# itailang/geometric_adv

Hardware: AMD Instinct MI355X
Metric: attack-iterations/sec (B=32, N=2048) at 1/2/4/8 GPUs; Chamfer rel-err vs ref (higher is better)
Workload: dtype f32 (encoder products: f16x2); 1 GPU; BASELINE configs[1]: B=32 random clouds x N=2048, output-space attack (chamfer/chamfer, dist_weight 1.0, lr 0.01), one batch per GPU; batch_per_gpu=32, n_points=2048, global_batch=32, parallelism=batches sharded, dp1, no data-path collective, ranks=1, collective_backend=none, collective_world=1

## Files before the change

### geometric_adv_amd/_abi.py

```python
import ctypes as C

_TYPES = {"i": C.c_int, "f": C.c_float, "d": C.c_double, "q": C.c_longlong, "Q": C.c_ulonglong, "z": C.c_size_t, "p": C.c_void_p,
          "s": C.c_char_p, "v": None}

SIGNATURES = {
    "geoadv_version": "i:",
    "geoadv_last_error": "s:",
    "geoadv_nn_distance": "i:iipipppppp",
    "geoadv_nn_distance_sym_workspace_floats": "z:iii",
    "geoadv_nn_distance_sym_is_screened": "i:iii",
    "geoadv_set_chamfer_screen": "i:i",
    "geoadv_nn_distance_sym": "i:iipippppppzp",
    "geoadv_chamfer_per_pc": "i:iiipppp",
    "geoadv_nn_distance_paired": "i:iippppppp",
    "geoadv_nn_distance_grad": "i:iipipppppppp",
    "geoadv_chamfer_matrix_workspace_floats": "z:iiii",
    "geoadv_chamfer_matrix": "i:iiiippppzp",
    "geoadv_approx_match_temp_floats": "z:iii",
    "geoadv_approx_match": "i:iiippppp",
    "geoadv_approx_match_mode": "i:iiiippppp",
    "geoadv_emd_sparse_levels": "i:i",
    "geoadv_match_cost": "i:iiippppp",
    "geoadv_match_cost_workspace_floats": "z:iii",
    "geoadv_match_cost_ws": "i:iiipppppzp",
    "geoadv_emd_cost_grad1_temp_floats": "z:iii",
    "geoadv_emd_cost_grad1": "i:iiipppppp",
    "geoadv_emd_cost_grad1_mode": "i:iiiipppppp",
    "geoadv_match_cost_grad": "i:iiipppppp",
    "geoadv_query_ball_point": "i:iiifippppp",
    "geoadv_selection_sort": "i:iiiipppp",
    "geoadv_group_point": "i:iiiiipppp",
    "geoadv_group_point_grad": "i:iiiiipppp",
    "geoadv_group_point_grad_workspace_bytes": "z:iiiii",
    "geoadv_group_point_grad_ws": "i:iiiiippppzp",
    "geoadv_knn_point": "i:iiiippppp",
    "geoadv_knn_dists": "i:iiippp",
    "geoadv_knn_workspace_bytes": "z:iiii",
    "geoadv_knn_point_ws": "i:iiiiipppppzp",
    "geoadv_knn_dists_ws": "i:iiiipppzp",
    "geoadv_knn_grid_mode": "i:i",
    "geoadv_farthest_point_sample": "i:iipipipppp",
    "geoadv_farthest_point_sample_plan": "i:iippp",
    "geoadv_outlier_filter": "i:iippiifppppp",
    "geoadv_sor_filter": "i:iippiidpppppp",
    "geoadv_random_drop": "i:iipiQQQppp",
    "geoadv_knn_outlier_loss_workspace_bytes": "z:iii",
    "geoadv_knn_outlier_loss": "i:iiiidppppppppzp",
    "geoadv_debug_knn_outlier_loss_launch": "i:iiidppppzp",
    "geoadv_critical_split": "i:iiippppppppp",
    "geoadv_sort_axes": "i:iipppip",
    "geoadv_batch_gather": "i:iipqpppppp",
    "geoadv_normalize_clouds": "i:iiippp",
    "geoadv_augment_batch": "i:iipqipppppp",
    "geoadv_latent_dist_matrix": "i:iiipppp",
    "geoadv_ae_create": "i:pp",
    "geoadv_ae_destroy": "v:p",
    "geoadv_set_default_encoder_arith": "i:i",
    "geoadv_ae_set_encoder_arith": "i:pi",
    "geoadv_ae_encoder_arith": "i:p",
    "geoadv_ae_status": "i:pp",
    "geoadv_ae_workspace_bytes": "z:pi",
    "geoadv_ae_critical": "i:pippppp",
    "geoadv_ae_forward": "i:pippppp",
    "geoadv_ae_decode": "i:pipppp",
    "geoadv_cls_create": "i:pp",
    "geoadv_cls_destroy": "v:p",
    "geoadv_cls_workspace_bytes": "z:pii",
    "geoadv_cls_forward": "i:piippppppp",
    "geoadv_cls_input_grad_workspace_bytes": "z:pii",
    "geoadv_cls_input_grad": "i:piippifpppppp",
    "geoadv_rotate_y": "i:iipddpp",
    "geoadv_cls_evaluate_workspace_bytes": "z:pii",
    "geoadv_cls_evaluate": "i:piippippppppp",
    "geoadv_cls_trainer_create": "i:ppp",
    "geoadv_cls_trainer_destroy": "v:p",
    "geoadv_cls_trainer_set_slots": "i:pppff",
    "geoadv_cls_trainer_step": "i:pppppp",
    "geoadv_cls_trainer_buffers": "i:pppp",
    "geoadv_cls_trainer_layout": "i:ppp",
    "geoadv_cls_trainer_counters": "i:pppp",
    "geoadv_cls_trainer_state": "i:piipp",
    "geoadv_atlas_create": "i:pppp",
    "geoadv_atlas_destroy": "v:p",
    "geoadv_atlas_workspace_bytes": "z:pii",
    "geoadv_atlas_forward": "i:piippppp",
    "geoadv_fold_create": "i:pp",
    "geoadv_fold_destroy": "v:p",
    "geoadv_fold_workspace_bytes": "z:pii",
    "geoadv_fold_graph": "i:piipppppp",
    "geoadv_fold_forward": "i:piipiQqppppppp",
    "geoadv_fold_trainer_create": "i:ppp",
    "geoadv_fold_trainer_destroy": "v:p",
    "geoadv_fold_trainer_set_slots": "i:ppp",
    "geoadv_fold_trainer_step": "i:ppipppp",
    "geoadv_fold_trainer_buffers": "i:pppp",
    "geoadv_fold_trainer_layout": "i:ppp",
    "geoadv_fold_trainer_counters": "i:ppp",
    "geoadv_fold_trainer_state": "i:piipp",
    "geoadv_fold_train_pool": "i:iiippppp",
    "geoadv_fold_train_pool_grad": "i:iiippppppp",
    "geoadv_fold_train_gmax": "i:iiipppppp",
    "geoadv_atlas_trainer_create": "i:pppp",
    "geoadv_atlas_trainer_destroy": "v:p",
    "geoadv_atlas_trainer_set_slots": "i:ppp",
    "geoadv_atlas_trainer_set_learning_rate": "i:pfi",
    "geoadv_atlas_trainer_step": "i:ppippp",
    "geoadv_atlas_trainer_buffers": "i:pppp",
    "geoadv_atlas_trainer_layout": "i:ppp",
    "geoadv_atlas_trainer_counters": "i:ppp",
    "geoadv_atlas_trainer_state": "i:piipp",
    "geoadv_train_gemm_partial_floats": "z:",
    "geoadv_train_gemm": "i:ipqqqpqqqpqqpqiiiipzpp",
    "geoadv_attack_create": "i:ppp",
    "geoadv_attack_destroy": "v:p",
    "geoadv_attack_set_inputs": "i:pppppp",
    "geoadv_attack_init_pert": "i:ppip",
    "geoadv_attack_run": "i:piiipp",
    "geoadv_attack_get_best": "i:pppppp",
    "geoadv_attack_set_source_search": "i:pi",
    "geoadv_attack_status": "i:pp",
    "geoadv_attack_peek": "i:ppppppppppp",
    "geoadv_attack_test_loss_form": "i:pi",
    "geoadv_attack_test_loss_state": "i:ppppppp",
    "geoadv_attack_test_plan": "i:pppp",
    "geoadv_debug_chamfer_sym_plan": "i:pp",
    "geoadv_debug_chamfer_sym_workspace_floats": "z:iiii",
    "geoadv_debug_h2_split": "i:pipppp",
    "geoadv_debug_emd_sparse_state": "i:iiiippp",
    "geoadv_attack_search_state": "i:pppp",
    "geoadv_trainer_create": "i:ppp",
    "geoadv_trainer_destroy": "v:p",
    "geoadv_trainer_step": "i:pppppp",
    "geoadv_trainer_forward_backward": "i:pppppp",
    "geoadv_trainer_apply": "i:pfp",
    "geoadv_trainer_set_world": "i:pi",
    "geoadv_trainer_num_phases": "i:",
    "geoadv_trainer_run_phase": "i:pippp",
    "geoadv_trainer_exchange": "i:pipp",
    "geoadv_trainer_fetch": "i:pppp",
    "geoadv_trainer_buffers": "i:pppp",
    "geoadv_trainer_layout": "i:pp",
    "geoadv_trainer_state": "i:piipp",
    "geoadv_trainer_export": "i:ppp",
    "geoadv_attack_profile": "i:pi",
    "geoadv_attack_profile_read": "i:pipp",
    "geoadv_attack_markers": "i:pi",
    "geoadv_attack_profile_stride": "i:pi",
}


def ctypes_signature(name):
    ret, _, args = SIGNATURES[name].partition(":")
    return _TYPES[ret], tuple(_TYPES[a] for a in args)


GEOADV_OK, GEOADV_EINVAL = 0, 1
GEOADV_EMD_FAST, GEOADV_EMD_REFERENCE, GEOADV_EMD_DENSE_LEVELS = 0, 1, 0x100
GEOADV_KNN_AUTO, GEOADV_KNN_ALL_POINTS, GEOADV_KNN_GRID, GEOADV_KNN_GRID_SHELLS = 0, 1, 2, 3
GEOADV_KNN_LOSS_SURFACE = 0x100
GEOADV_FPS_AUTO, GEOADV_FPS_WORKGROUP, GEOADV_FPS_WAVE = 0, 1, 2
GEOADV_NORMALIZE_IDENTITY, GEOADV_NORMALIZE_UNIT_BALL, GEOADV_NORMALIZE_BOUNDING_BOX = 0, 1, 2
GEOADV_AUGMENT_RECORD = 45
GEOADV_ENC_LAYERS, GEOADV_DEC_LAYERS = 5, 3
GEOADV_ENC_ARITH_AUTO, GEOADV_ENC_ARITH_F32, GEOADV_ENC_ARITH_BF16X3, GEOADV_ENC_ARITH_F16X2 = -1, 0, 1, 2
GEOADV_CLS_LAYERS = 20
GEOADV_CLS_LOSS_XENT, GEOADV_CLS_LOSS_CW_TARGETED, GEOADV_CLS_LOSS_CW_UNTARGETED = 0, 1, 2
GEOADV_CLS_OPT_ADAM, GEOADV_CLS_OPT_MOMENTUM = 0, 1
(GEOADV_CLS_STATE_BN_MEAN, GEOADV_CLS_STATE_BN_VAR, GEOADV_CLS_STATE_MOVING_MEAN, GEOADV_CLS_STATE_MOVING_VAR,
 GEOADV_CLS_STATE_DROPOUT_MASK, GEOADV_CLS_STATE_POOL_ARGMAX, GEOADV_CLS_STATE_T1, GEOADV_CLS_STATE_T2, GEOADV_CLS_STATE_LOGITS,
 GEOADV_CLS_STATE_SLOT1, GEOADV_CLS_STATE_SLOT2, GEOADV_CLS_STATE_PRE_BN, GEOADV_CLS_STATE_BN_INV, GEOADV_CLS_STATE_BN_SHIFT) = range(14)
GEOADV_ATLAS_ENC_LAYERS, GEOADV_ATLAS_MAX_DEC_LAYERS = 5, 7
GEOADV_FOLD_ENC_LAYERS, GEOADV_FOLD_DEC_LAYERS = 7, 6
GEOADV_FOLD_PICKS_GIVEN, GEOADV_FOLD_PICKS_DEVICE = 0, 1
(GEOADV_FOLD_STATE_BN_MEAN, GEOADV_FOLD_STATE_BN_VAR, GEOADV_FOLD_STATE_RUNNING_MEAN, GEOADV_FOLD_STATE_RUNNING_VAR,
 GEOADV_FOLD_STATE_BN_INV, GEOADV_FOLD_STATE_BN_SHIFT, GEOADV_FOLD_STATE_PRE_BN, GEOADV_FOLD_STATE_POOL_WINNER,
 GEOADV_FOLD_STATE_GMAX_ROW, GEOADV_FOLD_STATE_HIDDEN, GEOADV_FOLD_STATE_PICKS, GEOADV_FOLD_STATE_COLS, GEOADV_FOLD_STATE_COV,
 GEOADV_FOLD_STATE_CODE, GEOADV_FOLD_STATE_MID, GEOADV_FOLD_STATE_RECON, GEOADV_FOLD_STATE_CHAMFER_IDX, GEOADV_FOLD_STATE_SLOT1,
 GEOADV_FOLD_STATE_SLOT2) = range(19)
(GEOADV_ATLAS_STATE_BN_MEAN, GEOADV_ATLAS_STATE_BN_VAR, GEOADV_ATLAS_STATE_RUNNING_MEAN, GEOADV_ATLAS_STATE_RUNNING_VAR,
 GEOADV_ATLAS_STATE_BN_INV, GEOADV_ATLAS_STATE_BN_SHIFT, GEOADV_ATLAS_STATE_PRE_BN, GEOADV_ATLAS_STATE_GMAX_ROW,
 GEOADV_ATLAS_STATE_TEMPLATE, GEOADV_ATLAS_STATE_LATENT, GEOADV_ATLAS_STATE_RECON, GEOADV_ATLAS_STATE_CHAMFER_IDX,
 GEOADV_ATLAS_STATE_SLOT1, GEOADV_ATLAS_STATE_SLOT2) = range(14)
GEOADV_LOSS_ADV_CHAMFER, GEOADV_LOSS_ADV_LATENT = 0, 1
GEOADV_LOSS_DIST_CHAMFER, GEOADV_LOSS_DIST_PERT = 0, 1
GEOADV_ENC_BWD_AUTO, GEOADV_ENC_BWD_MASKED, GEOADV_ENC_BWD_JACOBIAN = 0, 1, 2
GEOADV_CHAMFER_AUTO, GEOADV_CHAMFER_TWO_SCAN, GEOADV_CHAMFER_SYMMETRIC = 0, 1, 2
GEOADV_PLAN_COUNT = 9
GEOADV_TRAIN_LOSS_CHAMFER, GEOADV_TRAIN_LOSS_EMD = 0, 1
(GEOADV_TRAIN_STATE_ACT, GEOADV_TRAIN_STATE_BN_MEAN, GEOADV_TRAIN_STATE_BN_INV_STD, GEOADV_TRAIN_STATE_BN_SCALE,
 GEOADV_TRAIN_STATE_BN_SHIFT, GEOADV_TRAIN_STATE_IDX1, GEOADV_TRAIN_STATE_IDX2, GEOADV_TRAIN_STATE_POOL_MAX,
 GEOADV_TRAIN_STATE_POOL_TIES, GEOADV_TRAIN_STATE_DEC1, GEOADV_TRAIN_STATE_DEC2) = range(11)
(GEOADV_PROF_ENCODER_FWD, GEOADV_PROF_DECODER_FWD, GEOADV_PROF_CHAMFER_FWD, GEOADV_PROF_LOSS_GRAD, GEOADV_PROF_DECODER_BWD,
 GEOADV_PROF_ENCODER_BWD, GEOADV_PROF_ADAM, GEOADV_PROF_COUNT) = range(8)


def _ptrs(count, *names):
    return [(n, C.c_void_p * count) for n in names]


class BatchAugment(C.Structure):
    _fields_ = [("seed", C.c_ulonglong), ("counter", C.c_ulonglong), ("slot_offset", C.c_int), ("noise_mu", C.c_float),
                ("noise_sigma", C.c_float), ("noise_clip", C.c_float), ("rot_count", C.c_int), ("rotate_first", C.c_int)]


class CloudAugment(C.Structure):
    _fields_ = [("seed", C.c_ulonglong), ("counter", C.c_ulonglong), ("slot_offset", C.c_int), ("sample", C.c_int),
                ("rot_axes", C.c_int), ("range_rot", C.c_float), ("rot_3d", C.c_int), ("scale", C.c_int), ("scale_min", C.c_float),
                ("scale_max", C.c_float), ("flip_axes", C.c_int), ("translate", C.c_int), ("translate_scale", C.c_float)]
    DEFAULTS = dict(range_rot=360.0, scale_min=0.75, scale_max=1.25, translate_scale=0.03)


class AEWeights(C.Structure):
    _fields_ = [("n_points", C.c_int), ("enc_dims", C.c_int * (GEOADV_ENC_LAYERS + 1)), ("dec_dims", C.c_int * (GEOADV_DEC_LAYERS + 1))] + \
               _ptrs(GEOADV_ENC_LAYERS, "enc_w", "enc_b", "bn_gamma", "bn_beta", "bn_mean", "bn_var") + \
               _ptrs(GEOADV_DEC_LAYERS, "dec_w", "dec_b")


class ClsWeights(C.Structure):
    _fields_ = [("num_classes", C.c_int)] + _ptrs(GEOADV_CLS_LAYERS, "w", "b", "gamma", "beta", "mean", "var")


class ClsTrainConfig(C.Structure):
    _fields_ = [("batch", C.c_int), ("n_points", C.c_int), ("optimizer", C.c_int), ("learning_rate", C.c_float),
                ("momentum", C.c_float), ("decay_step", C.c_int), ("decay_rate", C.c_float), ("initial_step", C.c_int),
                ("dropout_seed", C.c_int)]


class AtlasConfig(C.Structure):
    _fields_ = [(f, C.c_int) for f in ("nb_primitives", "points_per_primitive", "dim_template", "bottleneck_size",
                                       "hidden_neurons", "num_layers", "activation", "decoder_bn")]


class AtlasWeights(C.Structure):
    _fields_ = _ptrs(GEOADV_ATLAS_ENC_LAYERS, "enc_w", "enc_b", "enc_gamma", "enc_beta", "enc_mean", "enc_var") + \
               _ptrs(GEOADV_ATLAS_MAX_DEC_LAYERS, "dec_w", "dec_b", "dec_gamma", "dec_beta", "dec_mean", "dec_var")


class FoldWeights(C.Structure):
    _fields_ = _ptrs(GEOADV_FOLD_ENC_LAYERS, "enc_w", "enc_b", "enc_gamma", "enc_beta", "enc_mean", "enc_var") + \
               _ptrs(GEOADV_FOLD_DEC_LAYERS, "dec_w", "dec_b")


class FoldTrainConfig(C.Structure):
    _fields_ = [("batch", C.c_int), ("n_points", C.c_int), ("learning_rate", C.c_float), ("weight_decay", C.c_float),
                ("seed", C.c_longlong), ("initial_step", C.c_longlong), ("initial_ordinal", C.c_longlong)]


class AtlasTrainConfig(C.Structure):
    _fields_ = [("batch", C.c_int), ("n_points", C.c_int), ("points_per_primitive", C.c_int), ("learning_rate", C.c_float),
                ("seed", C.c_longlong), ("initial_step", C.c_longlong), ("initial_tracked", C.c_longlong)]


class AttackConfig(C.Structure):
    _fields_ = [("batch", C.c_int), ("loss_adv_type", C.c_int), ("loss_dist_type", C.c_int),
                ("max_point_pert_weight", C.c_float), ("max_point_dist_weight", C.c_float),
                ("learning_rate", C.c_float), ("emd_weight", C.c_float), ("all_pairs_source_dist", C.c_int),
                ("emd_weight_mode", C.c_int), ("recompute_backward", C.c_int), ("encoder_backward", C.c_int),
                ("separate_adam", C.c_int), ("chamfer_kernel", C.c_int),
                ("knn_rule", C.c_int), ("knn_thresh", C.c_float),
                ("knn_weight", C.c_float), ("knn_k", C.c_int), ("knn_alpha", C.c_float), ("loss_in_scan", C.c_int)]


class TrainConfig(C.Structure):
    _fields_ = [("batch", C.c_int), ("learning_rate", C.c_float), ("bn_decay", C.c_float), ("loss", C.c_int),
                ("max_workgroups", C.c_int)]


STRUCTS = {"geoadv_batch_augment": BatchAugment, "geoadv_cloud_augment": CloudAugment, "geoadv_ae_weights": AEWeights,
           "geoadv_cls_weights": ClsWeights, "geoadv_cls_train_config": ClsTrainConfig, "geoadv_atlas_config": AtlasConfig,
           "geoadv_atlas_weights": AtlasWeights, "geoadv_fold_weights": FoldWeights, "geoadv_fold_train_config": FoldTrainConfig,
           "geoadv_atlas_train_config": AtlasTrainConfig, "geoadv_attack_config": AttackConfig, "geoadv_train_config": TrainConfig}
```

### geometric_adv_amd/adv_ae.py

```python
import ctypes as C
import math
import time

import numpy as np
import torch

from . import _abi, _lib
from ._abi import AttackConfig as _AttackConfig
from .adversary import init_pert_value
from .autoencoder import PointNetAE


class Configuration:

    def __init__(self, batch_size, n_points, weights, loss="chamfer", loss_adv_type="chamfer",
                 loss_dist_type="chamfer", dist_weight_list=(1.0,), max_point_pert_weight=0.0,
                 max_point_dist_weight=0.0, num_iterations=500, num_iterations_thresh=400,
                 learning_rate=0.01, ae_name="autoencoder", emd_weight=0.0, verbose=False, batch_slots=1,
                 chamfer_prune=True, emd_reference_weights=False, recompute_backward=False, separate_adam=False,
                 chamfer_kernel="auto", encoder_backward="auto", emd_dense_levels=False, encoder_arith=None, loss_in_scan=True,
                 knn_weight=0.0, knn_k=5, knn_alpha=1.05, knn_rule="sor", knn_thresh=0.04):
        self.batch_size = int(batch_size)
        self.n_input = [int(n_points), 3]
        self.n_output = [int(n_points), 3]
        self.weights = weights
        self.loss = loss
        self.loss_adv_type = loss_adv_type
        self.loss_dist_type = loss_dist_type
        self.dist_weight_list = list(dist_weight_list)
        self.max_point_pert_weight = float(max_point_pert_weight)
        self.max_point_dist_weight = float(max_point_dist_weight)
        self.num_iterations = int(num_iterations)
        self.num_iterations_thresh = int(num_iterations_thresh)
        self.learning_rate = float(learning_rate)
        self.ae_name = ae_name
        self.emd_weight = float(emd_weight)
        self.verbose = verbose
        self.batch_slots = int(batch_slots)
        if chamfer_prune not in (True, False, "always", "pinned"):
            raise ValueError("chamfer_prune must be True (grid search except for tiny batches; adaptive), 'pinned' (the same, never "
                             "switched off by adapt_source_search), False or 'always'")
        self.chamfer_prune = chamfer_prune
        self.emd_reference_weights = bool(emd_reference_weights)
        self.encoder_arith = encoder_arith
        self.emd_dense_levels = bool(emd_dense_levels)
        self.recompute_backward = bool(recompute_backward)
        self.separate_adam = bool(separate_adam)
        if chamfer_kernel not in CHAMFER_KERNELS:
            raise ValueError("chamfer_kernel must be one of %s" % sorted(CHAMFER_KERNELS))
        self.chamfer_kernel = chamfer_kernel
        if encoder_backward not in ENCODER_BACKWARDS:
            raise ValueError("encoder_backward must be one of %s" % sorted(ENCODER_BACKWARDS))
        self.encoder_backward = encoder_backward
        if loss_in_scan not in (True, False, "always"):
            raise ValueError("loss_in_scan must be True (where it pays), False or 'always'")
        self.loss_in_scan = loss_in_scan
        self.knn_weight, self.knn_k, self.knn_alpha = float(knn_weight), int(knn_k), float(knn_alpha)
        self.knn_rule, self.knn_thresh = knn_rule, float(knn_thresh)
        if self.knn_weight != 0.0:
            if knn_rule not in KNN_RULES:
                raise ValueError("knn_rule must be one of %s (got %r)" % (sorted(KNN_RULES), knn_rule))
            n = self.n_input[0]
            if not math.isfinite(self.knn_weight):
                raise ValueError("knn_weight must be finite (got %r)" % self.knn_weight)
            if loss_dist_type == "pert":
                raise ValueError("knn_weight needs loss_dist_type='chamfer': the 'pert' path has no Chamfer gradient to add the term to")
            surface = knn_rule == "surface"
            max_k = KNN_SURFACE_MAX_K if surface else KNN_TERM_MAX_K
            if not 1 <= self.knn_k <= max_k:
                raise ValueError("knn_k must be in [1, %d]%s (got %d)" % (max_k, " under knn_rule='surface'" if surface else "", self.knn_k))
            if surface:
                if not (self.knn_thresh >= 0.0 and math.isfinite(self.knn_thresh) and self.knn_thresh <= 3.4028234663852886e38):
                    raise ValueError("knn_thresh must be finite and >= 0 (got %r)" % self.knn_thresh)
            elif not (self.knn_alpha >= 0.0 and math.isfinite(self.knn_alpha) and self.knn_alpha <= 3.4028234663852886e38):
                raise ValueError("knn_alpha must be finite and >= 0 (got %r)" % self.knn_alpha)
            if not self.knn_k + 2 <= n <= KNN_TERM_MAX_POINTS:
                raise ValueError("the kNN term needs clouds of knn_k + 2 = %d <= n_points <= %d (got %d)"
                                 % (self.knn_k + 2, KNN_TERM_MAX_POINTS, n))
            if self.batch_size > KNN_TERM_MAX_BATCH:
                raise ValueError("the kNN term takes at most %d clouds per batch (got %d)" % (KNN_TERM_MAX_BATCH, self.batch_size))


CHAMFER_KERNELS = {"auto": _abi.GEOADV_CHAMFER_AUTO, "two_scan": _abi.GEOADV_CHAMFER_TWO_SCAN, "symmetric": _abi.GEOADV_CHAMFER_SYMMETRIC}
ENCODER_BACKWARDS = {"auto": _abi.GEOADV_ENC_BWD_AUTO, "masked": _abi.GEOADV_ENC_BWD_MASKED, "jacobian": _abi.GEOADV_ENC_BWD_JACOBIAN}
KNN_TERM_MAX_K, KNN_TERM_MAX_POINTS, KNN_TERM_MAX_BATCH = 15, 16384, 65535
KNN_RULES = {"sor": 0, "surface": 1}
KNN_SURFACE_MAX_K = 7
PROF_NAMES = ["encoder_fwd", "decoder_fwd", "chamfer_fwd", "loss_grad", "decoder_bwd", "encoder_bwd", "adam"]


class AdvAE:
    def __init__(self, adversary_name, configuration, device=None, ae=None):
        c = configuration
        self.configuration = c
        self.name = adversary_name
        if c.loss != "chamfer":
            raise ValueError("loss=%r: AdvAE as shipped only builds with loss='chamfer' (adv_ae.py:124 fails for 'emd')" % c.loss)
        if c.loss_adv_type not in ("chamfer", "latent"):
            raise ValueError("loss_adv_type must be 'latent' or 'chamfer' (run_attack.py:49)")
        if c.loss_dist_type not in ("pert", "chamfer"):
            raise ValueError("loss_dist_type must be 'pert' or 'chamfer' (run_attack.py:50)")
        self.device = torch.device(device if device is not None else "cuda:0")
        self.ae = ae if ae is not None else PointNetAE(c.weights, c.n_input[0], c.ae_name, self.device,
                                                       encoder_arith=getattr(c, "encoder_arith", None))
        self.n = c.n_input[0]
        self.B = c.batch_size
        emd_mode = (_abi.GEOADV_EMD_REFERENCE if getattr(c, "emd_reference_weights", False) else _abi.GEOADV_EMD_FAST) | \
                   (_abi.GEOADV_EMD_DENSE_LEVELS if getattr(c, "emd_dense_levels", False) else 0)
        cfg = _AttackConfig(self.B, _abi.GEOADV_LOSS_ADV_LATENT if c.loss_adv_type == "latent" else _abi.GEOADV_LOSS_ADV_CHAMFER,
                            _abi.GEOADV_LOSS_DIST_PERT if c.loss_dist_type == "pert" else _abi.GEOADV_LOSS_DIST_CHAMFER,
                            c.max_point_pert_weight, c.max_point_dist_weight, c.learning_rate, c.emd_weight,
                            {True: 0, "pinned": 0, False: 1, "always": 2}[getattr(c, "chamfer_prune", True)], emd_mode,
                            1 if getattr(c, "recompute_backward", False) else 0, ENCODER_BACKWARDS[getattr(c, "encoder_backward", "auto")],
                            1 if getattr(c, "separate_adam", False) else 0,
                            CHAMFER_KERNELS[getattr(c, "chamfer_kernel", "auto")],
                            KNN_RULES[getattr(c, "knn_rule", "sor")] if getattr(c, "knn_weight", 0.0) != 0.0 else 0,
                            float(getattr(c, "knn_thresh", 0.04)),
                            float(getattr(c, "knn_weight", 0.0)), int(getattr(c, "knn_k", 5)), float(getattr(c, "knn_alpha", 1.05)),
                            {True: 0, False: 1, "always": 2}[getattr(c, "loss_in_scan", True)])
        self._h = C.c_void_p()
        with torch.cuda.device(self.device):
            _lib.check(_lib.lib().geoadv_attack_create(C.byref(self._h), self.ae.handle, C.byref(cfg)), "attack_create")
        self.last_history = None

    def __del__(self):
        try:
            if getattr(self, "_h", None) is not None and self._h.value:
                _lib.lib().geoadv_attack_destroy(self._h)
                self._h = C.c_void_p()
        except Exception:
            pass

    def _dev(self, a, shape=None):
        t = a if isinstance(a, torch.Tensor) else torch.as_tensor(np.asarray(a, dtype=np.float32))
        t = t.to(self.device, dtype=torch.float32).contiguous()
        if shape is not None and tuple(t.shape) != tuple(shape):
            raise ValueError("expected shape %s, got %s" % (tuple(shape), tuple(t.shape)))
        return t

    def set_inputs(self, source_pc, target_pc, target_latent, dist_weight):
        B, n = self.B, self.n
        x = self._dev(source_pc, (B, n, 3)); gt = self._dev(target_pc, (B, n, 3))
        tz = None if target_latent is None else self._dev(target_latent, (B, self.ae.bneck))
        if tz is not None and self.ae.bneck != 128:
            tz = torch.cat([tz, torch.zeros((B, 128 - self.ae.bneck), dtype=torch.float32, device=self.device)], dim=1).contiguous()
        w = self._dev(np.ones(B, np.float32) * dist_weight if np.isscalar(dist_weight) else dist_weight, (B,))
        with torch.cuda.device(self.device):
            _lib.check(_lib.lib().geoadv_attack_set_inputs(self._h, _lib.ptr(x), _lib.ptr(gt), _lib.ptr(tz), _lib.ptr(w),
                                                           _lib.stream_handle()), "attack_set_inputs")
        if self.configuration.chamfer_prune is True and not getattr(self, "_search_on", True):
            self.set_source_search(True)

    def init_pert(self, init=None, reset_optimizer=False):
        if init is None:
            init = init_pert_value(self.B, self.n)
        p = self._dev(init, (self.B, self.n, 3))
        with torch.cuda.device(self.device):
            _lib.check(_lib.lib().geoadv_attack_init_pert(self._h, _lib.ptr(p), int(bool(reset_optimizer)),
                                                          _lib.stream_handle()), "attack_init_pert")

    def search_state(self):
        a, b = C.c_int(0), C.c_int(0)
        with torch.cuda.device(self.device):
            _lib.check(_lib.lib().geoadv_attack_search_state(self._h, C.byref(a), C.byref(b), _lib.stream_handle()), "attack_search_state")
        return bool(a.value), b.value

    def run(self, first_iteration, iterations, thresh, history=None):
        if history is not None and tuple(history.shape) != (iterations, 6, self.B):
            raise ValueError("history must be of shape (iterations, 6, batch)")
        with torch.cuda.device(self.device):
            _lib.check(_lib.lib().geoadv_attack_run(self._h, int(first_iteration), int(iterations), int(thresh),
                                                    _lib.ptr(history), _lib.stream_handle()), "attack_run")

    def get_best(self, target_ae_loss_ref, clouds=True):
        B, n = self.B, self.n
        ref = self._dev(target_ae_loss_ref, (B,))
        metrics = torch.empty((B, 5), dtype=torch.float32, device=self.device)
        adv = torch.empty((B, n, 3), dtype=torch.float32, device=self.device) if clouds else None
        recon = torch.empty((B, n, 3), dtype=torch.float32, device=self.device) if clouds else None
        with torch.cuda.device(self.device):
            _lib.check(_lib.lib().geoadv_attack_get_best(self._h, _lib.ptr(ref), _lib.ptr(metrics), _lib.ptr(adv),
                                                         _lib.ptr(recon), _lib.stream_handle()), "attack_get_best")
        return metrics, adv, recon

    def set_source_search(self, on):
        _lib.check(_lib.lib().geoadv_attack_set_source_search(self._h, int(bool(on))), "attack_set_source_search")
        self._search_on = bool(on)

    def adapt_source_search(self):
        if self.configuration.chamfer_prune is not True or not getattr(self, "_search_on", True):
            return None
        searched, handed_back = self.search_state()
        if not searched:
            return None
        if 2 * handed_back > self.B:
            self.set_source_search(False)
        return handed_back

    def status(self):
        with torch.cuda.device(self.device):
            _lib.check(_lib.lib().geoadv_attack_status(self._h, _lib.stream_handle()), "attack_status")

    def peek(self):
        B, n, dev = self.B, self.n, self.device
        f = lambda *s: torch.empty(s, dtype=torch.float32, device=dev)
        i = lambda *s: torch.empty(s, dtype=torch.int32, device=dev)
        out = dict(pert=f(B, n, 3), adv=f(B, n, 3), recon=f(B, n, 3), latent=f(B, 128), grad=f(B, n, 3),
                   idx_r1=i(B, n), idx_r2=i(B, n), idx_a1=i(B, n), idx_a2=i(B, n))
        with torch.cuda.device(dev):
            p = {k: _lib.ptr(t) for k, t in out.items()}
            _lib.check(_lib.lib().geoadv_attack_peek(self._h, p["pert"], p["adv"], p["recon"], p["latent"], p["grad"], p["idx_r1"],
                                                     p["idx_r2"], p["idx_a1"], p["idx_a2"], _lib.stream_handle()), "attack_peek")
        if self.ae.bneck != 128:
            out["latent"] = out["latent"][:, :self.ae.bneck].contiguous()
        return out

    def _test_loss_form(self, form):
        _lib.check(_lib.lib().geoadv_attack_test_loss_form(self._h, int(form)), "attack_test_loss_form")

    def _test_loss_state(self):
        B, n, dev = self.B, self.n, self.device
        f = lambda *s: torch.empty(s, dtype=torch.float32, device=dev)
        out = dict(g_recon=f(B, n, 3), g_dist=f(B, n, 3), losses=f(8, B), dist_r1=f(B, n), dist_a1=f(B, n))
        with torch.cuda.device(dev):
            p = {k: _lib.ptr(t) for k, t in out.items()}
            _lib.check(_lib.lib().geoadv_attack_test_loss_state(self._h, p["g_recon"], p["g_dist"], p["losses"], p["dist_r1"],
                                                                p["dist_a1"], _lib.stream_handle()), "attack_test_loss_state")
        return out

    def _test_plan(self):
        plan = (C.c_int * _abi.GEOADV_PLAN_COUNT)()
        jstar = torch.empty((2, self.B), dtype=torch.int32, device=self.device)
        with torch.cuda.device(self.device):
            _lib.check(_lib.lib().geoadv_attack_test_plan(self._h, plan, _lib.ptr(jstar), _lib.stream_handle()), "attack_test_plan")
        return dict(symmetric=bool(plan[0]), screened=bool(plan[1]), rtiles=plan[2], rslices=plan[3],
                    rows=("final", "partials", "packed", "merge_launch")[plan[4]], loss=("metrics", "fused", "riders")[plan[5]],
                    grad=("none", "fused_1pass", "fused_general", "step_fx_1pass", "step_fx_general", "step_sorted")[plan[6]],
                    H=plan[7], range=plan[8], jstar=jstar)

    def profile(self, classes, stride=1):
        _lib.check(_lib.lib().geoadv_attack_profile_stride(self._h, int(stride)), "attack_profile_stride")
        if classes is True:
            mask = -1
        elif not classes:
            mask = 0
        else:
            mask = sum(1 << PROF_NAMES.index(c) for c in classes)
        _lib.check(_lib.lib().geoadv_attack_profile(self._h, int(mask)), "attack_profile")

    def markers(self, enable=True):
        _lib.check(_lib.lib().geoadv_attack_markers(self._h, int(bool(enable))), "attack_markers")

    def profile_read(self):
        out = {}
        for k, name in enumerate(PROF_NAMES):
            n_, ms = C.c_int(0), C.c_float(0)
            _lib.check(_lib.lib().geoadv_attack_profile_read(self._h, k, C.byref(n_), C.byref(ms)), "attack_profile_read")
            out[name] = (n_.value, ms.value)
        return out

    def reconstruct(self, X, GT=None, compute_loss=True):
        return self.ae.reconstruct(X, GT, compute_loss)

    def attack(self, source_pc, target_latent, target_pc, target_ae_loss_ref, configuration=None, log_file=None):
        c = configuration if configuration is not None else self.configuration
        n_examples = len(source_pc)
        batch_size = c.batch_size
        assert n_examples % batch_size == 0, \
            'The number of examples (%d) should be divided by the batch size (%d)' % (n_examples, batch_size)
        n_batches = n_examples // batch_size
        if min(int(getattr(c, "batch_slots", 1)), n_batches) > 1:
            return self._attack_slots(source_pc, target_latent, target_pc, target_ae_loss_ref, n_batches, log_file)
        metrics, pcs_in, pcs_rec = [], [], []
        for i in range(n_batches):
            start_time = time.time()
            s, e = i * batch_size, (i + 1) * batch_size
            m_, a_, r_ = self._attack_one_batch(source_pc[s:e], None if target_latent is None else target_latent[s:e],
                                                target_pc[s:e], target_ae_loss_ref[s:e], log_file)
            metrics.append(m_); pcs_in.append(a_); pcs_rec.append(r_)
            duration = time.time() - start_time
            print("Batch: %04d out of %04d, attack time (minutes): %.4f" % (i + 1, n_batches, duration / 60.0))
            if log_file is not None:
                log_file.write('Batch %04d\tDuration %.4f\n' % (i + 1, duration / 60.0))
        return np.concatenate(metrics, axis=1), np.concatenate(pcs_in, axis=1), np.concatenate(pcs_rec, axis=1)

    def _attack_slots(self, source_pc, target_latent, target_pc, target_ae_loss_ref, n_batches, log_file):
        import io
        import threading
        from .dist import shard_batches
        c = self.configuration
        bs = c.batch_size
        slots = min(int(c.batch_slots), n_batches)
        if not hasattr(self, "_slot_workers"):
            self._slot_workers = []
        while len(self._slot_workers) < slots - 1:
            self._slot_workers.append(AdvAE(self.name, c, self.device, ae=self.ae))
        workers = [self] + self._slot_workers[:slots - 1]
        results, logs, errors = [None] * n_batches, [None] * n_batches, []
        lock = threading.Lock()

        def work(slot):
            try:
                with torch.cuda.device(self.device), torch.cuda.stream(torch.cuda.Stream(self.device)):
                    for i in shard_batches(n_batches, slot, slots):
                        start_time = time.time()
                        s, e = i * bs, (i + 1) * bs
                        buf = io.StringIO() if log_file is not None else None
                        results[i] = workers[slot]._attack_one_batch(source_pc[s:e], None if target_latent is None else target_latent[s:e],
                                                                     target_pc[s:e], target_ae_loss_ref[s:e], buf)
                        duration = time.time() - start_time
                        with lock:
                            print("Batch: %04d out of %04d, attack time (minutes): %.4f" % (i + 1, n_batches, duration / 60.0))
                        if buf is not None:
                            logs[i] = buf.getvalue() + 'Batch %04d\tDuration %.4f\n' % (i + 1, duration / 60.0)
            except BaseException as exc:
                errors.append(exc)

        threads = [threading.Thread(target=work, args=(k,)) for k in range(slots)]
        for t in threads:
            t.start()
        for t in threads:
            t.join()
        if errors:
            raise errors[0]
        if log_file is not None:
            for text in logs:
                log_file.write(text)
        return (np.concatenate([r[0] for r in results], axis=1), np.concatenate([r[1] for r in results], axis=1),
                np.concatenate([r[2] for r in results], axis=1))

    def _attack_one_batch(self, source_pc, target_latent, target_pc, target_ae_loss_ref, log_file=None, init_pert=None):
        c = self.configuration
        W = len(c.dist_weight_list)
        B, n = self.B, self.n
        metrics_all = np.zeros((W, B, 5), np.float32)
        adv_all = np.zeros((W, B, n, 3), np.float32)
        rec_all = np.zeros((W, B, n, 3), np.float32)
        hist = torch.empty((c.num_iterations, 6, B), dtype=torch.float32, device=self.device)
        self.last_history = []
        for i, dist_weight in enumerate(c.dist_weight_list):
            self.set_inputs(source_pc, target_pc, target_latent, float(dist_weight))
            self.init_pert(init_pert)
            self.run(0, c.num_iterations, c.num_iterations_thresh, hist)
            m_, a_, r_ = self.get_best(target_ae_loss_ref)
            self.status()
            self.adapt_source_search()
            h = hist.cpu().numpy()
            self.last_history.append(h)
            step = (c.num_iterations // 10) or 1
            for it in range(c.num_iterations):
                if (it + 1) % step == 0:
                    la, ld, lp, lm = (h[it, k].mean() for k in range(4))
                    loss = (h[it, 0] + dist_weight * h[it, 1]).mean()
                    if c.verbose:
                        print("Weight {} of {}, Iteration {} of {}, loss={} loss_adv={} loss_dist={} loss_pert={} loss_max={}"
                              .format(i + 1, W, it + 1, c.num_iterations, loss, la, ld, lp, lm))
                    if log_file is not None:
                        log_file.write('Dist weight %.4f\tIteration %.04d\tloss: %.4f\tloss_adv: %.4f\tloss_dist: %.4f\t'
                                       'loss_pert: %.4f\tloss_max: %.4f\n' % (dist_weight, it + 1, loss, la, ld, lp, lm))
            metrics_all[i] = m_.cpu().numpy(); adv_all[i] = a_.cpu().numpy(); rec_all[i] = r_.cpu().numpy()
        return metrics_all, adv_all, rec_all
```

### geometric_adv_amd/csrc/attack.hip

```cpp
#include "ae.h"
#include "chamfer_sym.h"
#include "chamfer_grad.h"
#include "chamfer_grid.h"
#include "encoder_jac.h"
#include "decoder_tail.h"
#include "knn_loss.h"
#define LC_STAMP(K, I) GA_STAMP(K, I)
#include "loss_cgrad.h"
#include "host_util.h"
#include <assert.h>
#include <dlfcn.h>
#include <limits.h>
#include <math.h>
#include <stdlib.h>
#include <vector>

#pragma clang fp contract(off)

namespace geoadv {

__global__ __launch_bounds__(256) void loss_metrics_kernel(LossArgs a) { loss_metrics_body(a, blockIdx.x, gridDim.x); }

__global__ __launch_bounds__(256) void chamfer_per_pc_kernel(int n, int m, const float *d1, const float *d2, float *out) {
    __shared__ float shf[4][8];
    __shared__ int shi[4][2];
    const int b = blockIdx.x, t = threadIdx.x;
    CloudRed r;
    r.s1 = r.s2 = r.s3 = r.s4 = r.sp = 0.f;
    r.ma = r.mp = -1.f;
    r.ja = r.jp = INT_MAX;
    for (int j = t; j < n; j += 256) r.s3 += d1[(size_t)b * n + j];
    for (int j = t; j < m; j += 256) r.s4 += d2[(size_t)b * m + j];
    r = block_reduce(r, shf, shi);
    if (t == 0) out[b] = r.s3 * (1.0f / (float)n) + r.s4 * (1.0f / (float)m);
}

__global__ __launch_bounds__(CGA_THREADS) void chamfer_grad_attack_kernel(CGradArgs a) {
    extern __shared__ __attribute__((aligned(16))) unsigned lds[];
    const CGradProblem pr = a.pr[blockIdx.y];
    const int b = blockIdx.x, n = a.n;
    const float wb = pr.w ? pr.w[b] : 1.0f;
    const float gd = wb * (1.0f / (float)n);
    GradSide s;
    s.n_own = n; s.n_oth = n;
    s.own = pr.p + (size_t)b * n * 3; s.oth = pr.q + (size_t)b * n * 3;
    s.match_own = pr.idx1 + (size_t)b * n; s.match_oth = pr.idx2 + (size_t)b * n;
    s.gd_own = nullptr; s.gd_oth = nullptr; s.gd_own_s = gd; s.gd_oth_s = gd;
    s.jstar = (pr.jstar && pr.extra_w > 0.f) ? pr.jstar[b] : -1;
    s.extra = wb * pr.extra_w;
    s.gout = pr.g + (size_t)b * n * 3;
    chamfer_grad_side<true, CGA_THREADS>(s, lds, a.P);
}

__global__ __launch_bounds__(CGA_THREADS) void chamfer_grad_attack_fx_kernel(CGradArgs a, int H) {
    extern __shared__ __attribute__((aligned(16))) unsigned fx_lds[];
    cgrad_fx(a, blockIdx.y / H, blockIdx.x, blockIdx.y % H, H, fx_lds);
}

__global__ __launch_bounds__(CGA_THREADS) void loss_cgrad_kernel(LossArgs la, CGradArgs ca, int H) {
    extern __shared__ __attribute__((aligned(16))) unsigned lc_lds[];
    GA_STAMP(0, 0);
    loss_cgrad_block(la, ca, H, blockIdx.x, gridDim.x, blockIdx.y, lc_lds);
    GA_STAMP(0, 7);
}

struct AdamArgs {
    int n, B;
    float *pert, *m, *v;
    float *g_enc;
    const float *g_dist;
    const float *w, *losses;
    const int *jstar;
    int loss_dist_type;
    float mp_pert_w;
    float alpha, one_minus_b1, one_minus_b2, eps;
    float *grad_out;
    const float *x;
    float *adv_out;
};

__global__ __launch_bounds__(256) void adam_kernel(AdamArgs a) {
    const size_t per = (size_t)a.n * 3;
    const size_t e = (size_t)blockIdx.x * 256 + threadIdx.x;
    if (e >= per * a.B) return;
    const int b = (int)(e / per);
    float g = a.g_enc[e];
    a.g_enc[e] = 0.f;
    if (a.loss_dist_type == GEOADV_LOSS_DIST_PERT) {
        const float p = a.pert[e];
        const float wb = a.w[b];
        float gp = wb * (p / a.losses[2 * a.B + b]);
        if (a.mp_pert_w > 0.f) {
            const int pt = (int)((e % per) / 3);
            if (pt == a.jstar[a.B + b]) gp += wb * a.mp_pert_w * (p / a.losses[6 * a.B + b]);
        }
        g += gp;
    } else {
        g += a.g_dist[e];
    }
    if (a.grad_out) a.grad_out[e] = g;
    float m = a.m[e], v = a.v[e];
    m += (g - m) * a.one_minus_b1;
    v += (g * g - v) * a.one_minus_b2;
    a.m[e] = m; a.v[e] = v;
    const float pnew = a.pert[e] - (m * a.alpha) / (sqrtf(v) + a.eps);
    a.pert[e] = pnew;
    a.adv_out[e] = a.x[e] + pnew;
}

__global__ void axpy_kernel(float *y, const float *x, float a, size_t count) {
    const size_t i = (size_t)blockIdx.x * blockDim.x + threadIdx.x;
    if (i < count) y[i] = fmaf(a, x[i], y[i]);
}

__global__ void fill_kernel(float *p, float v, size_t count) {
    const size_t i = (size_t)blockIdx.x * blockDim.x + threadIdx.x;
    if (i < count) p[i] = v;
}

__global__ void best_metrics_kernel(int B, const float *best_metrics, const float *best_err, const float *ref, float *out, const int *failed) {
    const int b = blockIdx.x * blockDim.x + threadIdx.x;
    if (b >= B) return;
    if (failed && *failed) {
        for (int k = 0; k < 5; ++k) out[b * 5 + k] = NAN;
        return;
    }
    out[b * 5 + 0] = best_metrics[b * 4 + 0];
    out[b * 5 + 1] = best_metrics[b * 4 + 1];
    out[b * 5 + 2] = best_metrics[b * 4 + 2];
    out[b * 5 + 3] = best_metrics[b * 4 + 3] / ref[b];
    out[b * 5 + 4] = best_err[b];
}

__global__ void xcd_probe_kernel(unsigned *out) {
    if (threadIdx.x == 0) {
        unsigned v;
        asm volatile("s_getreg_b32 %0, hwreg(HW_REG_XCC_ID)" : "=s"(v));
        out[blockIdx.x] = v & 0xf;
    }
}

}

using namespace geoadv;

struct geoadv_attack {
    const geoadv_ae *ae;
    geoadv_attack_config cfg;
    int B, n;
    void *arena; size_t arena_bytes;
    float *x, *gt, *tz, *w;
    float *pert, *m, *v;
    float *adv, *recon, *g_recon, *g_dist, *g_enc, *grad_last;
    float *r1, *r2, *a1, *a2; int *ir1, *ir2, *ia1, *ia2;
    ForwardScratch fs;
    float *dz, *dec_partial;
    float *losses; int *jstar;
    float *best_err, *best_metrics, *best_adv, *best_recon;
    float *emd_temp, *emd_cost, *emd_g1;
    char *knn_ws; size_t knn_ws_bytes;
    double *knn_loss;
    float *sym_ws;
    unsigned long long *row64;
    int test_loss_form = 0;
    int plan[GEOADV_PLAN_COUNT] = {};
    bool cgrad_done;
    bool counted = false;
    bool chamfer_prune;
    int *need_adv[2];
    int *need_last;
    float *x_box;
    int grid_calls;
    unsigned *masks;
    float *jac;
    bool jac_valid;
    unsigned *tail_ready;
    unsigned tail_epoch;
    unsigned *loss_done;
    unsigned loss_target;
    bool host_loss_force;
    bool host_loss;
    int cus;
    bool chamfer_sym;
    float beta1_pow, beta2_pow;
    bool fwd_valid;
    bool adv_valid;
    bool fuse_adam;
    bool adam_pending;
    FusedAdam pending;
    unsigned prof_mask;
    int prof_stride;
    unsigned prof_seen[GEOADV_PROF_COUNT];
    std::vector<hipEvent_t> ev;
    int ev_used;
    struct Mark { int which, e0, e1; };
    std::vector<Mark> marks;
    double prof_ms[GEOADV_PROF_COUNT];
    int prof_n[GEOADV_PROF_COUNT];
    hipStream_t prof_stream;
    bool markers;
};

namespace {

int prof_flush(geoadv_attack *at) {
    if (at->marks.empty()) return GEOADV_OK;
    GA_HIP(hipStreamSynchronize(at->prof_stream));
    for (const auto &mk : at->marks) {
        float ms = 0;
        GA_HIP(hipEventElapsedTime(&ms, at->ev[mk.e0], at->ev[mk.e1]));
        at->prof_ms[mk.which] += ms;
        at->prof_n[mk.which] += 1;
    }
    at->marks.clear();
    at->ev_used = 0;
    return GEOADV_OK;
}

struct Roctx {
    int (*push)(const char *) = nullptr;
    int (*pop)() = nullptr;
    Roctx() {
        void *h = dlopen("libroctx64.so.4", RTLD_LAZY | RTLD_GLOBAL);
        if (!h) h = dlopen("libroctx64.so", RTLD_LAZY | RTLD_GLOBAL);
        if (!h) return;
        push = reinterpret_cast<int (*)(const char *)>(dlsym(h, "roctxRangePushA"));
        pop = reinterpret_cast<int (*)()>(dlsym(h, "roctxRangePop"));
        if (!push || !pop) { push = nullptr; pop = nullptr; }
    }
};
const Roctx &roctx() { static const Roctx r; return r; }
const char *const kClassNames[GEOADV_PROF_COUNT] = {"geoadv:encoder_fwd", "geoadv:decoder_fwd", "geoadv:chamfer_fwd", "geoadv:loss_grad",
                                                    "geoadv:decoder_bwd", "geoadv:encoder_bwd", "geoadv:adam"};

struct ProfScope {
    geoadv_attack *at; int which; int e0, e1; hipStream_t st; bool on, kernel, marked;
    ProfScope(geoadv_attack *a, int w, hipStream_t s, bool kernel_timed = false)
        : at(a), which(w), e0(-1), e1(-1), st(s), on((a->prof_mask >> w) & 1u), kernel(kernel_timed),
          marked(a->markers && roctx().push != nullptr) {
        if (marked) roctx().push(kClassNames[w]);
        if (on && at->prof_stride > 1) on = (at->prof_seen[w]++ % (unsigned)at->prof_stride) == 0;
        if (!on) return;
        if (at->ev_used + 2 > (int)at->ev.size()) prof_flush(at);
        e0 = at->ev_used++;
        if (kernel) e1 = at->ev_used++;
        else (void)hipEventRecord(at->ev[e0], st);
    }
    hipEvent_t start() const { return on && kernel ? at->ev[e0] : nullptr; }
    hipEvent_t stop() const { return on && kernel ? at->ev[e1] : nullptr; }
    ~ProfScope() {
        if (marked) roctx().pop();
        if (!on) return;
        if (!kernel) {
            e1 = at->ev_used++;
            (void)hipEventRecord(at->ev[e1], st);
        }
        at->marks.push_back({which, e0, e1});
    }
};


bool cgrad_step_sorted(int n) { return n > CG_FX_MAX_N_PLANE; }

struct ForwardForm { bool pruned, rides_scan, rides_latent, loss_fused, merge_in_loss, jac_rides; };

int do_forward(geoadv_attack *at, float *hist_slot, int keep, hipStream_t st) {
    const DeviceAE &A = at->ae->d;
    const int B = at->B, n = at->n, H = cgrad_fx_parts(n);
    const bool adv_chamfer = at->cfg.loss_adv_type == GEOADV_LOSS_ADV_CHAMFER;
    const bool dist_chamfer = at->cfg.loss_dist_type == GEOADV_LOSS_DIST_CHAMFER;
    const bool max_term = dist_chamfer && at->cfg.max_point_dist_weight > 0.f;
    ForwardForm f;
    f.pruned = at->chamfer_prune && chamfer_grid_supports(n, n);
    f.rides_scan = f.pruned && chamfer_grid_rides(n) && at->chamfer_sym;
    f.rides_latent = f.pruned && chamfer_grid_rides(n) && !at->chamfer_sym;
    f.loss_fused = (adv_chamfer || dist_chamfer) && !max_term && n <= CG_FX_MAX_N_PLANE;
    f.merge_in_loss = f.loss_fused && adv_chamfer && dist_chamfer;
    f.jac_rides = at->jac && at->chamfer_sym;
    SymPlan plan{};
    if (at->chamfer_sym) {
        SymRequest rq{2, B, n, n, true, f.pruned, f.rides_scan, f.jac_rides};
        rq.loss = at->host_loss && f.merge_in_loss && !at->emd_temp; rq.loss_rows = 1 + 2 * H; rq.loss_force = at->host_loss_force;
        rq.defer = f.merge_in_loss; rq.packed = f.merge_in_loss && at->row64 != nullptr;
        rq.pack_from = (at->test_loss_form & 1) ? SYM_PACK_FROM + 1 : SYM_PACK_FROM;
        rq.screen = chamfer_sym_screen_on();
        plan = chamfer_sym_plan(rq);
    }
    const SymRows rows = chamfer_sym_rows(plan, at->sym_ws, at->row64);
    const bool packed = plan.rows == GEOADV_PLAN_ROWS_PACKED, hosted = plan.loss.count > 0;
    const int call = at->grid_calls;
    int *need_new = at->need_adv[f.rides_scan ? (call + 1) & 1 : 0];
    const int *need_scan = at->need_adv[f.rides_scan ? call & 1 : 0];
    if (f.pruned) { at->grid_calls++; at->need_last = need_new; }
    {
        ProfScope ps(at, GEOADV_PROF_ENCODER_FWD, st, true);
        if (int rc = launch_encoder_fwd(A, B, at->x, at->pert, (at->adv_valid && !at->adam_pending) ? nullptr : at->adv, at->fs.pmax,
                                        at->fs.parg, at->fs.pcnt, at->masks, st, ps.start(), ps.stop(),
                                        at->adam_pending ? &at->pending : nullptr)) return rc;
        at->adam_pending = false;
        at->adv_valid = true;
    }
    {
        ProfScope ps(at, GEOADV_PROF_DECODER_FWD, st);
        if (f.pruned && !f.rides_scan && !f.rides_latent) {
            if (int rc = launch_chamfer_grid(at->adv, at->x, at->a1, at->ia1, at->a2, at->ia2, B, n, need_new, call, at->x_box, st)) return rc;
        }
        if (f.rides_latent) {
            if (int rc = launch_latent_decode_and_grid(A, B, at->fs.pmax, at->fs.parg, at->fs.pcnt, at->fs.z, at->fs.crit, at->fs.zcnt,
                                                       at->fs.dense, at->fs.d1, at->fs.d2, at->adv, at->x, at->a1, at->ia1, at->a2,
                                                       at->ia2, n, need_new, call, at->x_box, st)) return rc;
        } else if (int rc = launch_latent_decode(A, B, at->fs.pmax, at->fs.parg, at->fs.pcnt, at->fs.z, at->fs.crit, at->fs.zcnt,
                                                 at->fs.dense, at->fs.d1, at->fs.d2, st)) return rc;
        if (int rc = launch_decoder_fc2(A, B, at->fs.d2, at->recon, st, packed ? at->row64 : nullptr, packed ? 2 * (size_t)B * n : 0)) return rc;
    }
    const JacArgs jargs{n, at->masks, at->fs.crit, at->fs.z, at->fs.dense, at->jac};
    at->jac_valid = f.jac_rides;
    if (at->jac && !f.jac_rides && at->cfg.encoder_backward == GEOADV_ENC_BWD_JACOBIAN) {
        ProfScope ps(at, GEOADV_PROF_ENCODER_BWD, st);
        if (int rc = launch_encoder_jac(A, B, jargs, st)) return rc;
        at->jac_valid = true;
    }
    LossArgs la;
    CGradArgs ca;
    int np = 0;
    la.n = n; la.loss_adv_type = at->cfg.loss_adv_type; la.loss_dist_type = at->cfg.loss_dist_type;
    la.mp_pert_w = at->cfg.max_point_pert_weight; la.mp_dist_w = at->cfg.max_point_dist_weight;
    la.r1 = at->r1; la.r2 = at->r2; la.a1 = at->a1; la.a2 = at->a2; la.pert = at->pert;
    la.z = at->fs.z; la.tz = at->tz; la.w = at->w; la.losses = at->losses; la.jstar = at->jstar;
    la.emd_cost = at->emd_temp ? at->emd_cost : nullptr; la.emd_weight = at->cfg.emd_weight;
    la.dz_latent = at->dz; la.hist = hist_slot; la.keep = keep; la.best_err = at->best_err;
    la.best_metrics = at->best_metrics; la.adv = at->adv; la.recon = at->recon;
    la.best_adv = at->best_adv; la.best_recon = at->best_recon;
    la.fold_in_lds = (at->test_loss_form & 2) ? 1 : 0; ca.general = la.fold_in_lds;
    la.part = rows; la.a1_need = f.pruned ? need_scan : nullptr; la.a1_all = f.pruned ? 0 : 1; la.r1_out = at->r1; la.a1_out = at->a1;
    if (adv_chamfer) {
        ca.pr[np] = CGradProblem{at->recon, at->gt, at->ir1, at->ir2, at->g_recon, nullptr, nullptr, 0.f};
        if (rows.deferred) {
            ca.pr[np].part_d = rows.rowpart_d; ca.pr[np].part_i = rows.rowpart_i; ca.pr[np].part_slices = rows.slices;
            ca.pr[np].part_need = nullptr; ca.pr[np].idx1_out = at->ir1; ca.pr[np].part_w = rows.row64;
        }
        ++np;
    }
    if (dist_chamfer) {
        ca.pr[np] = CGradProblem{at->adv, at->x, at->ia1, at->ia2, at->g_dist, at->w, at->jstar, 0.f};
        if (rows.deferred) {
            const size_t off = (size_t)B * rows.slices * n;
            ca.pr[np].part_d = rows.rowpart_d + off; ca.pr[np].part_i = rows.rowpart_i + off; ca.pr[np].part_slices = rows.slices;
            ca.pr[np].part_need = f.pruned ? need_scan : nullptr; ca.pr[np].idx1_out = at->ia1;
            ca.pr[np].part_w = rows.row64 ? rows.row64 + (size_t)B * n : nullptr;
        }
        ++np;
    }
    ca.n = n; ca.P = 0;
    {
        ProfScope ps(at, GEOADV_PROF_CHAMFER_FWD, st);
        if (at->chamfer_sym) {
            const ChamferPair pairs[2] = {{at->recon, at->gt, at->r1, at->ir1, at->r2, at->ir2},
                                          {at->adv, at->x, at->a1, at->ia1, at->a2, at->ia2}};
            const GridArgs rider{at->adv, at->x, at->a1, at->ia1, at->a2, at->ia2, n, need_new, need_scan, call, at->x_box};
            JacRider jr;
            jr.j = jargs; jr.A = A; jr.first_block = 0; jr.blocks = 0; jr.raise_prio = 0;
            LossRider lr;
            if (hosted) {
                at->loss_target += plan.loss_arrivals;
                lr = LossRider{la, ca, H, 1 + 2 * H, 0, 0, B, at->loss_done, at->loss_target, reinterpret_cast<int *>(at->tail_ready + B)};
            }
            if (int rc = launch_chamfer_sym(plan, pairs, at->sym_ws, f.pruned ? need_scan : nullptr, f.rides_scan ? &rider : nullptr,
                                            f.jac_rides ? &jr : nullptr, hosted ? &lr : nullptr, at->row64, st)) return rc;
        } else {
            ChamferScan all[4] = {{at->recon, at->gt, at->r1, at->ir1, n, n}, {at->gt, at->recon, at->r2, at->ir2, n, n},
                                  {at->adv, at->x, at->a1, at->ia1, n, n}, {at->x, at->adv, at->a2, at->ia2, n, n}};
            if (f.pruned) all[2].need = all[3].need = need_scan;
            if (int rc = launch_chamfer_scans(all, 4, B, st)) return rc;
        }
    }
    if (at->emd_temp) {
        ProfScope ps(at, GEOADV_PROF_CHAMFER_FWD, st);
        if (int rc = geoadv_emd_cost_grad1_mode(at->cfg.emd_weight_mode, B, n, n, at->recon, at->gt, at->emd_cost, at->emd_g1, at->emd_temp, st)) return rc;
    }
    at->cgrad_done = hosted || f.loss_fused;
    if (!hosted) {
        ProfScope ps(at, GEOADV_PROF_LOSS_GRAD, st);
        if (f.loss_fused) loss_cgrad_kernel<<<dim3(B, 1 + np * H), CGA_THREADS, loss_cgrad_lds_bytes(n), st>>>(la, ca, H);
        else loss_metrics_kernel<<<B, 256, 0, st>>>(la);
        GA_LAUNCH_CHECK();
    }
    {
        const int general = (at->test_loss_form & 2) ? 1 : 0;
        int *pl = at->plan;
        pl[GEOADV_PLAN_SYMMETRIC] = at->chamfer_sym ? 1 : 0; pl[GEOADV_PLAN_SCREENED] = plan.shape.mx ? 1 : 0;
        pl[GEOADV_PLAN_RTILES] = plan.shape.rtiles; pl[GEOADV_PLAN_RSLICES] = plan.rslices; pl[GEOADV_PLAN_ROWS] = plan.rows;
        pl[GEOADV_PLAN_LOSS] = hosted ? GEOADV_PLAN_LOSS_RIDERS : f.loss_fused ? GEOADV_PLAN_LOSS_FUSED : GEOADV_PLAN_LOSS_METRICS;
        if (at->cgrad_done) pl[GEOADV_PLAN_GRAD] = cgrad_fx_one_pass(n, H, general) ? GEOADV_PLAN_GRAD_FUSED_1PASS : GEOADV_PLAN_GRAD_FUSED_GENERAL;
        else if (np == 0) pl[GEOADV_PLAN_GRAD] = GEOADV_PLAN_GRAD_NONE;
        else if (cgrad_step_sorted(n)) pl[GEOADV_PLAN_GRAD] = GEOADV_PLAN_GRAD_STEP_SORTED;
        else pl[GEOADV_PLAN_GRAD] = cgrad_fx_one_pass(n, H, 0) ? GEOADV_PLAN_GRAD_STEP_FX_1PASS : GEOADV_PLAN_GRAD_STEP_FX_GENERAL;
        const int g = pl[GEOADV_PLAN_GRAD];
        const bool fx = !(g == GEOADV_PLAN_GRAD_NONE || g == GEOADV_PLAN_GRAD_STEP_SORTED);
        pl[GEOADV_PLAN_H] = fx ? H : 0; pl[GEOADV_PLAN_RANGE] = fx ? cgrad_fx_range(n) : 0;
    }
    at->fwd_valid = true;
    return GEOADV_OK;
}

int pow2_ge(int v) { int p = 2; while (p < v) p <<= 1; return p; }

int launch_cgrad(const CGradProblem *pr, int np, int B, int n, hipStream_t st) {
    CGradArgs ca;
    for (int i = 0; i < np; ++i) ca.pr[i] = pr[i];
    ca.n = n; ca.P = pow2_ge(n);
    if (!cgrad_step_sorted(n)) {
        const int H = cgrad_fx_parts(n);
        chamfer_grad_attack_fx_kernel<<<dim3(B, np * H), CGA_THREADS, cgrad_fx_lds_bytes(n), st>>>(ca, H);
        GA_LAUNCH_CHECK();
        return GEOADV_OK;
    }
    chamfer_grad_attack_kernel<<<dim3(B, np), CGA_THREADS, sizeof(unsigned) * (size_t)ca.P * (ca.P <= CG_TERMS_MAX_P ? 4 : 1), st>>>(ca);
    GA_LAUNCH_CHECK();
    return GEOADV_OK;
}

int do_step(geoadv_attack *at, hipStream_t st) {
    const DeviceAE &A = at->ae->d;
    const int B = at->B, n = at->n;
    const bool adv_chamfer = at->cfg.loss_adv_type == GEOADV_LOSS_ADV_CHAMFER;
    const bool dist_chamfer = at->cfg.loss_dist_type == GEOADV_LOSS_DIST_CHAMFER;
    const CGradProblem p_recon{at->recon, at->gt, at->ir1, at->ir2, at->g_recon, nullptr, nullptr, 0.f};
    const CGradProblem p_dist{at->adv, at->x, at->ia1, at->ia2, at->g_dist, at->w, at->jstar, at->cfg.max_point_dist_weight};
    if (!at->cgrad_done) {
        ProfScope ps(at, GEOADV_PROF_LOSS_GRAD, st);
        CGradProblem pr[2];
        int np = 0;
        if (adv_chamfer) pr[np++] = p_recon;
        if (dist_chamfer) pr[np++] = p_dist;
        if (np)
            if (int rc = launch_cgrad(pr, np, B, n, st)) return rc;
    }
    at->cgrad_done = false;
    if (at->knn_ws) {
        ProfScope ps(at, GEOADV_PROF_LOSS_GRAD, st);
        const bool surface = at->cfg.knn_rule == 1;
        if (int rc = launch_knn_term(at->cfg.knn_rule, B, n, at->cfg.knn_k, (double)(surface ? at->cfg.knn_thresh : at->cfg.knn_alpha),
                                     at->cfg.knn_weight, at->w, at->adv, at->g_dist, at->knn_loss, at->knn_ws, at->knn_ws_bytes, st)) return rc;
    }
    if (adv_chamfer && at->emd_temp) {
        ProfScope ps(at, GEOADV_PROF_LOSS_GRAD, st);
        const size_t total = (size_t)B * n * 3;
        axpy_kernel<<<(unsigned)((total + 255) / 256), 256, 0, st>>>(at->g_recon, at->emd_g1, at->cfg.emd_weight / (float)n, total);
        GA_LAUNCH_CHECK();
    }
    if (adv_chamfer) {
        ProfScope ps(at, GEOADV_PROF_DECODER_BWD, st);
        if (at->jac_valid) {
            if (B + 2 * cdiv(n, 32) > at->cus) {
                if (int rc = launch_decoder_bwd(A, B, at->g_recon, at->fs.d1, at->fs.d2, at->dec_partial, at->dz, st, at->fs.crit, at->jac,
                                                at->fs.dense, at->g_enc)) return rc;
                if (int rc = launch_encoder_bwd_dense(A, B, at->adv, at->fs.z, at->fs.zcnt, at->dz, at->fs.dense, at->g_enc, st)) return rc;
            } else {
            if (int rc = launch_decoder_fc2_bwd(A, B, at->g_recon, at->dec_partial, st)) return rc;
            TailDenseArgs ta;
            ta.batch = B; ta.chunks = decoder_bwd_chunks(A); ta.n = n;
            ta.partial = at->dec_partial; ta.d1 = at->fs.d1; ta.d2 = at->fs.d2; ta.dz = at->dz;
            ta.ja = JacApply{at->fs.crit, at->jac, at->fs.dense, at->g_enc, n};
            ta.adv = at->adv; ta.z = at->fs.z; ta.zcnt = at->fs.zcnt; ta.dense_flag = at->fs.dense; ta.g_enc = at->g_enc;
            ta.ready = at->tail_ready; ta.epoch = ++at->tail_epoch; ta.spin_timeout = reinterpret_cast<int *>(at->tail_ready + B);
            if (int rc = launch_decoder_tail_dense(A, ta, st)) return rc;
            }
        } else if (int rc = launch_decoder_bwd(A, B, at->g_recon, at->fs.d1, at->fs.d2, at->dec_partial, at->dz, st)) return rc;
    }
    if (!(adv_chamfer && at->jac_valid)) {
        ProfScope ps(at, GEOADV_PROF_ENCODER_BWD, st);
        if (int rc = launch_encoder_bwd(A, B, at->adv, at->fs.crit, at->fs.z, at->fs.zcnt, at->dz, at->fs.dense, at->g_enc, at->masks, st))
            return rc;
    }
    {
        const float beta1 = 0.9f, beta2 = 0.999f;
        const float alpha = at->cfg.learning_rate * sqrtf(1.0f - at->beta2_pow) / (1.0f - at->beta1_pow);
        if (at->fuse_adam && dist_chamfer) {
            at->pending = FusedAdam{at->pert, at->m, at->v, at->g_enc, at->g_dist, at->grad_last, alpha, 1.0f - beta1, 1.0f - beta2, 1e-8f};
            at->adam_pending = true;
        } else {
            ProfScope ps(at, GEOADV_PROF_ADAM, st);
            AdamArgs aa;
            aa.n = n; aa.B = B; aa.pert = at->pert; aa.m = at->m; aa.v = at->v; aa.g_enc = at->g_enc;
            aa.g_dist = dist_chamfer ? at->g_dist : nullptr; aa.w = at->w; aa.losses = at->losses; aa.jstar = at->jstar;
            aa.loss_dist_type = at->cfg.loss_dist_type; aa.mp_pert_w = at->cfg.max_point_pert_weight;
            aa.alpha = alpha;
            aa.one_minus_b1 = 1.0f - beta1; aa.one_minus_b2 = 1.0f - beta2; aa.eps = 1e-8f;
            aa.grad_out = at->grad_last; aa.x = at->x; aa.adv_out = at->adv;
            const size_t total = (size_t)B * n * 3;
            adam_kernel<<<(unsigned)((total + 255) / 256), 256, 0, st>>>(aa);
            GA_LAUNCH_CHECK();
        }
        at->beta1_pow *= beta1;
        at->beta2_pow *= beta2;
    }
    at->fwd_valid = false;
    at->adv_valid = !at->adam_pending;
    return GEOADV_OK;
}

size_t carve_arena(geoadv_attack *at, void *base) {
    const geoadv_attack_config &cfg = at->cfg;
    const size_t B = at->B, n = at->n, bn3 = B * n * 3, bn = B * n;
    Carver c(base);
    auto F = [&](size_t count) { return c.take<float>(count); };
    auto I = [&](size_t count) { return c.take<int>(count); };
    at->x = F(bn3); at->gt = F(bn3); at->tz = F(B * 128); at->w = F(B);
    at->pert = F(bn3); at->m = F(bn3); at->v = F(bn3);
    at->adv = F(bn3); at->recon = F(bn3); at->g_recon = F(bn3); at->g_dist = F(bn3); at->g_enc = F(bn3); at->grad_last = F(bn3);
    at->r1 = F(bn); at->r2 = F(bn); at->a1 = F(bn); at->a2 = F(bn);
    at->ir1 = I(bn); at->ir2 = I(bn); at->ia1 = I(bn); at->ia2 = I(bn);
    at->fs = carve_forward_scratch(c.take<char>(carve_forward_scratch(nullptr, at->B, at->n).bytes), at->B, at->n);
    at->dz = F(B * 128); at->dec_partial = F((size_t)decoder_bwd_chunks(at->ae->d) * B * 256);
    at->losses = F(8 * B); at->jstar = I(2 * B);
    at->best_err = F(B); at->best_metrics = F(B * 4); at->best_adv = F(bn3); at->best_recon = F(bn3);
    at->sym_ws = F(chamfer_sym_workspace_floats(2, at->B, at->n, at->n));
    at->row64 = c.take<unsigned long long>(2 * bn);
    const size_t mask_words = cfg.recompute_backward ? 0 : (size_t)encoder_mask_words() * bn;
    at->masks = mask_words ? c.take<unsigned>(mask_words) : nullptr;
    const bool use_jac = mask_words != 0 && cfg.loss_adv_type == GEOADV_LOSS_ADV_CHAMFER && cfg.encoder_backward != GEOADV_ENC_BWD_MASKED;
    at->jac = use_jac ? F(B * 128 * 3) : nullptr;
    at->tail_ready = c.take<unsigned>(B + 1);
    at->loss_done = c.take<unsigned>(B);
    at->need_adv[0] = I(8 * B); at->need_adv[1] = I(8 * B);
    at->x_box = F(6 * B);
    at->emd_temp = at->emd_cost = at->emd_g1 = nullptr;
    if (cfg.emd_weight > 0.f) {
        at->emd_temp = F(geoadv_emd_cost_grad1_temp_floats(at->B, at->n, at->n) + 2);
        at->emd_cost = F(B); at->emd_g1 = F(bn3);
    }
    at->knn_ws = nullptr; at->knn_ws_bytes = 0; at->knn_loss = nullptr;
    if (cfg.knn_weight != 0.f) {
        at->knn_ws_bytes = geoadv_knn_outlier_loss_workspace_bytes(at->B, at->n, cfg.knn_k);
        at->knn_ws = c.take<char>(at->knn_ws_bytes);
        at->knn_loss = c.take<double>(B);
    }
    return c.bytes();
}

}

namespace geoadv {
int launch_chamfer_grad(const CGradProblem *pr, int np, int B, int n, hipStream_t st) { return launch_cgrad(pr, np, B, n, st); }
}

extern "C" int geoadv_chamfer_per_pc(int b, int n, int m, const float *dist1, const float *dist2, float *out, void *stream) {
    GA_REQUIRE(b >= 0 && n >= 1 && m >= 1, "chamfer_per_pc: bad dimensions (b=%d n=%d m=%d)", b, n, m);
    if (b == 0) return GEOADV_OK;
    GA_REQUIRE(dist1 && dist2 && out, "chamfer_per_pc: null pointer");
    chamfer_per_pc_kernel<<<b, 256, 0, as_stream(stream)>>>(n, m, dist1, dist2, out);
    GA_LAUNCH_CHECK();
    return GEOADV_OK;
}

extern "C" int geoadv_attack_create(geoadv_attack **out, const geoadv_ae *ae, const geoadv_attack_config *cfg) {
    GA_REQUIRE(out && ae && cfg, "attack_create: null argument");
    GA_REQUIRE(cfg->batch >= 1 && cfg->batch <= 65535, "attack_create: batch %d out of range", cfg->batch);
    GA_REQUIRE(cfg->loss_adv_type == GEOADV_LOSS_ADV_CHAMFER || cfg->loss_adv_type == GEOADV_LOSS_ADV_LATENT,
               "attack_create: unknown loss_adv_type %d", cfg->loss_adv_type);
    GA_REQUIRE(cfg->loss_dist_type == GEOADV_LOSS_DIST_CHAMFER || cfg->loss_dist_type == GEOADV_LOSS_DIST_PERT,
               "attack_create: unknown loss_dist_type %d", cfg->loss_dist_type);
    GA_REQUIRE(cfg->emd_weight >= 0.f, "attack_create: emd_weight must be >= 0");
    GA_REQUIRE((cfg->emd_weight_mode & ~GEOADV_EMD_DENSE_LEVELS) == GEOADV_EMD_FAST || (cfg->emd_weight_mode & ~GEOADV_EMD_DENSE_LEVELS) == GEOADV_EMD_REFERENCE,
               "attack_create: unknown emd_weight_mode %d", cfg->emd_weight_mode);
    GA_REQUIRE(cfg->all_pairs_source_dist >= 0 && cfg->all_pairs_source_dist <= 2, "attack_create: all_pairs_source_dist must be 0, 1 or 2");
    GA_REQUIRE(cfg->encoder_backward >= GEOADV_ENC_BWD_AUTO && cfg->encoder_backward <= GEOADV_ENC_BWD_JACOBIAN,
               "attack_create: unknown encoder_backward %d", cfg->encoder_backward);
    GA_REQUIRE(cfg->chamfer_kernel >= GEOADV_CHAMFER_AUTO && cfg->chamfer_kernel <= GEOADV_CHAMFER_SYMMETRIC,
               "attack_create: unknown chamfer_kernel %d", cfg->chamfer_kernel);
    GA_REQUIRE(cfg->emd_weight == 0.f || cfg->loss_adv_type == GEOADV_LOSS_ADV_CHAMFER,
               "attack_create: emd_weight needs the output-space attack (loss_adv_type chamfer)");
    if (cfg->knn_weight != 0.f) {
        const int n = ae->d.n_points;
        GA_REQUIRE(isfinite(cfg->knn_weight), "attack_create: knn_weight must be finite (got %g)", (double)cfg->knn_weight);
        GA_REQUIRE(cfg->loss_dist_type == GEOADV_LOSS_DIST_CHAMFER,
                   "attack_create: knn_weight needs loss_dist_type chamfer (the 'pert' path has no Chamfer gradient g_dist to add the term to)");
        GA_REQUIRE(cfg->knn_rule == 0 || cfg->knn_rule == 1, "attack_create: unknown knn_rule %d (0 = SOR, 1 = surface)", cfg->knn_rule);
        GA_REQUIRE(cfg->knn_k >= 1 && cfg->knn_k <= 15, "attack_create: knn_k=%d must be in [1, 15]", cfg->knn_k);
        if (cfg->knn_rule == 1) {
            GA_REQUIRE(cfg->knn_k <= 7, "attack_create: knn_k=%d must be in [1, 7] under knn_rule 1, as geoadv_outlier_filter's top_k", cfg->knn_k);
            GA_REQUIRE(cfg->knn_thresh >= 0.f && isfinite(cfg->knn_thresh), "attack_create: knn_thresh must be finite and >= 0 (got %g)",
                       (double)cfg->knn_thresh);
        } else
            GA_REQUIRE(cfg->knn_alpha >= 0.f && isfinite(cfg->knn_alpha), "attack_create: knn_alpha must be finite and >= 0 (got %g)", (double)cfg->knn_alpha);
        GA_REQUIRE(n >= cfg->knn_k + 2 && n <= 16384, "attack_create: the kNN term needs clouds of knn_k + 2 = %d <= n <= 16384 points (n=%d)",
                   cfg->knn_k + 2, n);
    }
    geoadv_attack *at = new geoadv_attack();
    at->ae = ae; at->cfg = *cfg; at->B = cfg->batch; at->n = ae->d.n_points;
    const size_t total = at->arena_bytes = carve_arena(at, nullptr);
    if (hipMalloc(&at->arena, total) != hipSuccess) {
        delete at;
        set_error("attack_create: hipMalloc of %zu bytes failed", total);
        return GEOADV_ENOMEM;
    }
    if (hipMemsetAsync(at->arena, 0, total, nullptr) != hipSuccess || hipStreamSynchronize(nullptr) != hipSuccess) {
        (void)hipFree(at->arena);
        delete at;
        set_error("attack_create: clearing %zu bytes failed", total);
        return GEOADV_EHIP;
    }
    const size_t carved = carve_arena(at, at->arena);
    assert(carved == at->arena_bytes); (void)carved;
    at->need_last = at->need_adv[0];
    at->jac_valid = false;
    at->tail_epoch = 0; at->loss_target = 0; at->grid_calls = 0;
    {
        int dev = 0, cus = 0;
        if (hipGetDevice(&dev) == hipSuccess && hipDeviceGetAttribute(&cus, hipDeviceAttributeMultiprocessorCount, dev) == hipSuccess) at->cus = cus;
        else at->cus = 0;
    }
    at->chamfer_prune = cfg->all_pairs_source_dist == 2 || (cfg->all_pairs_source_dist == 0 && (long)at->B * at->n >= GEOADV_SMALL_BATCH_POINTS);
    {
        at->chamfer_sym = cfg->chamfer_kernel == GEOADV_CHAMFER_AUTO ? (long)at->B * at->n >= GEOADV_SYM_MIN_POINTS
                                                                     : cfg->chamfer_kernel == GEOADV_CHAMFER_SYMMETRIC;
    }
    at->cgrad_done = false;
    at->fuse_adam = cfg->separate_adam == 0;
    at->adam_pending = false;
    at->beta1_pow = 0.9f; at->beta2_pow = 0.999f;
    at->fwd_valid = false; at->adv_valid = false;
    at->prof_mask = 0; at->ev_used = 0; at->prof_stream = nullptr; at->prof_stride = 1; at->markers = false;
    for (int i = 0; i < GEOADV_PROF_COUNT; ++i) at->prof_seen[i] = 0;
    for (int i = 0; i < GEOADV_PROF_COUNT; ++i) { at->prof_ms[i] = 0; at->prof_n[i] = 0; }
    static DeviceOnce attr;
    if (int rc = attr.run([]() -> int {
            GA_HIP(hipFuncSetAttribute(reinterpret_cast<const void *>(chamfer_grad_attack_kernel),
                                       hipFuncAttributeMaxDynamicSharedMemorySize, 160 * 1024 - 256));
            GA_HIP(hipFuncSetAttribute(reinterpret_cast<const void *>(chamfer_grad_attack_fx_kernel),
                                       hipFuncAttributeMaxDynamicSharedMemorySize, 24 * CG_FX_MAX_N));
            GA_HIP(hipFuncSetAttribute(reinterpret_cast<const void *>(loss_cgrad_kernel),
                                       hipFuncAttributeMaxDynamicSharedMemorySize, 24 * CG_FX_MAX_N));
            return GEOADV_OK;
        })) { geoadv_attack_destroy(at); return rc; }
    at->host_loss = false;
    at->host_loss_force = cfg->loss_in_scan == 2;
    if (cfg->loss_in_scan != 1 && at->chamfer_sym) {
        unsigned *d = reinterpret_cast<unsigned *>(at->sym_ws), h[64];
        xcd_probe_kernel<<<64, 64>>>(d);
        if (hipMemcpy(h, d, sizeof(h), hipMemcpyDeviceToHost) == hipSuccess) {
            bool ok = true;
            for (int i = 8; i < 64; ++i) ok = ok && h[i] == h[i & 7];
            for (int i = 0; i < 8; ++i)
                for (int j = 0; j < i; ++j) ok = ok && h[i] != h[j];
            at->host_loss = ok;
        }
        (void)hipGetLastError();
    }
    ae->attack_refs.fetch_add(1);
    at->counted = true;
    *out = at;
    return GEOADV_OK;
}

extern "C" void geoadv_attack_destroy(geoadv_attack *at) {
    if (!at) return;
    if (at->counted) at->ae->attack_refs.fetch_sub(1);
    for (auto e : at->ev) (void)hipEventDestroy(e);
    (void)hipFree(at->arena);
    delete at;
}

extern "C" int geoadv_attack_set_inputs(geoadv_attack *at, const float *source_pc, const float *target_pc,
                                        const float *target_latent, const float *dist_weight, void *stream) {
    GA_REQUIRE(at && source_pc && target_pc && dist_weight, "attack_set_inputs: null argument");
    GA_REQUIRE(target_latent || at->cfg.loss_adv_type != GEOADV_LOSS_ADV_LATENT,
               "attack_set_inputs: target_latent is required for loss_adv_type 'latent'");
    hipStream_t st = as_stream(stream);
    const size_t bn3 = (size_t)at->B * at->n * 3;
    if (at->adam_pending)
        if (int rc = do_forward(at, nullptr, 0, st)) return rc;
    GA_HIP(hipMemcpyAsync(at->x, source_pc, 4 * bn3, hipMemcpyDeviceToDevice, st));
    GA_HIP(hipMemcpyAsync(at->gt, target_pc, 4 * bn3, hipMemcpyDeviceToDevice, st));
    if (target_latent) GA_HIP(hipMemcpyAsync(at->tz, target_latent, 4 * (size_t)at->B * 128, hipMemcpyDeviceToDevice, st));
    GA_HIP(hipMemcpyAsync(at->w, dist_weight, 4 * (size_t)at->B, hipMemcpyDeviceToDevice, st));
    if (int rc = launch_chamfer_grid_box(at->x, at->B, at->n, at->x_box, st)) return rc;
    for (int i = 0; i < 2; ++i)
        GA_HIP(hipMemsetAsync(at->need_adv[i], 0, sizeof(int) * 8 * (size_t)at->B, st));
    GA_HIP(hipMemsetAsync(at->tail_ready + at->B, 0, sizeof(unsigned), st));
    at->fwd_valid = false; at->adv_valid = false;
    return GEOADV_OK;
}

extern "C" int geoadv_attack_init_pert(geoadv_attack *at, const float *init_pert, int reset_optimizer, void *stream) {
    GA_REQUIRE(at && init_pert, "attack_init_pert: null argument");
    hipStream_t st = as_stream(stream);
    const size_t bn3 = (size_t)at->B * at->n * 3;
    at->adam_pending = false;
    GA_HIP(hipMemsetAsync(at->tail_ready + at->B, 0, sizeof(unsigned), st));
    GA_HIP(hipMemcpyAsync(at->pert, init_pert, 4 * bn3, hipMemcpyDeviceToDevice, st));
    if (reset_optimizer) {
        GA_HIP(hipMemsetAsync(at->m, 0, 4 * bn3, st));
        GA_HIP(hipMemsetAsync(at->v, 0, 4 * bn3, st));
        at->beta1_pow = 0.9f; at->beta2_pow = 0.999f;
    }
    fill_kernel<<<(at->B + 255) / 256, 256, 0, st>>>(at->best_err, 1e10f, (size_t)at->B);
    GA_LAUNCH_CHECK();
    GA_HIP(hipMemsetAsync(at->best_metrics, 0, 4 * (size_t)at->B * 4, st));
    GA_HIP(hipMemsetAsync(at->best_adv, 0, 4 * bn3, st));
    GA_HIP(hipMemsetAsync(at->best_recon, 0, 4 * bn3, st));
    at->fwd_valid = false; at->adv_valid = false;
    return GEOADV_OK;
}

extern "C" int geoadv_attack_run(geoadv_attack *at, int first_iteration, int iterations, int thresh,
                                 float *metrics_hist, void *stream) {
    GA_REQUIRE(at && first_iteration >= 0 && iterations >= 0, "attack_run: bad arguments");
    hipStream_t st = as_stream(stream);
    at->prof_stream = st;
    if (iterations == 0) return GEOADV_OK;
    if (!at->fwd_valid)
        if (int rc = do_forward(at, nullptr, 0, st)) return rc;
    for (int i = 0; i < iterations; ++i) {
        if (int rc = do_step(at, st)) return rc;
        const int it = first_iteration + i;
        const int keep = (it + 1) >= thresh ? 1 : 0;
        float *slot = metrics_hist ? metrics_hist + (size_t)i * 6 * at->B : nullptr;
        if (int rc = do_forward(at, slot, keep, st)) return rc;
    }
    return GEOADV_OK;
}

extern "C" int geoadv_attack_get_best(geoadv_attack *at, const float *target_ae_loss_ref, float *metrics, float *adv,
                                      float *recon, void *stream) {
    GA_REQUIRE(at, "attack_get_best: null handle");
    hipStream_t st = as_stream(stream);
    const size_t bn3 = (size_t)at->B * at->n * 3;
    if (metrics) {
        GA_REQUIRE(target_ae_loss_ref, "attack_get_best: target_ae_loss_ref is required for the metrics");
        best_metrics_kernel<<<(at->B + 63) / 64, 64, 0, st>>>(at->B, at->best_metrics, at->best_err, target_ae_loss_ref, metrics,
                                                              reinterpret_cast<const int *>(at->tail_ready + at->B));
        GA_LAUNCH_CHECK();
    }
    if (adv) GA_HIP(hipMemcpyAsync(adv, at->best_adv, 4 * bn3, hipMemcpyDeviceToDevice, st));
    if (recon) GA_HIP(hipMemcpyAsync(recon, at->best_recon, 4 * bn3, hipMemcpyDeviceToDevice, st));
    return GEOADV_OK;
}

extern "C" int geoadv_attack_set_source_search(geoadv_attack *at, int on) {
    GA_REQUIRE(at, "attack_set_source_search: null handle");
    at->chamfer_prune = on != 0;
    return GEOADV_OK;
}

extern "C" int geoadv_attack_test_loss_form(geoadv_attack *at, int form) {
    GA_REQUIRE(at && form >= 0 && form <= 3, "attack_test_loss_form: bad arguments");
    at->test_loss_form = form;
    return GEOADV_OK;
}

extern "C" int geoadv_attack_test_loss_state(geoadv_attack *at, float *g_recon, float *g_dist, float *losses, float *dist_r1,
                                             float *dist_a1, void *stream) {
    GA_REQUIRE(at, "attack_test_loss_state: null handle");
    hipStream_t st = as_stream(stream);
    const size_t bn3 = 4 * (size_t)at->B * at->n * 3, bn = 4 * (size_t)at->B * at->n;
    if (at->adam_pending || !at->fwd_valid)
        if (int rc = do_forward(at, nullptr, 0, st)) return rc;
    GA_REQUIRE(at->cgrad_done || !(g_recon || g_dist), "attack_test_loss_state: this configuration forms the Chamfer gradients in the step");
    if (g_recon) GA_HIP(hipMemcpyAsync(g_recon, at->g_recon, bn3, hipMemcpyDeviceToDevice, st));
    if (g_dist) GA_HIP(hipMemcpyAsync(g_dist, at->g_dist, bn3, hipMemcpyDeviceToDevice, st));
    if (losses) GA_HIP(hipMemcpyAsync(losses, at->losses, 4 * 8 * (size_t)at->B, hipMemcpyDeviceToDevice, st));
    if (dist_r1) GA_HIP(hipMemcpyAsync(dist_r1, at->r1, bn, hipMemcpyDeviceToDevice, st));
    if (dist_a1) GA_HIP(hipMemcpyAsync(dist_a1, at->a1, bn, hipMemcpyDeviceToDevice, st));
    return GEOADV_OK;
}

extern "C" int geoadv_attack_test_plan(geoadv_attack *at, int plan[GEOADV_PLAN_COUNT], int *jstar, void *stream) {
    GA_REQUIRE(at && plan, "attack_test_plan: null argument");
    hipStream_t st = as_stream(stream);
    if (at->adam_pending || !at->fwd_valid)
        if (int rc = do_forward(at, nullptr, 0, st)) return rc;
    for (int i = 0; i < GEOADV_PLAN_COUNT; ++i) plan[i] = at->plan[i];
    if (jstar) GA_HIP(hipMemcpyAsync(jstar, at->jstar, sizeof(int) * 2 * (size_t)at->B, hipMemcpyDeviceToDevice, st));
    return GEOADV_OK;
}

extern "C" int geoadv_attack_status(geoadv_attack *at, void *stream) {
    GA_REQUIRE(at, "attack_status: null handle");
    hipStream_t st = as_stream(stream);
    int failed = 0;
    GA_HIP(hipMemcpyAsync(&failed, at->tail_ready + at->B, sizeof(int), hipMemcpyDeviceToHost, st));
    GA_HIP(hipStreamSynchronize(st));
    if (failed) {
        set_error("attack: an in-launch hand-off (decoder backward tail -> dense encoder backward of a cloud with a tied pool "
                  "maximum) timed out since the last set_inputs / init_pert; iterations after it used a stale latent gradient -- "
                  "the results of this run are invalid");
        return GEOADV_EHIP;
    }
    return ae_range_check(at->ae, st, "attack_status");
}

extern "C" int geoadv_attack_peek(geoadv_attack *at, float *pert, float *adv, float *recon, float *latent, float *grad,
                                  int *idx_r1, int *idx_r2, int *idx_a1, int *idx_a2, void *stream) {
    GA_REQUIRE(at, "attack_peek: null handle");
    hipStream_t st = as_stream(stream);
    const size_t bn3 = 4 * (size_t)at->B * at->n * 3, bn = 4 * (size_t)at->B * at->n;
    if (at->adam_pending || (!at->fwd_valid && (adv || recon || latent || idx_r1 || idx_r2 || idx_a1 || idx_a2)))
        if (int rc = do_forward(at, nullptr, 0, st)) return rc;
    if (pert) GA_HIP(hipMemcpyAsync(pert, at->pert, bn3, hipMemcpyDeviceToDevice, st));
    if (adv) GA_HIP(hipMemcpyAsync(adv, at->adv, bn3, hipMemcpyDeviceToDevice, st));
    if (recon) GA_HIP(hipMemcpyAsync(recon, at->recon, bn3, hipMemcpyDeviceToDevice, st));
    if (latent) GA_HIP(hipMemcpyAsync(latent, at->fs.z, 4 * (size_t)at->B * 128, hipMemcpyDeviceToDevice, st));
    if (grad) GA_HIP(hipMemcpyAsync(grad, at->grad_last, bn3, hipMemcpyDeviceToDevice, st));
    if (idx_r1) GA_HIP(hipMemcpyAsync(idx_r1, at->ir1, bn, hipMemcpyDeviceToDevice, st));
    if (idx_r2) GA_HIP(hipMemcpyAsync(idx_r2, at->ir2, bn, hipMemcpyDeviceToDevice, st));
    if (idx_a1) GA_HIP(hipMemcpyAsync(idx_a1, at->ia1, bn, hipMemcpyDeviceToDevice, st));
    if (idx_a2) GA_HIP(hipMemcpyAsync(idx_a2, at->ia2, bn, hipMemcpyDeviceToDevice, st));
    return GEOADV_OK;
}

extern "C" int geoadv_attack_search_state(geoadv_attack *at, int *searched, int *handed_back, void *stream) {
    GA_REQUIRE(at && searched && handed_back, "attack_search_state: null argument");
    const bool pruned = at->chamfer_prune && chamfer_grid_supports(at->n, at->n);
    *searched = pruned ? 1 : 0;
    *handed_back = 0;
    if (!pruned) return GEOADV_OK;
    hipStream_t st = as_stream(stream);
    std::vector<int> h(8 * (size_t)at->B);
    GA_HIP(hipMemcpyAsync(h.data(), at->need_last, sizeof(int) * h.size(), hipMemcpyDeviceToHost, st));
    GA_HIP(hipStreamSynchronize(st));
    for (int c = 0; c < at->B; ++c) {
        int any = 0;
        for (int k = 0; k < 8; ++k) any |= h[8 * (size_t)c + k];
        *handed_back += any ? 1 : 0;
    }
    return GEOADV_OK;
}

extern "C" int geoadv_attack_profile(geoadv_attack *at, int enable) {
    GA_REQUIRE(at, "attack_profile: null handle");
    if (enable && at->ev.empty()) {
        at->ev.resize(4096);
        for (auto &e : at->ev) GA_HIP(hipEventCreate(&e));
    }
    if (at->prof_mask) { if (int rc = prof_flush(at)) return rc; }
    at->prof_mask = (unsigned)enable;
    if (enable) for (int i = 0; i < GEOADV_PROF_COUNT; ++i) { at->prof_ms[i] = 0; at->prof_n[i] = 0; }
    return GEOADV_OK;
}

extern "C" int geoadv_attack_markers(geoadv_attack *at, int enable) {
    GA_REQUIRE(at, "attack_markers: null handle");
    GA_REQUIRE(!enable || roctx().push, "attack_markers: libroctx64.so not found");
    at->markers = enable != 0;
    return GEOADV_OK;
}

extern "C" int geoadv_attack_profile_stride(geoadv_attack *at, int stride) {
    GA_REQUIRE(at && stride >= 1, "attack_profile_stride: bad arguments");
    at->prof_stride = stride;
    return GEOADV_OK;
}

extern "C" int geoadv_attack_profile_read(geoadv_attack *at, int which, int *launches, float *total_ms) {
    GA_REQUIRE(at && which >= 0 && which < GEOADV_PROF_COUNT && launches && total_ms, "attack_profile_read: bad arguments");
    if (int rc = prof_flush(at)) return rc;
    *launches = at->prof_n[which];
    *total_ms = (float)at->prof_ms[which];
    return GEOADV_OK;
}
GA_STAMPS_GETTER(geoadv_debug_stamps_attack)
```

### geometric_adv_amd/csrc/chamfer_sym.h

```cpp
#pragma once
#include "common.h"

namespace geoadv {

struct ChamferPair {
    const float *p, *q;
    float *dist1; int *idx1;
    float *dist2; int *idx2;
};

constexpr int SYM_PACK_FROM = 8;
struct SymRows { const float *rowpart_d; const int *rowpart_i; int slices, clouds; bool deferred; const unsigned long long *row64; int unused_ = 0; };

struct SymRequest {
    int np, b, n, m;
    bool loop = false;
    bool need1 = false;
    bool search = false, jac = false, loss = false;
    int loss_rows = 0;
    bool loss_force = false;
    bool defer = false;
    bool packed = false;
    int pack_from = SYM_PACK_FROM;
    int q_clouds = 0, pair_base = 0;
    bool screen = true;
};
struct SymShape { int rw, cw, rtiles, C, S, cslices; bool mx; };
struct SymBlocks { int first, count; };
struct SymPlan {
    SymRequest req;
    SymShape shape;
    int kernel;
    int rslices;
    int rows;
    SymBlocks search, scan, jac, loss;
    unsigned grid;
    size_t lds_bytes;
    unsigned loss_arrivals;
    int raise_prio;
    size_t group_floats;
    size_t part_off[4];
};
SymPlan chamfer_sym_plan(const SymRequest &r);
bool chamfer_sym_screen_on();
SymRows chamfer_sym_rows(const SymPlan &p, const float *workspace, const unsigned long long *row64);

#ifdef __HIPCC__
__device__ __forceinline__ bool sym_needed(const int *need, int c) {
    if (!need) return true;
    const int4 lo = reinterpret_cast<const int4 *>(need)[2 * c], hi = reinterpret_cast<const int4 *>(need)[2 * c + 1];
    return (lo.x | lo.y | lo.z | lo.w | hi.x | hi.y | hi.z | hi.w) != 0;
}

__device__ __forceinline__ float sym_merge_pick(const float *d, int slices, size_t stride, int &slice) {
    float bd = d[0];
    int bs = 0;
    for (int s0 = 1; s0 < slices; s0 += 8) {
        float vd[8];
#pragma unroll
        for (int u = 0; u < 8; ++u) vd[u] = d[(size_t)(s0 + u < slices ? s0 + u : 0) * stride];
#pragma unroll
        for (int u = 0; u < 8; ++u)
            if (s0 + u < slices && vd[u] < bd) { bd = vd[u]; bs = s0 + u; }
    }
    slice = bs;
    return bd;
}
__device__ __forceinline__ void sym_merge_slices(const float *d, const int *i, int slices, size_t stride, float &od, int &oi) {
    int s;
    od = sym_merge_pick(d, slices, stride, s);
    oi = i[(size_t)s * stride];
}
__device__ __forceinline__ unsigned long long sym_pack(float d, int i) {
    return ((unsigned long long)__float_as_uint(d) << 32) | (unsigned)i;
}
__device__ __forceinline__ float sym_merge_min(const float *d, int slices, size_t stride) {
    float bd = d[0];
    for (int s0 = 1; s0 < slices; s0 += 8) {
        float vd[8];
#pragma unroll
        for (int u = 0; u < 8; ++u) vd[u] = d[(size_t)(s0 + u < slices ? s0 + u : 0) * stride];
#pragma unroll
        for (int u = 0; u < 8; ++u) bd = fminf(bd, vd[u]);
    }
    return bd;
}
#endif

struct CGradProblem {
    const float *p, *q;
    const int *idx1, *idx2;
    float *g;
    const float *w;
    const int *jstar;
    float extra_w;
    const float *part_d; const int *part_i; int part_slices; const int *part_need; int *idx1_out;
    const unsigned long long *part_w;
};
int launch_chamfer_grad(const CGradProblem *pr, int np, int B, int n, hipStream_t st);

struct ChamferScan {
    const float *query;
    const float *target;
    float *dist;
    int *idx;
    int nq, nt;
    const int *need;
};
int launch_chamfer_scans(const ChamferScan *scans, int nscan, int b, hipStream_t stream);

int launch_nn_nonfinite_fix(int b, int n, const float *xyz1, int m, const float *xyz2, float *dist1, int *idx1, float *dist2,
                            int *idx2, hipStream_t stream);

size_t chamfer_sym_workspace_floats(int pairs, int b, int n, int m);
struct GridArgs;
struct JacRider;
struct LossRider;
int launch_chamfer_sym(const SymPlan &p, const ChamferPair *pairs, float *workspace, const int *need1, const GridArgs *rider,
                       const JacRider *jac, const LossRider *loss, unsigned long long *row64, hipStream_t stream);
int launch_chamfer_sym(const ChamferPair *pairs, int np, int b, int n, int m, float *workspace, hipStream_t stream);

}
```

### geometric_adv_amd/csrc/chamfer_sym.hip

```cpp
#include "common.h"
#include "chamfer_grid.h"
#include "encoder_jac.h"
#include "chamfer_sym.h"
#include "chamfer_mx.h"
#include "loss_cgrad.h"
#include <atomic>
#include <limits.h>
#include <math.h>
#include <stdlib.h>

#pragma clang fp contract(off)

namespace geoadv {

struct ChamferSymArgs {
    ChamferPair pr[2];
    int n, m, clouds, pairs;
    int rw, cw;
    int rtiles;
    int C, S, cslices;
    int pair_base, q_clouds;
    float *rowpart_d;
    int *rowpart_i;
    float *colpart_d;
    int *colpart_i;
    unsigned long long *row64;
    const int *need[2];
    GridRider rider;
    JacRider jac;
    LossRider loss;
};

constexpr int CS_THREADS = 512;
constexpr int CS_WAVES = 8;
constexpr int CS_R = 4;
constexpr int CS_WROWS = kWave * CS_R;
constexpr int CS_CHUNK = 8;
constexpr int CS_ROUND = 16;
constexpr int CS_CMAX = 256;
constexpr int CS_CMIN = 64;
constexpr int CS_MAX_STAGES = 4;
constexpr int CS_TSTRIDE = 68;
constexpr int CS_SEG = CS_WROWS + 4;

__device__ __forceinline__ float sqdist_s(float tx, float ty, float tz, float qx, float qy, float qz) {
    const float dx = tx - qx, dy = ty - qy, dz = tz - qz;
    const float xx = dx * dx, yy = dy * dy, zz = dz * dz;
    return (xx + yy) + zz;
}

constexpr size_t CS_LDS_FLOATS = 3 * CS_CMAX + 4 * CS_WAVES * CS_CMAX + CS_WAVES * CS_ROUND * CS_TSTRIDE;
constexpr size_t CS_LDS_BYTES = sizeof(float) * CS_LDS_FLOATS;
static_assert(3 * CS_WAVES * CS_SEG <= CS_WAVES * CS_ROUND * CS_TSTRIDE, "the staged rows reuse the transpose buffers");

__device__ __forceinline__ int sym_find_half(const float *sx, const float *sy, const float *sz, int q, int h, float qx, float qy, float qz, float v) {
    int found = INT_MAX;
#pragma unroll
    for (int rr = 1; rr >= 0; --rr)
#pragma unroll
        for (int j4 = 3; j4 >= 0; --j4) {
            const int o = 64 * (2 * h + rr) + 16 * q + 4 * j4;
            const float4 xa = *reinterpret_cast<const float4 *>(sx + o);
            const float4 ya = *reinterpret_cast<const float4 *>(sy + o);
            const float4 za = *reinterpret_cast<const float4 *>(sz + o);
            const float d3 = sqdist_s(qx, qy, qz, xa.w, ya.w, za.w), d2 = sqdist_s(qx, qy, qz, xa.z, ya.z, za.z);
            const float d1 = sqdist_s(qx, qy, qz, xa.y, ya.y, za.y), d0 = sqdist_s(qx, qy, qz, xa.x, ya.x, za.x);
            found = d3 == v ? o + 3 : found;
            found = d2 == v ? o + 2 : found;
            found = d1 == v ? o + 1 : found;
            found = d0 == v ? o : found;
        }
    return found;
}

__global__ __launch_bounds__(CS_THREADS, 4) void chamfer_sym_kernel(ChamferSymArgs a) {
    constexpr int R = CS_R;
    extern __shared__ __attribute__((aligned(16))) float stage[];
    if (grid_rider_block<GR_MAX_N>(a.rider)) return;
    if (jac_rider_block(a.jac, stage)) return;
    if (loss_rider_block(a.loss, reinterpret_cast<unsigned *>(stage))) return;
    GA_STAMP(0, 0);
    const int lin = blockIdx.x - a.rider.blocks;
    const int xcd = lin & 7, slot = lin >> 3;
    const int per = a.rtiles * a.cslices;
    const int group = (slot / per) * 8 + xcd, sub = slot % per;
    if (group >= a.clouds * a.pairs) return;
    const int rt = sub % a.rtiles, cs = sub / a.rtiles;
    const int pi = group / a.clouds, c = group % a.clouds;
    if (!sym_needed(a.need[pi], c)) {
        if (a.loss.blocks) loss_rider_arrive(a.loss.done, c);
        return;
    }
    const ChamferPair pr = a.pr[pi];
    const int n = a.n, m = a.m;
    const int cp = a.q_clouds > 0 ? (a.pair_base + c) / a.q_clouds : c;
    const int cq = a.q_clouds > 0 ? (a.pair_base + c) % a.q_clouds : c;
    const float *P = pr.p + (size_t)cp * n * 3;
    const float *Q = pr.q + (size_t)cq * m * 3;

    float *sx = stage, *sy = stage + CS_CMAX, *sz = stage + 2 * CS_CMAX;
    unsigned *colq = reinterpret_cast<unsigned *>(stage + 3 * CS_CMAX);
    float *tbase = stage + 3 * CS_CMAX + 4 * CS_WAVES * CS_CMAX;

    const int lane = threadIdx.x & 63, wave = threadIdx.x >> 6;
    const int rwi = wave % a.rw, cwi = wave / a.rw;
    const int q0 = (rt * a.rw + rwi) * CS_WROWS;
    float px[R], py[R], pz[R], best[R];
    int bestk[R];
#pragma unroll
    for (int r = 0; r < R; ++r) {
        int j = q0 + r * kWave + lane;
        j = j < n ? j : n - 1;
        px[r] = P[3 * j]; py[r] = P[3 * j + 1]; pz[r] = P[3 * j + 2];
        best[r] = INFINITY; bestk[r] = -1;
    }
    float *tb = tbase + wave * (CS_ROUND * CS_TSTRIDE);
    unsigned *cq4 = colq + (size_t)rwi * CS_CMAX * 4;
    float *rx = tbase, *ry = tbase + CS_WAVES * CS_SEG, *rz = tbase + 2 * CS_WAVES * CS_SEG;
    int found[R];
#pragma unroll
    for (int r = 0; r < R; ++r) found[r] = INT_MAX;
    float nx = INFINITY, ny = INFINITY, nz = INFINITY;
    auto request = [&](int st) {
        nx = ny = nz = INFINITY;
        const int k = (cs * a.S + st) * a.C + (int)threadIdx.x;
        if (st < a.S && (int)threadIdx.x < a.C && k < m) { nx = Q[3 * (size_t)k]; ny = Q[3 * (size_t)k + 1]; nz = Q[3 * (size_t)k + 2]; }
    };
    request(0);
    for (int st = 0; st < a.S; ++st) {
        const int cbeg = (cs * a.S + st) * a.C;
        if (cbeg >= m) break;
        const int cnt = min(a.C, m - cbeg);
        const int cntp = (cnt + CS_ROUND - 1) / CS_ROUND * CS_ROUND;
        if ((int)threadIdx.x < cntp) { sx[threadIdx.x] = nx; sy[threadIdx.x] = ny; sz[threadIdx.x] = nz; }
        __syncthreads();
        const int nrounds = cntp / CS_ROUND;
        const int rbeg = nrounds * cwi / a.cw, rend = nrounds * (cwi + 1) / a.cw;
        float prev[R];
#pragma unroll
        for (int r = 0; r < R; ++r) prev[r] = best[r];
        if (st == 0 && rbeg < rend) {
#pragma unroll
            for (int r = 0; r < R; ++r) bestk[r] = rbeg * CS_ROUND;
        }
        for (int rd = rbeg; rd < rend; ++rd) {
            const int k0 = rd * CS_ROUND;
            float colp[CS_ROUND];
#pragma unroll
            for (int hf = 0; hf < CS_ROUND / CS_CHUNK; ++hf) {
                float tx[CS_CHUNK], ty[CS_CHUNK], tz[CS_CHUNK];
#pragma unroll
                for (int v = 0; v < CS_CHUNK / 4; ++v) {
                    const float4 xa = *reinterpret_cast<const float4 *>(&sx[k0 + hf * CS_CHUNK + 4 * v]);
                    const float4 ya = *reinterpret_cast<const float4 *>(&sy[k0 + hf * CS_CHUNK + 4 * v]);
                    const float4 za = *reinterpret_cast<const float4 *>(&sz[k0 + hf * CS_CHUNK + 4 * v]);
                    tx[4 * v] = xa.x; tx[4 * v + 1] = xa.y; tx[4 * v + 2] = xa.z; tx[4 * v + 3] = xa.w;
                    ty[4 * v] = ya.x; ty[4 * v + 1] = ya.y; ty[4 * v + 2] = ya.z; ty[4 * v + 3] = ya.w;
                    tz[4 * v] = za.x; tz[4 * v + 1] = za.y; tz[4 * v + 2] = za.z; tz[4 * v + 3] = za.w;
                }
#pragma unroll
                for (int r = 0; r < R; ++r) {
                    float cm = INFINITY;
#pragma unroll
                    for (int u = 0; u < CS_CHUNK; ++u) {
                        const float d = sqdist_s(tx[u], ty[u], tz[u], px[r], py[r], pz[r]);
                        cm = fminf(cm, d);
                        colp[hf * CS_CHUNK + u] = r == 0 ? d : fminf(colp[hf * CS_CHUNK + u], d);
                    }
                    if (cm < best[r]) { best[r] = cm; bestk[r] = k0 + hf * CS_CHUNK; }
                    __builtin_amdgcn_sched_barrier(0);
                }
            }
#pragma unroll
            for (int u = 0; u < CS_ROUND; ++u) tb[u * CS_TSTRIDE + lane] = colp[u];
            __builtin_amdgcn_wave_barrier();
            {
                const int col = lane >> 2, quarter = lane & 3;
                const uint4 *src = reinterpret_cast<const uint4 *>(tb + col * CS_TSTRIDE + quarter * 16);
                const uint4 v0 = src[0], v1 = src[1], v2 = src[2], v3 = src[3];
                unsigned mb = min(min(min(v0.x, v0.y), min(v0.z, v0.w)), min(min(v1.x, v1.y), min(v1.z, v1.w)));
                mb = min(mb, min(min(min(v2.x, v2.y), min(v2.z, v2.w)), min(min(v3.x, v3.y), min(v3.z, v3.w))));
                cq4[(k0 + col) * 4 + quarter] = mb;
            }
            __builtin_amdgcn_wave_barrier();
        }
        GA_STAMP(0, 1);
#pragma unroll
        for (int r = 0; r < R; ++r) {
            if ((st == 0 && rbeg < rend) || best[r] < prev[r]) {
                const int kb = bestk[r];
                const float4 xa = *reinterpret_cast<const float4 *>(&sx[kb]), xb = *reinterpret_cast<const float4 *>(&sx[kb + 4]);
                const float4 ya = *reinterpret_cast<const float4 *>(&sy[kb]), yb = *reinterpret_cast<const float4 *>(&sy[kb + 4]);
                const float4 za = *reinterpret_cast<const float4 *>(&sz[kb]), zb = *reinterpret_cast<const float4 *>(&sz[kb + 4]);
                const float tx[CS_CHUNK] = {xa.x, xa.y, xa.z, xa.w, xb.x, xb.y, xb.z, xb.w};
                const float ty[CS_CHUNK] = {ya.x, ya.y, ya.z, ya.w, yb.x, yb.y, yb.z, yb.w};
                const float tz[CS_CHUNK] = {za.x, za.y, za.z, za.w, zb.x, zb.y, zb.z, zb.w};
                int f = kb;
#pragma unroll
                for (int u = CS_CHUNK - 1; u >= 0; --u)
                    f = sqdist_s(tx[u], ty[u], tz[u], px[r], py[r], pz[r]) == best[r] ? kb + u : f;
                found[r] = f + cbeg;
            }
        }
        request(st + 1);
        __syncthreads();
        if (cwi == 0) {
#pragma unroll
            for (int r = 0; r < R; ++r) {
                rx[rwi * CS_SEG + r * kWave + lane] = px[r];
                ry[rwi * CS_SEG + r * kWave + lane] = py[r];
                rz[rwi * CS_SEG + r * kWave + lane] = pz[r];
            }
        }
        __syncthreads();
        GA_STAMP(0, 2);
        {
            const int col = threadIdx.x >> 1, h = threadIdx.x & 1;
            const int cc = col < cnt ? col : 0;
            const float4 *cq = reinterpret_cast<const float4 *>(colq);
            float4 cpv[CS_WAVES];
#pragma unroll
            for (int w = 0; w < CS_WAVES; ++w) cpv[w] = cq[(w < a.rw ? w : 0) * CS_CMAX + cc];
            float4 win = cpv[0];
            float v = fminf(fminf(win.x, win.y), fminf(win.z, win.w));
            int bt = 0;
#pragma unroll
            for (int w = 1; w < CS_WAVES; ++w) {
                const float tv = fminf(fminf(cpv[w].x, cpv[w].y), fminf(cpv[w].z, cpv[w].w));
                if (w < a.rw && tv < v) { v = tv; bt = w; win = cpv[w]; }
            }
            const float qx = sx[cc], qy = sy[cc], qz = sz[cc];
            const float *wx = rx + bt * CS_SEG, *wy = ry + bt * CS_SEG, *wz = rz + bt * CS_SEG;
            const float qv[4] = {win.x, win.y, win.z, win.w};
// ... 75 lines not shown
        if (row_atomic) atomicMin(&a.row64[((size_t)pi * a.clouds + c) * n + j], sym_pack(d, i));
        else {
            __builtin_amdgcn_raw_buffer_store_b32(__float_as_uint(d), rd, (unsigned)j * 4u, 0, 0);
            __builtin_amdgcn_raw_buffer_store_b32((unsigned)i, ri, (unsigned)j * 4u, 0, 0);
        }
    };
    auto out_col = [&](int k, float d, int i) {
        asm volatile("" : "+v"(k));
        __builtin_amdgcn_raw_buffer_store_b32(__float_as_uint(d), cd, (unsigned)k * 4u, 0, 0);
        __builtin_amdgcn_raw_buffer_store_b32((unsigned)i, ci, (unsigned)k * 4u, 0, 0);
    };
#ifdef GA_STAMPS
    unsigned long long clk0_, clk1_;
    asm volatile("s_memtime %0\n\ts_waitcnt lgkmcnt(0)" : "=s"(clk0_)::"memory");
#endif
    mx_scan_block<NCT>(v, reinterpret_cast<unsigned *>(stage), out_row, out_col);
#ifdef GA_STAMPS
    asm volatile("s_memtime %0\n\ts_waitcnt lgkmcnt(0)" : "=s"(clk1_)::"memory");
    if (threadIdx.x == 0 && blockIdx.x < GA_STAMP_BLOCKS) ga_stamps[(2 * GA_STAMP_BLOCKS + blockIdx.x) * 8 + 1] = clk1_ - clk0_;
    GA_STAMP(0, 6);
    __syncthreads();
#endif
    GA_STAMP(0, 7);
}

__global__ __launch_bounds__(256) void chamfer_sym_merge_kernel(ChamferSymArgs a) {
    const int group = blockIdx.y;
    const int pi = group / a.clouds, c = group % a.clouds;
    if (!sym_needed(a.need[pi], c)) return;
    const ChamferPair pr = a.pr[pi];
    const int n = a.n, m = a.m, e = blockIdx.x * 256 + threadIdx.x;
    const int rslices = a.cslices * a.cw;
    if (rslices > 1 && e < n) {
        const size_t o = ((size_t)pi * a.clouds + c) * rslices * n + e;
        float d; int i;
        sym_merge_slices(a.rowpart_d + o, a.rowpart_i + o, rslices, n, d, i);
        pr.dist1[(size_t)c * n + e] = d;
        pr.idx1[(size_t)c * n + e] = i;
    }
    if (a.rtiles > 1 && e < m) {
        const size_t o = ((size_t)pi * a.clouds + c) * a.rtiles * m + e;
        float d; int i;
        sym_merge_slices(a.colpart_d + o, a.colpart_i + o, a.rtiles, m, d, i);
        pr.dist2[(size_t)c * m + e] = d;
        pr.idx2[(size_t)c * m + e] = i;
    }
}

static std::atomic<int> g_mx_on{1};
bool chamfer_sym_screen_on() { return g_mx_on.load() != 0; }
static SymShape sym_shape(long groups, int n, int m, bool loop, bool screen) {
    SymShape s;
    s.mx = false;
    if (screen && n > 1024 && (long)cdiv(n, MX_ROWS) * cdiv(m, MX_CMAX) * groups >= (loop ? 4 : 1) * (long)kCUs) {
        s.mx = true; s.rw = MX_WAVES; s.cw = 1;
        s.rtiles = cdiv(n, MX_ROWS);
        s.C = MX_CMAX;
        s.S = 1;
        {
            const int ctiles = cdiv(m, s.C);
            long best = -1;
            for (int S = 1; S <= MX_MAX_STAGES && S <= std::max(1, ctiles); S *= 2) {
                const long wgs = (long)s.rtiles * cdiv(ctiles, S) * groups;
                const long cost = ((wgs + kCUs - 1) / kCUs) * (6 + 18L * S);
                if (best < 0 || cost < best) { best = cost; s.S = S; }
            }
        }
        s.cslices = cdiv(m, s.C * s.S);
        return s;
    }
    s.rw = n > 1024 ? 8 : n > 512 ? 4 : n > 256 ? 2 : 1;
    s.cw = CS_WAVES / s.rw;
    s.rtiles = cdiv(n, CS_WROWS * s.rw);
    const int cmin = std::max(CS_CMIN, 2 * CS_ROUND * s.cw);
    s.C = CS_CMAX;
    while (s.C > cmin && (long)s.rtiles * cdiv(m, s.C) * groups < kCUs &&
           (s.C > 128 || (long)s.rtiles * cdiv(m, s.C / 2) * groups <= kCUs)) s.C /= 2;
    s.S = 1;
    while (s.cw == 1 && s.S < CS_MAX_STAGES && (long)s.rtiles * cdiv(m, s.C * s.S * 2) * groups >= 4 * kCUs) s.S *= 2;
    s.cslices = cdiv(m, s.C * s.S);
    return s;
}
SymPlan chamfer_sym_plan(const SymRequest &r) {
    SymPlan p{};
    p.req = r;
    p.rows = GEOADV_PLAN_ROWS_FINAL;
    if (r.b <= 0 || r.np <= 0) return p;
    const int np_live = r.need1 ? 1 : r.np;
    const SymShape s = p.shape = sym_shape((long)r.b * np_live, r.n, r.m, r.loop, r.screen);
    p.kernel = s.mx ? 8 : 0;
    p.rslices = s.cslices * s.cw;
    p.group_floats = 2 * (size_t)p.rslices * r.n + (s.rtiles > 1 ? 2 * (size_t)s.rtiles * r.m : 0);
    const size_t groups = (size_t)r.np * r.b;
    p.part_off[0] = 0; p.part_off[1] = groups * p.rslices * r.n;
    p.part_off[2] = 2 * groups * p.rslices * r.n; p.part_off[3] = p.part_off[2] + groups * s.rtiles * r.m;
    if (p.rslices == 1 && s.rtiles == 1) p.rows = GEOADV_PLAN_ROWS_FINAL;
    else if (r.defer && r.packed && s.rtiles == 1 && p.rslices >= r.pack_from) p.rows = GEOADV_PLAN_ROWS_PACKED;
    else if (r.defer && s.rtiles == 1 && p.rslices <= 8) p.rows = GEOADV_PLAN_ROWS_PARTIALS;
    else p.rows = GEOADV_PLAN_ROWS_MERGE_LAUNCH;
    p.lds_bytes = s.mx ? MX_LDS_BYTES : CS_LDS_BYTES;
    if (r.search) {
        p.search.count = grid_rider_blocks(r.b);
        p.lds_bytes = std::max(p.lds_bytes, chamfer_grid_lds_bytes(r.n));
    }
    p.scan.first = p.search.count;
    p.scan.count = s.rtiles * s.cslices * 8 * cdiv(r.b * r.np, 8);
    p.grid = (unsigned)(p.search.count + p.scan.count);
    if (r.jac) {
        p.jac.first = (int)p.grid;
        p.jac.count = r.b * (128 / JAC_ROWS);
        p.raise_prio = p.jac.count * 2 <= kCUs ? 1 : 0;
        p.grid += (unsigned)p.jac.count;
        p.lds_bytes = std::max(p.lds_bytes, JAC_LDS_BYTES);
    }
    if (r.loss && !s.mx && s.rtiles == 1 && r.b % 8 == 0 && r.q_clouds == 0 && p.rows != GEOADV_PLAN_ROWS_MERGE_LAUNCH &&
        (r.loss_force || (r.search && (long)s.rtiles * s.cslices * r.b * np_live >= 2 * (long)kCUs))) {
        p.loss.first = (int)p.grid;
        p.loss.count = loss_rider_blocks(r.b, r.loss_rows);
        p.loss_arrivals = (unsigned)(r.np * s.rtiles * s.cslices + (r.search ? 2 * GR_QSPLIT : 0));
        p.grid += (unsigned)p.loss.count;
        p.lds_bytes = std::max(p.lds_bytes, loss_cgrad_lds_bytes(r.n));
    }
    return p;
}

static size_t sym_group_floats(long groups, int n, int m, bool loop) {
    SymRequest plain{1, (int)groups, n, m, loop}, screened = plain;
    plain.screen = false;
    return std::max(chamfer_sym_plan(plain).group_floats, chamfer_sym_plan(screened).group_floats);
}
size_t chamfer_sym_workspace_floats(int pairs, int b, int n, int m) {
    size_t per = 0;
    for (int loop = 0; loop < 2; ++loop) {
        for (long g = 1; g <= (long)pairs * b; g *= 2) per = std::max(per, sym_group_floats(g, n, m, loop != 0));
        per = std::max(per, sym_group_floats((long)pairs * b, n, m, loop != 0));
    }
    return (size_t)pairs * b * per + 64;
}

SymRows chamfer_sym_rows(const SymPlan &p, const float *workspace, const unsigned long long *row64) {
    if (p.rows == GEOADV_PLAN_ROWS_PACKED) return SymRows{nullptr, nullptr, 0, p.req.b, true, row64};
    if (p.rows == GEOADV_PLAN_ROWS_PARTIALS)
        return SymRows{workspace + p.part_off[0], reinterpret_cast<const int *>(workspace + p.part_off[1]), p.rslices, p.req.b, true, nullptr};
    return SymRows{nullptr, nullptr, 1, p.req.b, false, nullptr};
}

int launch_chamfer_sym(const ChamferPair *pairs, int np, int b, int n, int m, float *workspace, hipStream_t stream) {
    SymRequest r{np, b, n, m};
    r.screen = chamfer_sym_screen_on();
    return launch_chamfer_sym(chamfer_sym_plan(r), pairs, workspace, nullptr, nullptr, nullptr, nullptr, nullptr, stream);
}

int launch_chamfer_sym(const SymPlan &p, const ChamferPair *pairs, float *workspace, const int *need1, const GridArgs *rider,
                       const JacRider *jac, const LossRider *loss, unsigned long long *row64, hipStream_t stream) {
    const SymRequest &r = p.req;
    if (p.grid == 0) return GEOADV_OK;
    GA_REQUIRE((need1 != nullptr) == r.need1 && (rider != nullptr) == (p.search.count > 0) && (jac != nullptr) == (p.jac.count > 0) &&
                   (p.loss.count == 0 || loss) && (p.rows != GEOADV_PLAN_ROWS_PACKED || row64),
               "chamfer_sym: the launch's arguments are not the ones its plan was made for");
    const SymShape &s = p.shape;
    ChamferSymArgs a;
    a.need[0] = nullptr; a.need[1] = need1;
    a.pair_base = r.pair_base; a.q_clouds = r.q_clouds;
    for (int i = 0; i < r.np; ++i) a.pr[i] = pairs[i];
    a.n = r.n; a.m = r.m; a.clouds = r.b; a.pairs = r.np;
    a.rw = s.rw; a.cw = s.cw; a.rtiles = s.rtiles; a.C = s.C; a.S = s.S; a.cslices = s.cslices;
    a.rowpart_d = workspace + p.part_off[0];
    a.rowpart_i = reinterpret_cast<int *>(workspace + p.part_off[1]);
    a.colpart_d = workspace + p.part_off[2];
    a.colpart_i = reinterpret_cast<int *>(workspace + p.part_off[3]);
    a.row64 = p.rows == GEOADV_PLAN_ROWS_PACKED ? row64 : nullptr;
    static DeviceOnce attr;
    if (int rc = attr.run([]() -> int {
            const int need = (int)std::max(std::max(std::max(CS_LDS_BYTES, MX_LDS_BYTES), chamfer_grid_lds_bytes(GR_MAX_N)), JAC_LDS_BYTES);
            GA_HIP(hipFuncSetAttribute(reinterpret_cast<const void *>(chamfer_sym_kernel), hipFuncAttributeMaxDynamicSharedMemorySize, need));
            GA_HIP(hipFuncSetAttribute(reinterpret_cast<const void *>(chamfer_mx_kernel<8>), hipFuncAttributeMaxDynamicSharedMemorySize, need));
            return GEOADV_OK;
        })) return rc;
    a.rider.first_block = p.search.first; a.rider.blocks = p.search.count; a.rider.clouds = rider ? r.b : 0;
    a.rider.done = rider && p.loss.count ? loss->done : nullptr;
    if (rider) a.rider.g = *rider;
    if (jac) a.jac = *jac;
    a.jac.first_block = p.jac.first; a.jac.blocks = p.jac.count; a.jac.raise_prio = p.raise_prio;
    if (p.loss.count) a.loss = *loss;
    else a.loss.done = nullptr;
    a.loss.first_block = p.loss.first; a.loss.blocks = p.loss.count; a.loss.clouds = r.b;
    if (p.kernel == 0) chamfer_sym_kernel<<<p.grid, CS_THREADS, p.lds_bytes, stream>>>(a);
    else chamfer_mx_kernel<8><<<p.grid, MX_THREADS, p.lds_bytes, stream>>>(a);
    GA_LAUNCH_CHECK();
    if (p.rows != GEOADV_PLAN_ROWS_MERGE_LAUNCH) return GEOADV_OK;
    chamfer_sym_merge_kernel<<<dim3(cdiv(std::max(r.n, r.m), 256), r.b * r.np), 256, 0, stream>>>(a);
    GA_LAUNCH_CHECK();
    return GEOADV_OK;
}

__global__ __launch_bounds__(256) void chamfer_pair_mean_kernel(int n, int m, const float *d1, const float *d2, float *out) {
    __shared__ float sh[8];
    const int c = blockIdx.x, t = threadIdx.x;
    float s1 = 0.f, s2 = 0.f;
    for (int j = t; j < n; j += 256) s1 += d1[(size_t)c * n + j];
    for (int k = t; k < m; k += 256) s2 += d2[(size_t)c * m + k];
#pragma unroll
    for (int off = 32; off > 0; off >>= 1) { s1 += __shfl_xor(s1, off); s2 += __shfl_xor(s2, off); }
    if ((t & 63) == 0) { sh[t >> 6] = s1; sh[4 + (t >> 6)] = s2; }
    __syncthreads();
    if (t == 0) {
        const float a = ((sh[0] + sh[1]) + sh[2]) + sh[3], b = ((sh[4] + sh[5]) + sh[6]) + sh[7];
        out[c] = a * (1.0f / (float)n) + b * (1.0f / (float)m);
    }
}

}

using namespace geoadv;

static size_t matrix_floats(size_t cnt, int n, int m) {
    return cnt * 2 * ((size_t)n + m) + cnt * sym_group_floats((long)cnt, n, m, false) + 64;
}

extern "C" size_t geoadv_chamfer_matrix_workspace_floats(int na, int nb, int n, int m) {
    if (na <= 0 || nb <= 0 || n <= 0 || m <= 0) return 256;
    const size_t pairs = (size_t)na * nb;
    const size_t chunk = pairs < 8192 ? pairs : 8192;
    return std::max(matrix_floats(chunk, n, m), matrix_floats(1, n, m)) + 256;
}

extern "C" int geoadv_chamfer_matrix(int na, int nb, int n, int m, const float *A, const float *B, float *out,
                                     float *workspace, size_t workspace_floats, void *stream) {
    GA_REQUIRE(na >= 0 && nb >= 0 && n >= 1 && m >= 1, "chamfer_matrix: bad dimensions (na=%d nb=%d n=%d m=%d)", na, nb, n, m);
    if (na == 0 || nb == 0) return GEOADV_OK;
    GA_REQUIRE(A && B && out && workspace, "chamfer_matrix: null pointer");
    GA_REQUIRE(workspace_floats >= matrix_floats(1, n, m) + 256, "chamfer_matrix: workspace too small (%zu floats, need >= %zu)",
               workspace_floats, matrix_floats(1, n, m) + 256);
    const size_t avail = workspace_floats - 256;
    hipStream_t st = as_stream(stream);
    const size_t pairs = (size_t)na * nb;
    for (size_t base = 0; base < pairs;) {
        size_t cnt_ = std::min<size_t>(pairs - base, 32768);
        while (cnt_ > 1 && matrix_floats(cnt_, n, m) > avail) cnt_ = cnt_ * 7 / 8;
        const int cnt = (int)cnt_;
        float *d1 = workspace, *d2 = d1 + (size_t)cnt * n;
        int *i1 = reinterpret_cast<int *>(d2 + (size_t)cnt * m), *i2 = i1 + (size_t)cnt * n;
        float *ws = reinterpret_cast<float *>(i2 + (size_t)cnt * m);
        const ChamferPair pr{A, B, d1, i1, d2, i2};
        GA_REQUIRE(base <= 0x7fffffff, "chamfer_matrix: too many pairs");
        SymRequest rq{1, cnt, n, m};
        rq.q_clouds = nb; rq.pair_base = (int)base; rq.screen = chamfer_sym_screen_on();
        if (int rc = launch_chamfer_sym(chamfer_sym_plan(rq), &pr, ws, nullptr, nullptr, nullptr, nullptr, nullptr, st)) return rc;
        chamfer_pair_mean_kernel<<<cnt, 256, 0, st>>>(n, m, d1, d2, out + base);
        GA_LAUNCH_CHECK();
        base += cnt_;
    }
    return GEOADV_OK;
}

static size_t nn_sym_floats(int b, int n, int m) {
    return (size_t)b * sym_group_floats((long)b, n, m, false) + 64;
}
extern "C" int geoadv_set_chamfer_screen(int on) { return g_mx_on.exchange(on ? 1 : 0); }
extern "C" int geoadv_nn_distance_sym_is_screened(int b, int n, int m) {
    return (b > 0 && n > 0 && m > 0 && sym_shape((long)b, n, m, false, chamfer_sym_screen_on()).mx) ? 1 : 0;
}
extern "C" size_t geoadv_nn_distance_sym_workspace_floats(int b, int n, int m) {
    if (b <= 0 || n <= 0 || m <= 0) return 64;
    return nn_sym_floats(b, n, m);
}
extern "C" int geoadv_nn_distance_sym(int b, int n, const float *xyz1, int m, const float *xyz2, float *dist1, int *idx1,
                                      float *dist2, int *idx2, float *workspace, size_t workspace_floats, void *stream) {
    GA_REQUIRE(b >= 0 && n >= 1 && m >= 1, "nn_distance_sym: bad dimensions (b=%d n=%d m=%d)", b, n, m);
    if (b == 0) return GEOADV_OK;
    GA_REQUIRE(xyz1 && xyz2 && dist1 && idx1 && dist2 && idx2 && workspace, "nn_distance_sym: null pointer");
    GA_REQUIRE(workspace_floats >= nn_sym_floats(b, n, m), "nn_distance_sym: workspace too small (%zu floats, need %zu)",
               workspace_floats, nn_sym_floats(b, n, m));
    const ChamferPair pr{xyz1, xyz2, dist1, idx1, dist2, idx2};
    if (int rc = launch_chamfer_sym(&pr, 1, b, n, m, workspace, as_stream(stream))) return rc;
    return launch_nn_nonfinite_fix(b, n, xyz1, m, xyz2, dist1, idx1, dist2, idx2, as_stream(stream));
}
extern "C" int geoadv_debug_chamfer_sym_plan(const int *q, int *out) {
    GA_REQUIRE(q && out, "debug_chamfer_sym_plan: null argument");
    GA_REQUIRE(q[GEOADV_SYM_REQ_NP] >= 1 && q[GEOADV_SYM_REQ_NP] <= 2 && q[GEOADV_SYM_REQ_B] >= 1 && q[GEOADV_SYM_REQ_N] >= 1 && q[GEOADV_SYM_REQ_M] >= 1,
               "debug_chamfer_sym_plan: bad dimensions");
    SymRequest r{q[GEOADV_SYM_REQ_NP], q[GEOADV_SYM_REQ_B], q[GEOADV_SYM_REQ_N], q[GEOADV_SYM_REQ_M], q[GEOADV_SYM_REQ_LOOP] != 0,
                 q[GEOADV_SYM_REQ_NEED1] != 0, q[GEOADV_SYM_REQ_SEARCH] != 0, q[GEOADV_SYM_REQ_JAC] != 0, q[GEOADV_SYM_REQ_LOSS] != 0,
                 q[GEOADV_SYM_REQ_LOSS_ROWS], q[GEOADV_SYM_REQ_LOSS_FORCE] != 0, q[GEOADV_SYM_REQ_DEFER] != 0, q[GEOADV_SYM_REQ_PACKED] != 0,
                 q[GEOADV_SYM_REQ_PACK_FROM], q[GEOADV_SYM_REQ_Q_CLOUDS], 0, q[GEOADV_SYM_REQ_SCREEN] != 0};
    const SymPlan p = chamfer_sym_plan(r);
    auto clip = [](size_t v) { return (int)std::min<size_t>(v, INT_MAX); };
    const int o[GEOADV_SYM_OUT_COUNT] = {p.shape.mx ? 1 : 0, p.kernel, p.shape.rw, p.shape.cw, p.shape.rtiles, p.shape.C, p.shape.S, p.shape.cslices,
                                         p.rslices, p.rows, p.search.first, p.search.count, p.scan.first, p.scan.count, p.jac.first, p.jac.count,
                                         p.loss.first, p.loss.count, clip(p.grid), clip(p.lds_bytes), (int)p.loss_arrivals, p.raise_prio,
                                         clip(p.group_floats), clip(p.part_off[0]), clip(p.part_off[1]), clip(p.part_off[2]), clip(p.part_off[3])};
    for (int i = 0; i < GEOADV_SYM_OUT_COUNT; ++i) out[i] = o[i];
    return GEOADV_OK;
}
extern "C" size_t geoadv_debug_chamfer_sym_workspace_floats(int pairs, int b, int n, int m) {
    return (pairs <= 0 || b <= 0 || n <= 0 || m <= 0) ? 64 : chamfer_sym_workspace_floats(pairs, b, n, m);
}
GA_STAMPS_GETTER(geoadv_debug_stamps_chamfer_sym)
```

### geometric_adv_amd/ops.py

```python
import ctypes as C

import torch

from . import _abi, _lib
from ._abi import BatchAugment, CloudAugment


def _f32(t, name, rank):
    if not isinstance(t, torch.Tensor):
        raise TypeError("%s must be a torch.Tensor" % name)
    if not t.is_cuda:
        raise ValueError("%s must live on the GPU (got %s); there is no CPU path" % (name, t.device))
    if t.dtype != torch.float32:
        raise ValueError("%s must be float32 (got %s)" % (name, t.dtype))
    if t.dim() != rank:
        raise ValueError("%s must have rank %d (got shape %s)" % (name, rank, tuple(t.shape)))
    return t.contiguous()


def _i32(t, name, shape):
    if not t.is_cuda or t.dtype != torch.int32:
        raise ValueError("%s must be an int32 GPU tensor" % name)
    if tuple(t.shape) != tuple(shape):
        raise ValueError("%s must be of shape %s (got %s)" % (name, tuple(shape), tuple(t.shape)))
    return t.contiguous()


def _xyz_pair(xyz1, xyz2, op):
    xyz1 = _f32(xyz1, "xyz1", 3)
    xyz2 = _f32(xyz2, "xyz2", 3)
    if xyz1.shape[2] != 3:
        raise ValueError("%s only accepts 3d point set xyz1" % op)
    if xyz2.shape[2] != 3:
        raise ValueError("%s only accepts 3d point set xyz2" % op)
    if xyz1.shape[0] != xyz2.shape[0]:
        raise ValueError("%s expects xyz1 and xyz2 have same batch size" % op)
    return xyz1, xyz2


NN_SYM_MIN_PAIRS = 1 << 26


def nn_distance(xyz1, xyz2, kernel="auto"):
    if kernel not in ("auto", "scan", "symmetric"):
        raise ValueError("kernel must be 'auto', 'scan' or 'symmetric'")
    xyz1, xyz2 = _xyz_pair(xyz1, xyz2, "NnDistance")
    b, n, _ = xyz1.shape
    m = xyz2.shape[1]
    if n >= 1 and m >= 1 and b >= 1 and (kernel == "symmetric" or (kernel == "auto" and b * n * m >= NN_SYM_MIN_PAIRS)):
        return nn_distance_sym(xyz1, xyz2)
    dist1 = torch.empty((b, n), dtype=torch.float32, device=xyz1.device)
    idx1 = torch.empty((b, n), dtype=torch.int32, device=xyz1.device)
    dist2 = torch.empty((b, m), dtype=torch.float32, device=xyz1.device)
    idx2 = torch.empty((b, m), dtype=torch.int32, device=xyz1.device)
    with torch.cuda.device(xyz1.device):
        st = _lib.lib().geoadv_nn_distance(b, n, _lib.ptr(xyz1), m, _lib.ptr(xyz2), _lib.ptr(dist1), _lib.ptr(idx1),
                                           _lib.ptr(dist2), _lib.ptr(idx2), _lib.stream_handle())
    _lib.check(st, "nn_distance")
    return dist1, idx1, dist2, idx2


def chamfer_screen(on):
    return bool(_lib.lib().geoadv_set_chamfer_screen(1 if on else 0))


def nn_distance_sym(xyz1, xyz2):
    xyz1, xyz2 = _xyz_pair(xyz1, xyz2, "NnDistance")
    b, n, _ = xyz1.shape
    m = xyz2.shape[1]
    if n < 1 or m < 1:
        raise ValueError("nn_distance_sym needs non-empty clouds")
    dist1 = torch.empty((b, n), dtype=torch.float32, device=xyz1.device)
    idx1 = torch.empty((b, n), dtype=torch.int32, device=xyz1.device)
    dist2 = torch.empty((b, m), dtype=torch.float32, device=xyz1.device)
    idx2 = torch.empty((b, m), dtype=torch.int32, device=xyz1.device)
    wf = int(_lib.lib().geoadv_nn_distance_sym_workspace_floats(b, n, m))
    ws = torch.empty((wf,), dtype=torch.float32, device=xyz1.device)
    with torch.cuda.device(xyz1.device):
        st = _lib.lib().geoadv_nn_distance_sym(b, n, _lib.ptr(xyz1), m, _lib.ptr(xyz2), _lib.ptr(dist1), _lib.ptr(idx1),
                                               _lib.ptr(dist2), _lib.ptr(idx2), _lib.ptr(ws), wf, _lib.stream_handle())
    _lib.check(st, "nn_distance_sym")
    return dist1, idx1, dist2, idx2


def chamfer_per_pc(dist1, dist2):
    dist1, dist2 = _f32(dist1, "dist1", 2), _f32(dist2, "dist2", 2)
    if dist1.shape[0] != dist2.shape[0]:
        raise ValueError("chamfer_per_pc expects dist1 and dist2 have same batch size")
    b, n = dist1.shape
    m = dist2.shape[1]
    out = torch.empty((b,), dtype=torch.float32, device=dist1.device)
    with torch.cuda.device(dist1.device):
        st = _lib.lib().geoadv_chamfer_per_pc(b, n, m, _lib.ptr(dist1), _lib.ptr(dist2), _lib.ptr(out), _lib.stream_handle())
    _lib.check(st, "chamfer_per_pc")
    return out


def nn_distance_paired(xyz1, xyz2):
    xyz1, xyz2 = _xyz_pair(xyz1, xyz2, "NnDistance")
    b, n, _ = xyz1.shape
    if xyz2.shape[1] != n:
        raise ValueError("nn_distance_paired needs clouds of equal size")
    dist1 = torch.empty((b, n), dtype=torch.float32, device=xyz1.device)
    idx1 = torch.empty((b, n), dtype=torch.int32, device=xyz1.device)
    dist2, idx2 = torch.empty_like(dist1), torch.empty_like(idx1)
    with torch.cuda.device(xyz1.device):
        st = _lib.lib().geoadv_nn_distance_paired(b, n, _lib.ptr(xyz1), _lib.ptr(xyz2), _lib.ptr(dist1), _lib.ptr(idx1),
                                                  _lib.ptr(dist2), _lib.ptr(idx2), _lib.stream_handle())
    _lib.check(st, "nn_distance_paired")
    return dist1, idx1, dist2, idx2


def nn_distance_grad(xyz1, xyz2, grad_dist1, idx1, grad_dist2, idx2):
    xyz1, xyz2 = _xyz_pair(xyz1, xyz2, "NnDistanceGrad")
    b, n, _ = xyz1.shape
    m = xyz2.shape[1]
    grad_dist1 = _f32(grad_dist1, "grad_dist1", 2)
    grad_dist2 = _f32(grad_dist2, "grad_dist2", 2)
    if tuple(grad_dist1.shape) != (b, n):
        raise ValueError("NnDistanceGrad requires grad_dist1 be of shape(batch,#points)")
    if tuple(grad_dist2.shape) != (b, m):
        raise ValueError("NnDistanceGrad requires grad_dist2 be of shape(batch,#points)")
    idx1 = _i32(idx1, "idx1", (b, n))
    idx2 = _i32(idx2, "idx2", (b, m))
    g1 = torch.empty_like(xyz1)
    g2 = torch.empty_like(xyz2)
    with torch.cuda.device(xyz1.device):
        st = _lib.lib().geoadv_nn_distance_grad(b, n, _lib.ptr(xyz1), m, _lib.ptr(xyz2), _lib.ptr(grad_dist1),
                                                _lib.ptr(idx1), _lib.ptr(grad_dist2), _lib.ptr(idx2), _lib.ptr(g1),
                                                _lib.ptr(g2), _lib.stream_handle())
    _lib.check(st, "nn_distance_grad")
    return g1, g2


class _NnDistanceFn(torch.autograd.Function):

    @staticmethod
    def forward(ctx, xyz1, xyz2):
        d1, i1, d2, i2 = nn_distance(xyz1, xyz2)
        ctx.save_for_backward(xyz1, xyz2, i1, i2)
        ctx.mark_non_differentiable(i1, i2)
        return d1, i1, d2, i2

    @staticmethod
    def backward(ctx, gd1, _gi1, gd2, _gi2):
        xyz1, xyz2, i1, i2 = ctx.saved_tensors
        g1, g2 = nn_distance_grad(xyz1, xyz2, gd1.contiguous(), i1, gd2.contiguous(), i2)
        return g1, g2


def nn_distance_autograd(xyz1, xyz2):
    return _NnDistanceFn.apply(xyz1, xyz2)


def _call(name, *args):
    st = getattr(_lib.lib(), name)(*args, _lib.stream_handle())
    _lib.check(st, name.replace("geoadv_", ""))


def query_ball_point(radius, nsample, xyz1, xyz2):
    xyz1, xyz2 = _xyz_pair(xyz1, xyz2, "QueryBallPoint")
    b, n, _ = xyz1.shape
    m = xyz2.shape[1]
    idx = torch.zeros((b, m, int(nsample)), dtype=torch.int32, device=xyz1.device)
    cnt = torch.zeros((b, m), dtype=torch.int32, device=xyz1.device)
    with torch.cuda.device(xyz1.device):
        _call("geoadv_query_ball_point", b, n, m, float(radius), int(nsample), _lib.ptr(xyz1), _lib.ptr(xyz2),
              _lib.ptr(idx), _lib.ptr(cnt))
    return idx, cnt


def select_top_k(k, dist):
    dist = _f32(dist, "dist", 3)
    b, m, n = dist.shape
    outi = torch.empty((b, m, n), dtype=torch.int32, device=dist.device)
    out = torch.empty_like(dist)
    with torch.cuda.device(dist.device):
        _call("geoadv_selection_sort", b, n, m, int(k), _lib.ptr(dist), _lib.ptr(outi), _lib.ptr(out))
    return outi, out


def group_point(points, idx):
    points = _f32(points, "points", 3)
    b, n, c = points.shape
    if idx.dim() != 3 or idx.shape[0] != b:
        raise ValueError("GroupPoint expects idx of shape (batch, npoint, nsample)")
    idx = _i32(idx, "idx", idx.shape)
    m, ns = idx.shape[1], idx.shape[2]
    out = torch.empty((b, m, ns, c), dtype=torch.float32, device=points.device)
    with torch.cuda.device(points.device):
        _call("geoadv_group_point", b, n, c, m, ns, _lib.ptr(points), _lib.ptr(idx), _lib.ptr(out))
    return out


def group_point_grad(points, idx, grad_out):
    points = _f32(points, "points", 3)
    b, n, c = points.shape
    idx = _i32(idx, "idx", idx.shape)
    m, ns = idx.shape[1], idx.shape[2]
    grad_out = _f32(grad_out, "grad_out", 4)
    if tuple(grad_out.shape) != (b, m, ns, c):
        raise ValueError("GroupPointGrad expects grad_out of shape (batch, npoint, nsample, channel)")
    gp = torch.empty_like(points)
    with torch.cuda.device(points.device):
        wb = int(_lib.lib().geoadv_group_point_grad_workspace_bytes(b, n, c, m, ns))
        ws = torch.empty(wb, dtype=torch.uint8, device=points.device)
        _call("geoadv_group_point_grad_ws", b, n, c, m, ns, _lib.ptr(grad_out), _lib.ptr(idx), _lib.ptr(gp), _lib.ptr(ws), wb)
    return gp


KNN_KERNELS = {"auto": _abi.GEOADV_KNN_AUTO, "all_points": _abi.GEOADV_KNN_ALL_POINTS, "grid": _abi.GEOADV_KNN_GRID,
               "grid_shells": _abi.GEOADV_KNN_GRID_SHELLS}
_knn_default = "auto"


def _knn_kernel(kernel):
    k = _knn_default if kernel is None else kernel
    if k not in KNN_KERNELS:
        raise ValueError("kernel must be one of %s" % sorted(KNN_KERNELS))
    return KNN_KERNELS[k]


def knn_point(k, xyz1, xyz2, kernel=None):
    xyz1, xyz2 = _xyz_pair(xyz1, xyz2, "knn_point")
    b, n, _ = xyz1.shape
    m = xyz2.shape[1]
    val = torch.empty((b, m, int(k)), dtype=torch.float32, device=xyz1.device)
    idx = torch.empty((b, m, int(k)), dtype=torch.int32, device=xyz1.device)
    with torch.cuda.device(xyz1.device):
        wb = int(_lib.lib().geoadv_knn_workspace_bytes(b, n, m, int(k)))
        ws = torch.empty(wb, dtype=torch.uint8, device=xyz1.device)
        _call("geoadv_knn_point_ws", _knn_kernel(kernel), b, n, m, int(k), _lib.ptr(xyz1), _lib.ptr(xyz2), _lib.ptr(val), _lib.ptr(idx),
              _lib.ptr(ws), wb)
    return val, idx

# ... 551 lines not shown
```

### include/geoadv.h

```cpp
#ifndef GEOADV_H
#define GEOADV_H

#include <stddef.h>

#ifdef __cplusplus
extern "C" {
#endif

#define GEOADV_OK      0
#define GEOADV_EINVAL  1
#define GEOADV_EHIP    2
#define GEOADV_ENOMEM  3
#define GEOADV_ERANGE  4

int         geoadv_version(void);
const char *geoadv_last_error(void);


int geoadv_nn_distance(int b, int n, const float *xyz1, int m, const float *xyz2,
                       float *dist1, int *idx1, float *dist2, int *idx2, void *stream);

size_t geoadv_nn_distance_sym_workspace_floats(int b, int n, int m);
int geoadv_nn_distance_sym_is_screened(int b, int n, int m);
int geoadv_set_chamfer_screen(int on);
int geoadv_nn_distance_sym(int b, int n, const float *xyz1, int m, const float *xyz2,
                           float *dist1, int *idx1, float *dist2, int *idx2,
                           float *workspace, size_t workspace_floats, void *stream);

int geoadv_chamfer_per_pc(int b, int n, int m, const float *dist1, const float *dist2, float *out, void *stream);

int geoadv_nn_distance_paired(int b, int n, const float *xyz1, const float *xyz2,
                              float *dist1, int *idx1, float *dist2, int *idx2, void *stream);

int geoadv_nn_distance_grad(int b, int n, const float *xyz1, int m, const float *xyz2,
                            const float *grad_dist1, const int *idx1,
                            const float *grad_dist2, const int *idx2,
                            float *grad_xyz1, float *grad_xyz2, void *stream);

size_t geoadv_chamfer_matrix_workspace_floats(int na, int nb, int n, int m);
int geoadv_chamfer_matrix(int na, int nb, int n, int m, const float *A, const float *B, float *out,
                          float *workspace, size_t workspace_floats, void *stream);

size_t geoadv_approx_match_temp_floats(int b, int n, int m);
int geoadv_approx_match(int b, int n, int m, const float *xyz1, const float *xyz2,
                        float *match, float *temp, void *stream);
#define GEOADV_EMD_FAST 0
#define GEOADV_EMD_REFERENCE 1
#define GEOADV_EMD_DENSE_LEVELS 0x100
int geoadv_approx_match_mode(int mode, int b, int n, int m, const float *xyz1, const float *xyz2,
                             float *match, float *temp, void *stream);
int geoadv_emd_sparse_levels(int on);
int geoadv_match_cost(int b, int n, int m, const float *xyz1, const float *xyz2,
                      const float *match, float *out, void *stream);
size_t geoadv_match_cost_workspace_floats(int b, int n, int m);
int geoadv_match_cost_ws(int b, int n, int m, const float *xyz1, const float *xyz2, const float *match, float *out,
                         float *workspace, size_t workspace_floats, void *stream);
size_t geoadv_emd_cost_grad1_temp_floats(int b, int n, int m);
int geoadv_emd_cost_grad1(int b, int n, int m, const float *xyz1, const float *xyz2, float *cost, float *grad1,
                          float *temp, void *stream);
int geoadv_emd_cost_grad1_mode(int mode, int b, int n, int m, const float *xyz1, const float *xyz2, float *cost,
                               float *grad1, float *temp, void *stream);
int geoadv_match_cost_grad(int b, int n, int m, const float *xyz1, const float *xyz2,
                           const float *match, float *grad1, float *grad2, void *stream);


int geoadv_query_ball_point(int b, int n, int m, float radius, int nsample,
                            const float *xyz1, const float *xyz2, int *idx, int *pts_cnt, void *stream);
int geoadv_selection_sort(int b, int n, int m, int k, const float *dist, int *outi, float *out, void *stream);
int geoadv_group_point(int b, int n, int c, int m, int nsample, const float *points, const int *idx,
                       float *out, void *stream);
int geoadv_group_point_grad(int b, int n, int c, int m, int nsample, const float *grad_out, const int *idx,
                            float *grad_points, void *stream);
size_t geoadv_group_point_grad_workspace_bytes(int b, int n, int c, int m, int nsample);
int geoadv_group_point_grad_ws(int b, int n, int c, int m, int nsample, const float *grad_out, const int *idx,
                               float *grad_points, void *workspace, size_t workspace_bytes, void *stream);
int geoadv_knn_point(int b, int n, int m, int k, const float *xyz1, const float *xyz2,
                     float *val, int *idx, void *stream);
int geoadv_knn_dists(int b, int n, int k, const float *pc, float *out, void *stream);
#define GEOADV_KNN_AUTO        0
#define GEOADV_KNN_ALL_POINTS  1
#define GEOADV_KNN_GRID        2
#define GEOADV_KNN_GRID_SHELLS 3
size_t geoadv_knn_workspace_bytes(int b, int n, int m, int k);
int geoadv_knn_point_ws(int kernel, int b, int n, int m, int k, const float *xyz1, const float *xyz2,
                        float *val, int *idx, void *workspace, size_t workspace_bytes, void *stream);
int geoadv_knn_dists_ws(int kernel, int b, int n, int k, const float *pc, float *out,
                        void *workspace, size_t workspace_bytes, void *stream);
int geoadv_knn_grid_mode(int mode);

#define GEOADV_FPS_AUTO      0
#define GEOADV_FPS_WORKGROUP 1
#define GEOADV_FPS_WAVE      2
int geoadv_farthest_point_sample(int b, int n, const float *xyz , int m,
                                 const int *start , int form, int *idx ,
                                 float *sampled , float *mindist , void *stream);
int geoadv_farthest_point_sample_plan(int n, int form, int *form_out, int *waves, int *points_per_thread);

int geoadv_outlier_filter(int b, int n, const float *pc, const float *knn_dists, int knn_stride, int top_k, float thresh,
                          float *outlier_pc, short *outlier_idx, short *outlier_num, float *inlier_pc, void *stream);

int geoadv_sor_filter(int b, int n, const float *pc , const float *knn_dists , int knn_stride,
                      int k, double alpha, float *outlier_pc, short *outlier_idx, short *outlier_num, float *inlier_pc,
                      double *stats , void *stream);

int geoadv_random_drop(int b, int n, const float *pc , int drop, unsigned long long seed, unsigned long long counter,
                       unsigned long long slot_offset, float *kept_pc , int *dropped_idx ,
                       void *stream);

#define GEOADV_KNN_LOSS_SURFACE 0x100
size_t geoadv_knn_outlier_loss_workspace_bytes(int b, int n, int k);
int geoadv_knn_outlier_loss(int kernel , int b, int n, int k, double alpha,
                            const float *xyz , double *loss , float *grad ,
                            double *score , unsigned char *mask ,
                            int *idx , double *stats ,
                            void *workspace, size_t workspace_bytes, void *stream);
int geoadv_debug_knn_outlier_loss_launch(int b, int n, int k, double alpha, const float *xyz, double *loss, float *grad ,
                                         void *workspace, size_t workspace_bytes, void *stream);

int geoadv_critical_split(int b, int n, int c, const float *pc, const float *max_val, const int *max_idx,
                          float *critical_points, short *critical_idx, short *critical_num, float *critical_pc,
                          float *non_critical_pc, void *stream);

int geoadv_sort_axes(int b, int n, const float *pc, float *out, int *axes_idx , int neg_rot,
                     void *stream);

typedef struct geoadv_batch_augment {
    unsigned long long seed, counter;
    int   slot_offset;
    float noise_mu, noise_sigma;
    float noise_clip;
    int   rot_count;
    int   rotate_first;
} geoadv_batch_augment;
int geoadv_batch_gather(int b, int n, const float *data, long long num_clouds, const int *index ,
                        const geoadv_batch_augment *aug , const double *rot ,
                        float *clean , float *feed , void *stream);

#define GEOADV_NORMALIZE_IDENTITY 0
#define GEOADV_NORMALIZE_UNIT_BALL 1
#define GEOADV_NORMALIZE_BOUNDING_BOX 2
int geoadv_normalize_clouds(int b, int n, int kind, const float *pc, float *out, void *stream);

#define GEOADV_AUGMENT_RECORD 45
typedef struct geoadv_cloud_augment {
    unsigned long long seed, counter;
    int   slot_offset;
    int   sample;
    int   rot_axes;
    float range_rot;
    int   rot_3d;
    int   scale;
    float scale_min, scale_max;
    int   flip_axes;
    int   translate;
    float translate_scale;
} geoadv_cloud_augment;
int geoadv_augment_batch(int b, int n_out, const float *data, long long num_clouds, int n_src,
                         const int *index , const geoadv_cloud_augment *cfg ,
                         const float *params , float *params_out ,
                         float *out , void *stream);

int geoadv_latent_dist_matrix(int na, int nb, int d, const float *a, const float *b, float *out, void *stream);

typedef struct geoadv_ae geoadv_ae;

#define GEOADV_ENC_LAYERS 5
#define GEOADV_DEC_LAYERS 3

typedef struct geoadv_ae_weights {
    int n_points;
    int enc_dims[GEOADV_ENC_LAYERS + 1];
    int dec_dims[GEOADV_DEC_LAYERS + 1];
    const float *enc_w[GEOADV_ENC_LAYERS], *enc_b[GEOADV_ENC_LAYERS];
    const float *bn_gamma[GEOADV_ENC_LAYERS], *bn_beta[GEOADV_ENC_LAYERS];
    const float *bn_mean[GEOADV_ENC_LAYERS], *bn_var[GEOADV_ENC_LAYERS];
    const float *dec_w[GEOADV_DEC_LAYERS], *dec_b[GEOADV_DEC_LAYERS];
} geoadv_ae_weights;

int  geoadv_ae_create(geoadv_ae **out, const geoadv_ae_weights *host_weights);
void geoadv_ae_destroy(geoadv_ae *ae);
// ... 109 lines not shown
    int points_per_primitive;
    int dim_template;
    int bottleneck_size;
    int hidden_neurons;
    int num_layers;
    int activation;
    int decoder_bn;
} geoadv_atlas_config;
typedef struct geoadv_atlas_weights {
    const float *enc_w[GEOADV_ATLAS_ENC_LAYERS], *enc_b[GEOADV_ATLAS_ENC_LAYERS];
    const float *enc_gamma[GEOADV_ATLAS_ENC_LAYERS], *enc_beta[GEOADV_ATLAS_ENC_LAYERS];
    const float *enc_mean[GEOADV_ATLAS_ENC_LAYERS], *enc_var[GEOADV_ATLAS_ENC_LAYERS];
    const float *dec_w[GEOADV_ATLAS_MAX_DEC_LAYERS], *dec_b[GEOADV_ATLAS_MAX_DEC_LAYERS];
    const float *dec_gamma[GEOADV_ATLAS_MAX_DEC_LAYERS], *dec_beta[GEOADV_ATLAS_MAX_DEC_LAYERS];
    const float *dec_mean[GEOADV_ATLAS_MAX_DEC_LAYERS], *dec_var[GEOADV_ATLAS_MAX_DEC_LAYERS];
} geoadv_atlas_weights;

int  geoadv_atlas_create(geoadv_atlas **out, const geoadv_atlas_config *config, const geoadv_atlas_weights *host_weights,
                         const float *host_template);
void geoadv_atlas_destroy(geoadv_atlas *atlas);
size_t geoadv_atlas_workspace_bytes(const geoadv_atlas *atlas, int b, int n);
int geoadv_atlas_forward(const geoadv_atlas *atlas, int b, int n, const float *pc, float *latent, float *recon,
                         void *workspace, void *stream);

typedef struct geoadv_fold geoadv_fold;

#define GEOADV_FOLD_ENC_LAYERS  7
#define GEOADV_FOLD_DEC_LAYERS  6
#define GEOADV_FOLD_PICKS_GIVEN  0
#define GEOADV_FOLD_PICKS_DEVICE 1
typedef struct geoadv_fold_weights {
    const float *enc_w[GEOADV_FOLD_ENC_LAYERS], *enc_b[GEOADV_FOLD_ENC_LAYERS];
    const float *enc_gamma[GEOADV_FOLD_ENC_LAYERS], *enc_beta[GEOADV_FOLD_ENC_LAYERS];
    const float *enc_mean[GEOADV_FOLD_ENC_LAYERS], *enc_var[GEOADV_FOLD_ENC_LAYERS];
    const float *dec_w[GEOADV_FOLD_DEC_LAYERS], *dec_b[GEOADV_FOLD_DEC_LAYERS];
} geoadv_fold_weights;

int  geoadv_fold_create(geoadv_fold **out, const geoadv_fold_weights *host_weights);
void geoadv_fold_destroy(geoadv_fold *fold);
size_t geoadv_fold_workspace_bytes(const geoadv_fold *fold, int b, int n);
int geoadv_fold_graph(const geoadv_fold *fold, int b, int n, const float *pc, int *degree, int *knn, float *cov,
                      void *workspace, void *stream);
int geoadv_fold_forward(const geoadv_fold *fold, int b, int n, const float *pc, int sampling, unsigned long long seed,
                        long long cloud_offset, int *picks, int *cols, float *code, float *p1, float *recon,
                        void *workspace, void *stream);

typedef struct geoadv_fold_trainer geoadv_fold_trainer;
typedef struct geoadv_fold_train_config {
    int   batch;
    int   n_points;
    float learning_rate;
    float weight_decay;
    long long seed;
    long long initial_step;
    long long initial_ordinal;
} geoadv_fold_train_config;
int  geoadv_fold_trainer_create(geoadv_fold_trainer **out, const geoadv_fold_weights *init, const geoadv_fold_train_config *cfg);
void geoadv_fold_trainer_destroy(geoadv_fold_trainer *t);
int  geoadv_fold_trainer_set_slots(geoadv_fold_trainer *t, const float *slot1, const float *slot2);
int geoadv_fold_trainer_step(geoadv_fold_trainer *t, const float *x, int sampling, int *picks, float *loss, float *mid_loss,
                             void *stream);
int geoadv_fold_trainer_buffers(geoadv_fold_trainer *t, float **params, float **grads, size_t *count);
int geoadv_fold_trainer_layout(const geoadv_fold_trainer *t, size_t *offsets52, size_t *moving_offsets13);
int geoadv_fold_trainer_counters(const geoadv_fold_trainer *t, long long *step, long long *ordinal);
#define GEOADV_FOLD_STATE_BN_MEAN       0
#define GEOADV_FOLD_STATE_BN_VAR        1
#define GEOADV_FOLD_STATE_RUNNING_MEAN  2
#define GEOADV_FOLD_STATE_RUNNING_VAR   3
#define GEOADV_FOLD_STATE_BN_INV        4
#define GEOADV_FOLD_STATE_BN_SHIFT      5
#define GEOADV_FOLD_STATE_PRE_BN        6
#define GEOADV_FOLD_STATE_POOL_WINNER   7
#define GEOADV_FOLD_STATE_GMAX_ROW      8
#define GEOADV_FOLD_STATE_HIDDEN        9
#define GEOADV_FOLD_STATE_PICKS        10
#define GEOADV_FOLD_STATE_COLS         11
#define GEOADV_FOLD_STATE_COV          12
#define GEOADV_FOLD_STATE_CODE         13
#define GEOADV_FOLD_STATE_MID          14
#define GEOADV_FOLD_STATE_RECON        15
#define GEOADV_FOLD_STATE_CHAMFER_IDX  16
#define GEOADV_FOLD_STATE_SLOT1        17
#define GEOADV_FOLD_STATE_SLOT2        18
int geoadv_fold_trainer_state(const geoadv_fold_trainer *t, int what, int layer, const void **ptr, size_t *count);

int geoadv_fold_train_pool(int b, int n, int c, const float *h, const int *cols, float *g, int *win, void *stream);
int geoadv_fold_train_pool_grad(int b, int n, int c, const float *dg, const int *win, const int *off, const int *deg, const int *col,
                                float *dh, void *stream);
int geoadv_fold_train_gmax(int b, int n, int c, const float *a, const float *inv, const float *shift, float *pooled, int *arg,
                           void *stream);

typedef struct geoadv_atlas_trainer geoadv_atlas_trainer;
typedef struct geoadv_atlas_train_config {
    int   batch;
    int   n_points;
    int   points_per_primitive;
    float learning_rate;
    long long seed;
    long long initial_step;
    long long initial_tracked;
} geoadv_atlas_train_config;
int  geoadv_atlas_trainer_create(geoadv_atlas_trainer **out, const geoadv_atlas_config *config, const geoadv_atlas_weights *init,
                                 const geoadv_atlas_train_config *cfg);
void geoadv_atlas_trainer_destroy(geoadv_atlas_trainer *t);
int  geoadv_atlas_trainer_set_slots(geoadv_atlas_trainer *t, const float *slot1, const float *slot2);
int  geoadv_atlas_trainer_set_learning_rate(geoadv_atlas_trainer *t, float learning_rate, int reset_optimizer);
int geoadv_atlas_trainer_step(geoadv_atlas_trainer *t, const float *x, int given_template, float *template_points, float *loss,
                              void *stream);
int geoadv_atlas_trainer_buffers(geoadv_atlas_trainer *t, float **params, float **grads, size_t *count);
int geoadv_atlas_trainer_layout(const geoadv_atlas_trainer *t, size_t *offsets48, size_t *moving_offsets12);
int geoadv_atlas_trainer_counters(const geoadv_atlas_trainer *t, long long *step, long long *tracked);
#define GEOADV_ATLAS_STATE_BN_MEAN       0
#define GEOADV_ATLAS_STATE_BN_VAR        1
#define GEOADV_ATLAS_STATE_RUNNING_MEAN  2
#define GEOADV_ATLAS_STATE_RUNNING_VAR   3
#define GEOADV_ATLAS_STATE_BN_INV        4
#define GEOADV_ATLAS_STATE_BN_SHIFT      5
#define GEOADV_ATLAS_STATE_PRE_BN        6
#define GEOADV_ATLAS_STATE_GMAX_ROW      7
#define GEOADV_ATLAS_STATE_TEMPLATE      8
#define GEOADV_ATLAS_STATE_LATENT        9
#define GEOADV_ATLAS_STATE_RECON        10
#define GEOADV_ATLAS_STATE_CHAMFER_IDX  11
#define GEOADV_ATLAS_STATE_SLOT1        12
#define GEOADV_ATLAS_STATE_SLOT2        13
int geoadv_atlas_trainer_state(const geoadv_atlas_trainer *t, int what, int layer, const void **ptr, size_t *count);

size_t geoadv_train_gemm_partial_floats(void);
int geoadv_train_gemm(int kernel, const float *A, long long sAi, long long sAk, long long sAz, const float *B, long long sBk,
                      long long sBj, long long sBz, float *C, long long ldc, long long sCz, const float *bias, long long sBiasZ,
                      int M, int N, int K, int batch, float *partials, size_t partial_floats, int *ksplit_out, void *stream);

typedef struct geoadv_attack geoadv_attack;

#define GEOADV_LOSS_ADV_CHAMFER 0
#define GEOADV_LOSS_ADV_LATENT  1
#define GEOADV_LOSS_DIST_CHAMFER 0
#define GEOADV_LOSS_DIST_PERT    1

typedef struct geoadv_attack_config {
    int   batch;
    int   loss_adv_type;
    int   loss_dist_type;
    float max_point_pert_weight;
    float max_point_dist_weight;
    float learning_rate;
    float emd_weight;
    int   all_pairs_source_dist;
    int   emd_weight_mode;
    int   recompute_backward;
    int   encoder_backward;
    int   separate_adam;
    int   chamfer_kernel;
    int    knn_rule;
    float  knn_thresh;
    float  knn_weight;
    int    knn_k;
    float  knn_alpha;
    int   loss_in_scan;
} geoadv_attack_config;
#define GEOADV_SMALL_BATCH_POINTS 10240
#define GEOADV_SYM_MIN_POINTS      4096
#define GEOADV_ENC_BWD_AUTO      0
#define GEOADV_ENC_BWD_MASKED    1
#define GEOADV_ENC_BWD_JACOBIAN  2
#define GEOADV_CHAMFER_AUTO      0
#define GEOADV_CHAMFER_TWO_SCAN  1
#define GEOADV_CHAMFER_SYMMETRIC 2

int  geoadv_attack_create(geoadv_attack **out, const geoadv_ae *ae, const geoadv_attack_config *cfg);
void geoadv_attack_destroy(geoadv_attack *at);

int geoadv_attack_set_inputs(geoadv_attack *at, const float *source_pc, const float *target_pc,
                             const float *target_latent, const float *dist_weight, void *stream);
int geoadv_attack_init_pert(geoadv_attack *at, const float *init_pert, int reset_optimizer, void *stream);

int geoadv_attack_run(geoadv_attack *at, int first_iteration, int iterations, int thresh,
                      float *metrics_hist, void *stream);

int geoadv_attack_get_best(geoadv_attack *at, const float *target_ae_loss_ref,
                           float *metrics, float *adv, float *recon, void *stream);

int geoadv_attack_set_source_search(geoadv_attack *at, int on);

int geoadv_attack_status(geoadv_attack *at, void *stream);

int geoadv_attack_peek(geoadv_attack *at, float *pert, float *adv, float *recon, float *latent,
                       float *grad, int *idx_r1, int *idx_r2, int *idx_a1, int *idx_a2, void *stream);

int geoadv_attack_test_loss_form(geoadv_attack *at, int form);
int geoadv_attack_test_loss_state(geoadv_attack *at, float *g_recon, float *g_dist, float *losses, float *dist_r1, float *dist_a1,
                                  void *stream);
enum {
    GEOADV_PLAN_SYMMETRIC = 0,
    GEOADV_PLAN_SCREENED = 1,
    GEOADV_PLAN_RTILES = 2,
    GEOADV_PLAN_RSLICES = 3,
    GEOADV_PLAN_ROWS = 4,
    GEOADV_PLAN_LOSS = 5,
    GEOADV_PLAN_GRAD = 6,
    GEOADV_PLAN_H = 7,
    GEOADV_PLAN_RANGE = 8,
    GEOADV_PLAN_COUNT = 9
};
enum { GEOADV_PLAN_ROWS_FINAL = 0, GEOADV_PLAN_ROWS_PARTIALS = 1, GEOADV_PLAN_ROWS_PACKED = 2, GEOADV_PLAN_ROWS_MERGE_LAUNCH = 3 };
enum { GEOADV_PLAN_LOSS_METRICS = 0, GEOADV_PLAN_LOSS_FUSED = 1, GEOADV_PLAN_LOSS_RIDERS = 2 };
enum { GEOADV_PLAN_GRAD_NONE = 0, GEOADV_PLAN_GRAD_FUSED_1PASS = 1, GEOADV_PLAN_GRAD_FUSED_GENERAL = 2, GEOADV_PLAN_GRAD_STEP_FX_1PASS = 3,
       GEOADV_PLAN_GRAD_STEP_FX_GENERAL = 4, GEOADV_PLAN_GRAD_STEP_SORTED = 5 };
int geoadv_attack_test_plan(geoadv_attack *at, int plan[GEOADV_PLAN_COUNT], int *jstar, void *stream);
enum { GEOADV_SYM_REQ_NP = 0, GEOADV_SYM_REQ_B, GEOADV_SYM_REQ_N, GEOADV_SYM_REQ_M, GEOADV_SYM_REQ_LOOP, GEOADV_SYM_REQ_NEED1,
       GEOADV_SYM_REQ_SEARCH, GEOADV_SYM_REQ_JAC, GEOADV_SYM_REQ_LOSS, GEOADV_SYM_REQ_LOSS_ROWS, GEOADV_SYM_REQ_LOSS_FORCE,
       GEOADV_SYM_REQ_DEFER, GEOADV_SYM_REQ_PACKED, GEOADV_SYM_REQ_PACK_FROM, GEOADV_SYM_REQ_Q_CLOUDS, GEOADV_SYM_REQ_SCREEN,
       GEOADV_SYM_REQ_COUNT };
enum { GEOADV_SYM_OUT_SCREENED = 0, GEOADV_SYM_OUT_KERNEL, GEOADV_SYM_OUT_RW, GEOADV_SYM_OUT_CW, GEOADV_SYM_OUT_RTILES, GEOADV_SYM_OUT_C,
       GEOADV_SYM_OUT_S, GEOADV_SYM_OUT_CSLICES, GEOADV_SYM_OUT_RSLICES, GEOADV_SYM_OUT_ROWS, GEOADV_SYM_OUT_SEARCH_FIRST,
       GEOADV_SYM_OUT_SEARCH_BLOCKS, GEOADV_SYM_OUT_SCAN_FIRST, GEOADV_SYM_OUT_SCAN_BLOCKS, GEOADV_SYM_OUT_JAC_FIRST, GEOADV_SYM_OUT_JAC_BLOCKS,
       GEOADV_SYM_OUT_LOSS_FIRST, GEOADV_SYM_OUT_LOSS_BLOCKS, GEOADV_SYM_OUT_GRID, GEOADV_SYM_OUT_LDS_BYTES, GEOADV_SYM_OUT_LOSS_ARRIVALS,
       GEOADV_SYM_OUT_RAISE_PRIO, GEOADV_SYM_OUT_GROUP_FLOATS, GEOADV_SYM_OUT_ROWPART_D, GEOADV_SYM_OUT_ROWPART_I, GEOADV_SYM_OUT_COLPART_D,
       GEOADV_SYM_OUT_COLPART_I, GEOADV_SYM_OUT_COUNT };
int geoadv_debug_chamfer_sym_plan(const int *request, int *out);
size_t geoadv_debug_chamfer_sym_workspace_floats(int pairs, int b, int n, int m);
int geoadv_debug_h2_split(const float *in, int n, unsigned *w0, unsigned *w1, unsigned *w1_ref, void *stream);
#define GEOADV_EMD_SPARSE_LEVELS 3
int geoadv_debug_emd_sparse_state(int fused, int b, int n, int m, const float *temp, int *out, void *stream);

int geoadv_attack_search_state(geoadv_attack *at, int *searched, int *handed_back, void *stream);

typedef struct geoadv_trainer geoadv_trainer;
typedef struct geoadv_train_config {
    int   batch;
    float learning_rate;
    float bn_decay;
    int   loss;
    int   max_workgroups;
} geoadv_train_config;
#define GEOADV_TRAIN_LOSS_CHAMFER 0
#define GEOADV_TRAIN_LOSS_EMD     1

int  geoadv_trainer_create(geoadv_trainer **out, const geoadv_ae_weights *init, const geoadv_train_config *cfg);
void geoadv_trainer_destroy(geoadv_trainer *t);
int geoadv_trainer_step(geoadv_trainer *t, const float *x, const float *gt, float *loss, float *recon, void *stream);
int geoadv_trainer_forward_backward(geoadv_trainer *t, const float *x, const float *gt, float *loss, float *recon, void *stream);
int geoadv_trainer_apply(geoadv_trainer *t, float grad_scale, void *stream);
int geoadv_trainer_set_world(geoadv_trainer *t, int world);
int geoadv_trainer_num_phases(void);
int geoadv_trainer_run_phase(geoadv_trainer *t, int phase, const float *x, const float *gt, void *stream);
int geoadv_trainer_exchange(geoadv_trainer *t, int phase, double **buf, size_t *count);
int geoadv_trainer_fetch(geoadv_trainer *t, float *loss, float *recon, void *stream);
int geoadv_trainer_buffers(geoadv_trainer *t, float **params, float **grads, size_t *count);
int geoadv_trainer_layout(const geoadv_trainer *t, size_t *offsets26);
#define GEOADV_TRAIN_STATE_ACT         0
#define GEOADV_TRAIN_STATE_BN_MEAN     1
#define GEOADV_TRAIN_STATE_BN_INV_STD  2
#define GEOADV_TRAIN_STATE_BN_SCALE    3
#define GEOADV_TRAIN_STATE_BN_SHIFT    4
#define GEOADV_TRAIN_STATE_IDX1        5
#define GEOADV_TRAIN_STATE_IDX2        6
#define GEOADV_TRAIN_STATE_POOL_MAX    7
#define GEOADV_TRAIN_STATE_POOL_TIES   8
#define GEOADV_TRAIN_STATE_DEC1        9
#define GEOADV_TRAIN_STATE_DEC2        10
int geoadv_trainer_state(const geoadv_trainer *t, int what, int layer, const void **ptr, size_t *count);
int geoadv_trainer_export(geoadv_trainer *t, const geoadv_ae_weights *dst, void *stream);

#define GEOADV_PROF_ENCODER_FWD 0
#define GEOADV_PROF_DECODER_FWD 1
#define GEOADV_PROF_CHAMFER_FWD 2
#define GEOADV_PROF_LOSS_GRAD   3
#define GEOADV_PROF_DECODER_BWD 4
#define GEOADV_PROF_ENCODER_BWD 5
#define GEOADV_PROF_ADAM        6
#define GEOADV_PROF_COUNT       7
int geoadv_attack_profile(geoadv_attack *at, int enable);
int geoadv_attack_profile_read(geoadv_attack *at, int which, int *launches, float *total_ms);
int geoadv_attack_markers(geoadv_attack *at, int enable);
int geoadv_attack_profile_stride(geoadv_attack *at, int stride);

#ifdef __cplusplus
}
#endif
#endif
```

Measured before the change: 9504 attack-iterations/sec.

## Add Verlet-style candidate lists for reconstruction Chamfer with adaptive fallback

Adds per-point neighbour candidate lists built at periodic anchor iterations with a skin radius. On the iterations between anchors, the recon-to-target nearest-neighbour queries are answered from these lists and ride inside the symmetric chamfer kernel, so rows certified by the lists skip the full scan. A pinned host hint counter and a Python-side check turn the lists off when too many queries are refused or handed back. The cost is extra list-build kernels, workspace, warmup logic and the risk of wrong minima if the certification logic is wrong.

```diff
diff --git a/geometric_adv_amd/_abi.py b/geometric_adv_amd/_abi.py
--- a/geometric_adv_amd/_abi.py
+++ b/geometric_adv_amd/_abi.py
@@ -11,6 +11,8 @@
     "geoadv_nn_distance_sym_is_screened": "i:iii",
     "geoadv_set_chamfer_screen": "i:i",
     "geoadv_nn_distance_sym": "i:iipippppppzp",
+    "geoadv_nn_distance_lists_workspace_bytes": "z:iiii",
+    "geoadv_nn_distance_lists": "i:iiipppppippppppppzp",
     "geoadv_chamfer_per_pc": "i:iiipppp",
     "geoadv_nn_distance_paired": "i:iippppppp",
     "geoadv_nn_distance_grad": "i:iipipppppppp",
@@ -128,6 +130,8 @@
     "geoadv_debug_h2_split": "i:pipppp",
     "geoadv_debug_emd_sparse_state": "i:iiiippp",
     "geoadv_attack_search_state": "i:pppp",
+    "geoadv_attack_set_recon_lists": "i:pi",
+    "geoadv_attack_list_state": "i:ppp",
     "geoadv_trainer_create": "i:ppp",
     "geoadv_trainer_destroy": "v:p",
     "geoadv_trainer_step": "i:pppppp",
@@ -185,6 +189,10 @@
 GEOADV_LOSS_DIST_CHAMFER, GEOADV_LOSS_DIST_PERT = 0, 1
 GEOADV_ENC_BWD_AUTO, GEOADV_ENC_BWD_MASKED, GEOADV_ENC_BWD_JACOBIAN = 0, 1, 2
 GEOADV_CHAMFER_AUTO, GEOADV_CHAMFER_TWO_SCAN, GEOADV_CHAMFER_SYMMETRIC = 0, 1, 2
+GEOADV_RECON_LISTS_ADAPTIVE, GEOADV_RECON_LISTS_OFF, GEOADV_RECON_LISTS_PINNED = 0, 1, 2
+(GEOADV_LIST_STATE_ON, GEOADV_LIST_STATE_ANCHORS, GEOADV_LIST_STATE_LIST_ITERATIONS, GEOADV_LIST_STATE_CERTIFIED,
+ GEOADV_LIST_STATE_REFUSED, GEOADV_LIST_STATE_UNLISTED, GEOADV_LIST_STATE_HANDED_BACK, GEOADV_LIST_STATE_FLAGGED,
+ GEOADV_LIST_STATE_PERIOD, GEOADV_LIST_STATE_COUNT) = range(10)
 GEOADV_PLAN_COUNT = 9
 GEOADV_TRAIN_LOSS_CHAMFER, GEOADV_TRAIN_LOSS_EMD = 0, 1
 (GEOADV_TRAIN_STATE_ACT, GEOADV_TRAIN_STATE_BN_MEAN, GEOADV_TRAIN_STATE_BN_INV_STD, GEOADV_TRAIN_STATE_BN_SCALE,
@@ -256,7 +264,7 @@
                 ("max_point_pert_weight", C.c_float), ("max_point_dist_weight", C.c_float),
                 ("learning_rate", C.c_float), ("emd_weight", C.c_float), ("all_pairs_source_dist", C.c_int),
                 ("emd_weight_mode", C.c_int), ("recompute_backward", C.c_int), ("encoder_backward", C.c_int),
-                ("separate_adam", C.c_int), ("chamfer_kernel", C.c_int),
+                ("separate_adam", C.c_int), ("chamfer_kernel", C.c_int), ("recon_lists", C.c_int),
                 ("knn_rule", C.c_int), ("knn_thresh", C.c_float),
                 ("knn_weight", C.c_float), ("knn_k", C.c_int), ("knn_alpha", C.c_float), ("loss_in_scan", C.c_int)]
 
diff --git a/geometric_adv_amd/adv_ae.py b/geometric_adv_amd/adv_ae.py
--- a/geometric_adv_amd/adv_ae.py
+++ b/geometric_adv_amd/adv_ae.py
@@ -19,7 +19,7 @@
                  learning_rate=0.01, ae_name="autoencoder", emd_weight=0.0, verbose=False, batch_slots=1,
                  chamfer_prune=True, emd_reference_weights=False, recompute_backward=False, separate_adam=False,
                  chamfer_kernel="auto", encoder_backward="auto", emd_dense_levels=False, encoder_arith=None, loss_in_scan=True,
-                 knn_weight=0.0, knn_k=5, knn_alpha=1.05, knn_rule="sor", knn_thresh=0.04):
+                 knn_weight=0.0, knn_k=5, knn_alpha=1.05, knn_rule="sor", knn_thresh=0.04, recon_lists=True):
         self.batch_size = int(batch_size)
         self.n_input = [int(n_points), 3]
         self.n_output = [int(n_points), 3]
@@ -54,6 +54,9 @@
         self.encoder_backward = encoder_backward
         if loss_in_scan not in (True, False, "always"):
             raise ValueError("loss_in_scan must be True (where it pays), False or 'always'")
+        if recon_lists not in (True, False, "pinned"):
+            raise ValueError("recon_lists must be True (adaptive), False or 'pinned'")
+        self.recon_lists = recon_lists
         self.loss_in_scan = loss_in_scan
         self.knn_weight, self.knn_k, self.knn_alpha = float(knn_weight), int(knn_k), float(knn_alpha)
         self.knn_rule, self.knn_thresh = knn_rule, float(knn_thresh)
@@ -82,6 +85,8 @@
 
 
 CHAMFER_KERNELS = {"auto": _abi.GEOADV_CHAMFER_AUTO, "two_scan": _abi.GEOADV_CHAMFER_TWO_SCAN, "symmetric": _abi.GEOADV_CHAMFER_SYMMETRIC}
+RECON_LISTS = {True: _abi.GEOADV_RECON_LISTS_ADAPTIVE, False: _abi.GEOADV_RECON_LISTS_OFF, "pinned": _abi.GEOADV_RECON_LISTS_PINNED}
+LIST_STATE_NAMES = ["on", "anchors", "list_iterations", "certified", "refused", "unlisted", "handed_back", "flagged", "period"]
 ENCODER_BACKWARDS = {"auto": _abi.GEOADV_ENC_BWD_AUTO, "masked": _abi.GEOADV_ENC_BWD_MASKED, "jacobian": _abi.GEOADV_ENC_BWD_JACOBIAN}
 KNN_TERM_MAX_K, KNN_TERM_MAX_POINTS, KNN_TERM_MAX_BATCH = 15, 16384, 65535
 KNN_RULES = {"sor": 0, "surface": 1}
@@ -114,6 +119,7 @@
                             1 if getattr(c, "recompute_backward", False) else 0, ENCODER_BACKWARDS[getattr(c, "encoder_backward", "auto")],
                             1 if getattr(c, "separate_adam", False) else 0,
                             CHAMFER_KERNELS[getattr(c, "chamfer_kernel", "auto")],
+                            RECON_LISTS[getattr(c, "recon_lists", True)],
                             KNN_RULES[getattr(c, "knn_rule", "sor")] if getattr(c, "knn_weight", 0.0) != 0.0 else 0,
                             float(getattr(c, "knn_thresh", 0.04)),
                             float(getattr(c, "knn_weight", 0.0)), int(getattr(c, "knn_k", 5)), float(getattr(c, "knn_alpha", 1.05)),
@@ -196,6 +202,32 @@
         if 2 * handed_back > self.B:
             self.set_source_search(False)
         return handed_back
+
+    def list_state(self):
+        st = (C.c_longlong * _abi.GEOADV_LIST_STATE_COUNT)()
+        with torch.cuda.device(self.device):
+            _lib.check(_lib.lib().geoadv_attack_list_state(self._h, st, _lib.stream_handle()), "attack_list_state")
+        out = {k: int(st[i]) for i, k in enumerate(LIST_STATE_NAMES)}
+        out["on"] = bool(out["on"])
+        return out
+
+    def set_recon_lists(self, on, period=None):
+        _lib.check(_lib.lib().geoadv_attack_set_recon_lists(self._h, (int(period) if period else 1) if on else 0), "attack_set_recon_lists")
+
+    def adapt_recon_lists(self):
+        if getattr(self.configuration, "recon_lists", True) is not True:
+            return None
+        s = self.list_state()
+        last = getattr(self, "_lists_seen", None) or {k: 0 for k in s}
+        self._lists_seen = s
+        if not s["on"]:
+            return None
+        d = {k: s[k] - last[k] for k in ("list_iterations", "certified", "refused", "unlisted", "handed_back")}
+        cloud_iters = d["list_iterations"] * self.B
+        queries = d["certified"] + d["refused"] + d["unlisted"]
+        if cloud_iters and (4 * d["handed_back"] > cloud_iters or 4 * (d["refused"] + d["unlisted"]) > max(queries, 1)):
+            self.set_recon_lists(False)
+        return d
 
     def status(self):
         with torch.cuda.device(self.device):
@@ -345,6 +377,7 @@
             m_, a_, r_ = self.get_best(target_ae_loss_ref)
             self.status()
             self.adapt_source_search()
+            self.adapt_recon_lists()
             h = hist.cpu().numpy()
             self.last_history.append(h)
             step = (c.num_iterations // 10) or 1
diff --git a/geometric_adv_amd/csrc/attack.hip b/geometric_adv_amd/csrc/attack.hip
--- a/geometric_adv_amd/csrc/attack.hip
+++ b/geometric_adv_amd/csrc/attack.hip
@@ -2,6 +2,7 @@
 #include "chamfer_sym.h"
 #include "chamfer_grad.h"
 #include "chamfer_grid.h"
+#include "chamfer_lists.h"
 #include "encoder_jac.h"
 #include "decoder_tail.h"
 #include "knn_loss.h"
@@ -182,6 +183,14 @@
     bool host_loss;
     int cus;
     bool chamfer_sym;
+    ReconLists lists;
+    bool lists_on;
+    int list_age;
+    int list_period;
+    int list_warm_left;
+    unsigned long long n_anchors, n_list_iters;
+    unsigned long long *list_hint;
+    unsigned long long hint_seen[5];
     float beta1_pow, beta2_pow;
     bool fwd_valid;
     bool adv_valid;
@@ -261,6 +270,25 @@
 
 
 bool cgrad_step_sorted(int n) { return n > CG_FX_MAX_N_PLANE; }
+
+constexpr float RL_SKIN_FIRST = 0.010f, RL_SKIN_FACTOR = 1.4f, RL_SKIN_MIN = 0.002f, RL_SKIN_MAX = 0.016f;
+constexpr int RL_PERIOD = 16, RL_CAPACITY = 16;
+constexpr int RL_WARM_FORWARDS = 48;
+
+void lists_adapt_from_hint(geoadv_attack *at) {
+    unsigned long long h[5];
+    h[4] = reinterpret_cast<volatile unsigned long long *>(at->list_hint)[4];
+    if (h[4] == at->hint_seen[4]) return;
+    for (int k = 0; k < 4; ++k) h[k] = reinterpret_cast<volatile unsigned long long *>(at->list_hint)[k];
+    if (reinterpret_cast<volatile unsigned long long *>(at->list_hint)[4] != h[4]) return;
+    if (at->hint_seen[4] >= 1) {
+        const unsigned long long periods = h[4] - at->hint_seen[4];
+        const unsigned long long handed = h[3] - at->hint_seen[3], refused = (h[1] - at->hint_seen[1]) + (h[2] - at->hint_seen[2]);
+        const unsigned long long cloud_iters = periods * (unsigned long long)(at->list_period - 1) * at->B;
+        if (4 * handed > cloud_iters || 4 * refused > cloud_iters * 2ull * at->n) at->lists_on = false;
+    }
+    for (int k = 0; k < 5; ++k) at->hint_seen[k] = h[k];
+}
 
 struct ForwardForm { bool pruned, rides_scan, rides_latent, loss_fused, merge_in_loss, jac_rides; };
 
@@ -288,6 +316,13 @@
     }
     const SymRows rows = chamfer_sym_rows(plan, at->sym_ws, at->row64);
     const bool packed = plan.rows == GEOADV_PLAN_ROWS_PACKED, hosted = plan.loss.count > 0;
+    const bool listed = at->lists.list_row && at->lists_on && adv_chamfer && at->chamfer_sym && packed && plan.shape.rtiles == 1 && !at->emd_temp && f.pruned;
+    if (listed && at->list_hint && at->cfg.recon_lists == GEOADV_RECON_LISTS_ADAPTIVE) lists_adapt_from_hint(at);
+    bool warm = false;
+    if (listed && at->lists_on && at->list_warm_left > 0) { at->list_warm_left--; warm = true; }
+    const bool list_iter = listed && !warm && at->lists_on && at->list_age >= 0 && at->list_age + 1 < at->list_period;
+    const bool list_anchor = listed && !warm && at->lists_on && !list_iter;
+    if (!listed || warm || !at->lists_on) at->list_age = -1;
     const int call = at->grid_calls;
     int *need_new = at->need_adv[f.rides_scan ? (call + 1) & 1 : 0];
     const int *need_scan = at->need_adv[f.rides_scan ? call & 1 : 0];
@@ -365,8 +400,29 @@
                 at->loss_target += plan.loss_arrivals;
                 lr = LossRider{la, ca, H, 1 + 2 * H, 0, 0, B, at->loss_done, at->loss_target, reinterpret_cast<int *>(at->tail_ready + B)};
             }
+            const int *need0 = nullptr;
+            ListRider list_rider;
+            bool rides = false;
+            if (list_iter) {
+                ListQuery lq{};
+                lq.P = at->recon; lq.Q = at->gt; lq.row64 = at->row64; lq.dist2 = at->r2; lq.idx2 = at->ir2;
+                lq.call = at->list_age; lq.answer_all = false;
+                rides = !hosted && plan.kernel == 0;
+                if (rides) list_rider = recon_lists_rider(at->lists, lq, 512);
+                else if (int rc = launch_recon_lists_query(at->lists, lq, st)) return rc;
+                need0 = at->lists.need[at->list_age & 1];
+                at->list_age++; at->n_list_iters++;
+            }
             if (int rc = launch_chamfer_sym(plan, pairs, at->sym_ws, f.pruned ? need_scan : nullptr, f.rides_scan ? &rider : nullptr,
-                                            f.jac_rides ? &jr : nullptr, hosted ? &lr : nullptr, at->row64, st)) return rc;
+                                            f.jac_rides ? &jr : nullptr, hosted ? &lr : nullptr, at->row64, st, need0, rides ? &list_rider : nullptr)) return rc;
+            if (list_anchor) {
+                ListBuild lb{};
+                lb.P = at->recon; lb.Q = at->gt; lb.row64 = at->row64; lb.dist2 = at->r2;
+                lb.first = RL_SKIN_FIRST; lb.factor = RL_SKIN_FACTOR; lb.lo = RL_SKIN_MIN; lb.hi = RL_SKIN_MAX;
+                lb.hint = at->list_hint; lb.serial = ++at->n_anchors;
+                if (int rc = launch_recon_lists_build(at->lists, lb, st)) return rc;
+                at->list_age = 0;
+            }
         } else {
             ChamferScan all[4] = {{at->recon, at->gt, at->r1, at->ir1, n, n}, {at->gt, at->recon, at->r2, at->ir2, n, n},
                                   {at->adv, at->x, at->a1, at->ia1, n, n}, {at->x, at->adv, at->a2, at->ia2, n, n}};
@@ -400,6 +456,13 @@
         pl[GEOADV_PLAN_H] = fx ? H : 0; pl[GEOADV_PLAN_RANGE] = fx ? cgrad_fx_range(n) : 0;
     }
     at->fwd_valid = true;
+    return GEOADV_OK;
+}
+
+int lists_invalidate(geoadv_attack *at, hipStream_t st) {
+    at->list_age = -1;
+    at->list_warm_left = at->cfg.recon_lists == GEOADV_RECON_LISTS_ADAPTIVE ? RL_WARM_FORWARDS : 0;
+    if (at->lists.list_row) GA_HIP(hipMemsetAsync(at->lists.dmax, 0, sizeof(float) * (size_t)at->B, st));
     return GEOADV_OK;
 }
 
@@ -530,6 +593,13 @@
         at->emd_temp = F(geoadv_emd_cost_grad1_temp_floats(at->B, at->n, at->n) + 2);
         at->emd_cost = F(B); at->emd_g1 = F(bn3);
     }
+    at->lists = ReconLists{};
+    if (cfg.recon_lists != GEOADV_RECON_LISTS_OFF && cfg.loss_adv_type == GEOADV_LOSS_ADV_CHAMFER && cfg.emd_weight == 0.f && at->n <= RL_MAX_POINTS) {
+        ReconLists measure;
+        const size_t lb = carve_recon_lists(measure, nullptr, at->B, at->n, at->n, RL_CAPACITY, true);
+        char *p = c.take<char>(lb);
+        if (base) carve_recon_lists(at->lists, p, at->B, at->n, at->n, RL_CAPACITY, true);
+    }
     at->knn_ws = nullptr; at->knn_ws_bytes = 0; at->knn_loss = nullptr;
     if (cfg.knn_weight != 0.f) {
         at->knn_ws_bytes = geoadv_knn_outlier_loss_workspace_bytes(at->B, at->n, cfg.knn_k);
@@ -569,6 +639,8 @@
                "attack_create: unknown encoder_backward %d", cfg->encoder_backward);
     GA_REQUIRE(cfg->chamfer_kernel >= GEOADV_CHAMFER_AUTO && cfg->chamfer_kernel <= GEOADV_CHAMFER_SYMMETRIC,
                "attack_create: unknown chamfer_kernel %d", cfg->chamfer_kernel);
+    GA_REQUIRE(cfg->recon_lists >= GEOADV_RECON_LISTS_ADAPTIVE && cfg->recon_lists <= GEOADV_RECON_LISTS_PINNED,
+               "attack_create: unknown recon_lists %d", cfg->recon_lists);
     GA_REQUIRE(cfg->emd_weight == 0.f || cfg->loss_adv_type == GEOADV_LOSS_ADV_CHAMFER,
                "attack_create: emd_weight needs the output-space attack (loss_adv_type chamfer)");
     if (cfg->knn_weight != 0.f) {
@@ -604,6 +676,15 @@
     const size_t carved = carve_arena(at, at->arena);
     assert(carved == at->arena_bytes); (void)carved;
     at->need_last = at->need_adv[0];
+    at->lists_on = at->lists.list_row != nullptr; at->list_age = -1; at->list_period = RL_PERIOD;
+    at->n_anchors = at->n_list_iters = 0; at->list_hint = nullptr;
+    at->list_warm_left = cfg->recon_lists == GEOADV_RECON_LISTS_ADAPTIVE ? RL_WARM_FORWARDS : 0;
+    for (auto &v : at->hint_seen) v = 0;
+    if (at->lists_on && cfg->recon_lists == GEOADV_RECON_LISTS_ADAPTIVE) {
+        if (hipHostMalloc(reinterpret_cast<void **>(&at->list_hint), sizeof(unsigned long long) * 5, hipHostMallocDefault) == hipSuccess)
+            for (int k = 0; k < 5; ++k) at->list_hint[k] = 0;
+        else { at->list_hint = nullptr; (void)hipGetLastError(); }
+    }
     at->jac_valid = false;
     at->tail_epoch = 0; at->loss_target = 0; at->grid_calls = 0;
     {
@@ -658,6 +739,7 @@
     if (!at) return;
     if (at->counted) at->ae->attack_refs.fetch_sub(1);
     for (auto e : at->ev) (void)hipEventDestroy(e);
+    if (at->list_hint) (void)hipHostFree(at->list_hint);
     (void)hipFree(at->arena);
     delete at;
 }
@@ -679,6 +761,8 @@
     for (int i = 0; i < 2; ++i)
         GA_HIP(hipMemsetAsync(at->need_adv[i], 0, sizeof(int) * 8 * (size_t)at->B, st));
     GA_HIP(hipMemsetAsync(at->tail_ready + at->B, 0, sizeof(unsigned), st));
+    if (int rc = lists_invalidate(at, st)) return rc;
+    if (at->lists.list_row && at->cfg.recon_lists == GEOADV_RECON_LISTS_ADAPTIVE) at->lists_on = true;
     at->fwd_valid = false; at->adv_valid = false;
     return GEOADV_OK;
 }
@@ -700,6 +784,7 @@
     GA_HIP(hipMemsetAsync(at->best_metrics, 0, 4 * (size_t)at->B * 4, st));
     GA_HIP(hipMemsetAsync(at->best_adv, 0, 4 * bn3, st));
     GA_HIP(hipMemsetAsync(at->best_recon, 0, 4 * bn3, st));
+    if (int rc = lists_invalidate(at, st)) return rc;
     at->fwd_valid = false; at->adv_valid = false;
     return GEOADV_OK;
 }
@@ -741,6 +826,41 @@
 extern "C" int geoadv_attack_set_source_search(geoadv_attack *at, int on) {
     GA_REQUIRE(at, "attack_set_source_search: null handle");
     at->chamfer_prune = on != 0;
+    return GEOADV_OK;
+}
+
+extern "C" int geoadv_attack_set_recon_lists(geoadv_attack *at, int on) {
+    GA_REQUIRE(at, "attack_set_recon_lists: null handle");
+    GA_REQUIRE(on >= 0 && on <= 256, "attack_set_recon_lists: on=%d must be 0, 1 or a period of 2 ... 256 forwards", on);
+    at->lists_on = on != 0 && at->lists.list_row != nullptr;
+    if (on >= 2) at->list_period = on;
+    if (!at->lists_on || on >= 2) at->list_age = -1;
+    return GEOADV_OK;
+}
+
+extern "C" int geoadv_attack_list_state(geoadv_attack *at, long long state[GEOADV_LIST_STATE_COUNT], void *stream) {
+    GA_REQUIRE(at && state, "attack_list_state: null argument");
+    for (int i = 0; i < GEOADV_LIST_STATE_COUNT; ++i) state[i] = 0;
+    state[GEOADV_LIST_STATE_ON] = at->lists_on ? 1 : 0;
+    state[GEOADV_LIST_STATE_ANCHORS] = (long long)at->n_anchors;
+    state[GEOADV_LIST_STATE_LIST_ITERATIONS] = (long long)at->n_list_iters;
+    state[GEOADV_LIST_STATE_PERIOD] = at->list_period;
+    if (!at->lists.list_row) return GEOADV_OK;
+    hipStream_t st = as_stream(stream);
+    unsigned long long h[4];
+    std::vector<int> need(8 * (size_t)at->B);
+    const int *cur = at->lists.need[(at->list_age < 0 ? 0 : at->list_age) & 1];
+    GA_HIP(hipMemcpyAsync(h, at->lists.stats, sizeof(h), hipMemcpyDeviceToHost, st));
+    GA_HIP(hipMemcpyAsync(need.data(), cur, sizeof(int) * need.size(), hipMemcpyDeviceToHost, st));
+    GA_HIP(hipStreamSynchronize(st));
+    state[GEOADV_LIST_STATE_CERTIFIED] = (long long)h[0]; state[GEOADV_LIST_STATE_REFUSED] = (long long)h[1];
+    state[GEOADV_LIST_STATE_UNLISTED] = (long long)h[2]; state[GEOADV_LIST_STATE_HANDED_BACK] = (long long)h[3];
+    if (at->list_age >= 0)
+        for (int c = 0; c < at->B; ++c) {
+            int any = 0;
+            for (int k = 0; k < 8; ++k) any |= need[8 * (size_t)c + k];
+            state[GEOADV_LIST_STATE_FLAGGED] += any ? 1 : 0;
+        }
     return GEOADV_OK;
 }
 
diff --git a/geometric_adv_amd/csrc/chamfer_lists.h b/geometric_adv_amd/csrc/chamfer_lists.h
--- /dev/null
+++ b/geometric_adv_amd/csrc/chamfer_lists.h
@@ -0,0 +1,205 @@
+#pragma once
+#include "common.h"
+#include "chamfer_sym.h"
+
+namespace geoadv {
+
+constexpr int RL_CAP_MAX = 32;
+constexpr int RL_MAX_POINTS = 2048;
+constexpr int RL_THREADS = 256;
+
+struct ReconLists {
+    int b, n, m, cap;
+    float *anchor;
+    float *tau_row, *tau_col;
+    int *need[2];
+    unsigned *cnt_row, *cnt_col;
+    unsigned short *list_row;
+    unsigned short *list_col;
+    float *dmax;
+    float *skin;
+    unsigned long long *stats;
+    void *clear; size_t clear_bytes;
+};
+size_t carve_recon_lists(ReconLists &L, void *base, int b, int n, int m, int cap, bool own_anchor);
+
+struct ListBuild {
+    const float *P, *Q;
+    const float *dist1;
+    const unsigned long long *row64;
+    const float *dist2;
+    const float *skin;
+    float first, factor, lo, hi;
+    unsigned long long *hint;
+    unsigned long long serial;
+};
+int launch_recon_lists_build(const ReconLists &L, const ListBuild &in, hipStream_t st);
+
+struct ListQuery {
+    const float *P, *Q;
+    float *dist1; int *idx1;
+    unsigned long long *row64;
+    float *dist2; int *idx2;
+    int call;
+    bool answer_all;
+};
+int launch_recon_lists_query(const ReconLists &L, const ListQuery &q, hipStream_t st);
+
+struct ListQueryArgs { ReconLists L; ListQuery q; const int *need_prev; int *need_next; };
+struct ListRider { ListQueryArgs a; int first_block, blocks, per_cloud; };
+ListRider recon_lists_rider(const ReconLists &L, const ListQuery &q, int threads);
+
+#ifdef __HIPCC__
+__device__ __forceinline__ float rl_sqdist(float tx, float ty, float tz, float qx, float qy, float qz) {
+    const float dx = tx - qx, dy = ty - qy, dz = tz - qz;
+    const float xx = dx * dx, yy = dy * dy, zz = dz * dz;
+    return (xx + yy) + zz;
+}
+__device__ __forceinline__ float rl_sqrt(float v) { return __builtin_amdgcn_sqrtf(v); }
+__device__ __forceinline__ float rl_tau(float dmin, float skin) {
+    const float t = rl_sqrt(dmin) + skin;
+    return t * t;
+}
+constexpr float RL_MARGIN = 0x1p-18f;
+constexpr float RL_TAU_MIN = 0x1p-80f;
+
+
+template <int THREADS>
+__device__ __forceinline__ void recon_lists_query_block(const ListQueryArgs &a, int blk, int c, unsigned *lds) {
+    constexpr int RL_THREADS = THREADS;
+    unsigned *red = lds, &qn = lds[8], &unl = lds[9];
+    int *queue = reinterpret_cast<int *>(lds + 16);
+    const ReconLists &L = a.L;
+    const int n = L.n, m = L.m, cap = L.cap, t = threadIdx.x, lane = t & 63, wave = t >> 6;
+    if (!a.q.answer_all && sym_needed(a.need_prev, c)) {
+        if (t == 0) {
+            a.need_next[8 * c + (blk & 7)] = 1;
+            if (blk == 0) {
+                atomicAdd(&L.stats[3], 1ull);
+                L.dmax[c] = INFINITY;
+            }
+        }
+        return;
+    }
+    const int rblocks = (n + RL_THREADS - 1) / RL_THREADS;
+    const bool is_row = blk < rblocks;
+    const int N = is_row ? n : m, M = is_row ? m : n;
+    const int q = (is_row ? blk : blk - rblocks) * RL_THREADS + t;
+    const bool valid = q < N;
+    const float *P = a.q.P + (size_t)c * n * 3, *Q = a.q.Q + (size_t)c * m * 3, *A = L.anchor + (size_t)c * n * 3;
+    const float *own = is_row ? P : Q, *oth = is_row ? Q : P;
+    if (t == 0) { qn = 0; unl = 0; }
+    float move = 0.f;
+    if (is_row) {
+        if (valid) move = rl_sqrt(rl_sqdist(P[3 * q], P[3 * q + 1], P[3 * q + 2], A[3 * q], A[3 * q + 1], A[3 * q + 2]));
+    } else {
+        unsigned mx = 0;
+        for (int j0 = t; j0 < n; j0 += 8 * RL_THREADS) {
+            float v[8][6];
+#pragma unroll
+            for (int u = 0; u < 8; ++u) {
+                const int j = min(j0 + u * RL_THREADS, n - 1);
+#pragma unroll
+                for (int e = 0; e < 3; ++e) { v[u][e] = P[3 * j + e]; v[u][3 + e] = A[3 * j + e]; }
+            }
+#pragma unroll
+            for (int u = 0; u < 8; ++u) mx = max(mx, __float_as_uint(rl_sqdist(v[u][0], v[u][1], v[u][2], v[u][3], v[u][4], v[u][5])));
+        }
+#pragma unroll
+        for (int off = 32; off > 0; off >>= 1) mx = max(mx, (unsigned)__shfl_xor((int)mx, off));
+        if (lane == 0) red[wave] = mx;
+    }
+    __syncthreads();
+    if (!is_row) {
+        unsigned mx = red[0];
+#pragma unroll
+        for (int w = 1; w < RL_THREADS / 64; ++w) mx = max(mx, red[w]);
+        move = rl_sqrt(__uint_as_float(mx));
+        if (blk == rblocks && t == 0) L.dmax[c] = move;
+    }
+    float ox = 0.f, oy = 0.f, oz = 0.f;
+    if (valid) { ox = own[3 * (size_t)q]; oy = own[3 * (size_t)q + 1]; oz = own[3 * (size_t)q + 2]; }
+    if (valid) {
+        const unsigned cnt = (is_row ? L.cnt_row : L.cnt_col)[(size_t)c * N + q];
+        const float tau = (is_row ? L.tau_row : L.tau_col)[(size_t)c * N + q];
+        const unsigned short *lst = (is_row ? L.list_row : L.list_col) + ((size_t)c * N + q) * cap;
+        const bool listed = cnt >= 1u && cnt <= (unsigned)cap;
+        float best = INFINITY;
+        int bi = 0;
+        if (listed) {
+            bi = 0x7fffffff;
+            for (unsigned s0 = 0; s0 < cnt; s0 += 8) {
+                int k[8];
+                float x[8], y[8], z[8];
+#pragma unroll
+                for (int u = 0; u < 8; ++u) k[u] = s0 + u < cnt ? min((int)lst[s0 + u], M - 1) : -1;
+#pragma unroll
+                for (int u = 0; u < 8; ++u) {
+                    const size_t o = 3 * (size_t)max(k[u], 0);
+                    x[u] = oth[o]; y[u] = oth[o + 1]; z[u] = oth[o + 2];
+                }
+#pragma unroll
+                for (int u = 0; u < 8; ++u) {
+                    const float d = rl_sqdist(x[u], y[u], z[u], ox, oy, oz);
+                    if (k[u] >= 0 && (d < best || (d == best && k[u] < bi))) { best = d; bi = k[u]; }
+                }
+            }
+        }
+        const float sd = rl_sqrt(best), st = rl_sqrt(tau);
+        const bool ok = listed && bi != 0x7fffffff && tau >= RL_TAU_MIN && (sd + move) + RL_MARGIN * st < st;
+        if (ok) {
+            if (!is_row) { a.q.dist2[(size_t)c * m + q] = best; a.q.idx2[(size_t)c * m + q] = bi; }
+            else if (a.q.row64) a.q.row64[(size_t)c * n + q] = sym_pack(best, bi);
+            else { a.q.dist1[(size_t)c * n + q] = best; a.q.idx1[(size_t)c * n + q] = bi; }
+        } else {
+            queue[atomicAdd(&qn, 1u)] = q;
+            if (!listed) atomicAdd(&unl, 1u);
+        }
+    }
+    __syncthreads();
+    const int nq = (int)qn;
+    for (int e = wave; e < nq; e += RL_THREADS / 64) {
+        const int qq = queue[e];
+        const float qx = own[3 * (size_t)qq], qy = own[3 * (size_t)qq + 1], qz = own[3 * (size_t)qq + 2];
+        float best = INFINITY;
+        int bi = 0;
+        for (int k0 = lane; k0 < M; k0 += 4 * 64) {
+            float x[4], y[4], z[4];
+#pragma unroll
+            for (int u = 0; u < 4; ++u) {
+                const size_t o = 3 * (size_t)min(k0 + 64 * u, M - 1);
+                x[u] = oth[o]; y[u] = oth[o + 1]; z[u] = oth[o + 2];
+            }
+#pragma unroll
+            for (int u = 0; u < 4; ++u) {
+                const float d = rl_sqdist(x[u], y[u], z[u], qx, qy, qz);
+                if (k0 + 64 * u < M && d < best) { best = d; bi = k0 + 64 * u; }
+            }
+        }
+        wave_lexmin(best, bi);
+        if (lane == 0) {
+            if (!is_row) { a.q.dist2[(size_t)c * m + qq] = best; a.q.idx2[(size_t)c * m + qq] = bi; }
+            else if (a.q.row64) a.q.row64[(size_t)c * n + qq] = sym_pack(best, bi);
+            else { a.q.dist1[(size_t)c * n + qq] = best; a.q.idx1[(size_t)c * n + qq] = bi; }
+        }
+    }
+    if (t == 0) {
+        const int mine = min(RL_THREADS, N - (q - t));
+        if (mine > nq) atomicAdd(&L.stats[0], (unsigned long long)(mine - nq));
+        if (nq > (int)unl) atomicAdd(&L.stats[1], (unsigned long long)(nq - (int)unl));
+        if (unl) atomicAdd(&L.stats[2], (unsigned long long)unl);
+        if (nq > THREADS / 4) a.need_next[8 * c + (blk & 7)] = 1;
+    }
+}
+
+
+template <int THREADS>
+__device__ __forceinline__ bool list_rider_block(const ListRider &r, unsigned *lds) {
+    if (r.blocks == 0 || (int)blockIdx.x < r.first_block) return false;
+    const int lin = (int)blockIdx.x - r.first_block;
+    recon_lists_query_block<THREADS>(r.a, lin % r.per_cloud, lin / r.per_cloud, lds);
+    return true;
+}
+#endif
+
+}
diff --git a/geometric_adv_amd/csrc/chamfer_lists.hip b/geometric_adv_amd/csrc/chamfer_lists.hip
--- /dev/null
+++ b/geometric_adv_amd/csrc/chamfer_lists.hip
@@ -0,0 +1,199 @@
+#include "chamfer_lists.h"
+#include "chamfer_sym.h"
+#include <math.h>
+
+#pragma clang fp contract(off)
+
+namespace geoadv {
+
+struct ListBuildArgs { ReconLists L; ListBuild in; int cslices, span; };
+
+__global__ __launch_bounds__(RL_THREADS) void recon_lists_build_kernel(ListBuildArgs a) {
+    __shared__ float4 sq[RL_THREADS];
+    const ReconLists &L = a.L;
+    const int c = blockIdx.y, n = L.n, m = L.m, cap = L.cap, t = threadIdx.x, lane = t & 63;
+    const int rt = blockIdx.x / a.cslices, cs = blockIdx.x % a.cslices;
+    const float *P = a.in.P + (size_t)c * n * 3, *Q = a.in.Q + (size_t)c * m * 3;
+    float skin;
+    if (a.in.skin) skin = a.in.skin[c];
+    else {
+        const float seen = L.dmax[c];
+        skin = seen > 0.f ? fminf(fmaxf(a.in.factor * seen, a.in.lo), a.in.hi) : a.in.first;
+    }
+    unsigned *crow = L.cnt_row + (size_t)c * n, *ccol = L.cnt_col + (size_t)c * m;
+    const int i = rt * RL_THREADS + t;
+    const bool rv = i < n;
+    float px = 0.f, py = 0.f, pz = 0.f, ti = -1.f;
+    if (rv) {
+        px = P[3 * i]; py = P[3 * i + 1]; pz = P[3 * i + 2];
+        const float d1 = a.in.row64 ? __uint_as_float((unsigned)(a.in.row64[(size_t)c * n + i] >> 32)) : a.in.dist1[(size_t)c * n + i];
+        ti = rl_tau(d1, skin);
+        if (cs == 0) {
+            L.tau_row[(size_t)c * n + i] = ti;
+            if (L.anchor != a.in.P) {
+                float *A = L.anchor + ((size_t)c * n + i) * 3;
+                A[0] = px; A[1] = py; A[2] = pz;
+            }
+        }
+    }
+    if (blockIdx.x == 0 && t == 0) {
+        L.skin[c] = skin;
+        if (a.in.hint && c == 0) {
+            for (int k = 0; k < 4; ++k) a.in.hint[k] = L.stats[k];
+            __threadfence_system();
+            a.in.hint[4] = a.in.serial;
+        }
+    }
+    unsigned short *lrow = L.list_row + (size_t)c * cap * n, *lcol = L.list_col + (size_t)c * cap * m;
+    const int k0 = cs * a.span, k1 = min(m, k0 + a.span);
+    for (int kb = k0; kb < k1; kb += RL_THREADS) {
+        __syncthreads();
+        {
+            const int k = kb + t;
+            float4 v = make_float4(INFINITY, INFINITY, INFINITY, -1.f);
+            if (k < k1) {
+                v.x = Q[3 * (size_t)k]; v.y = Q[3 * (size_t)k + 1]; v.z = Q[3 * (size_t)k + 2];
+                v.w = rl_tau(a.in.dist2[(size_t)c * m + k], skin);
+                if (rt == 0) L.tau_col[(size_t)c * m + k] = v.w;
+                if (__hip_atomic_load(&ccol[k], __ATOMIC_RELAXED, __HIP_MEMORY_SCOPE_AGENT) > (unsigned)cap) v.w = -1.f;
+            }
+            sq[t] = v;
+        }
+        __syncthreads();
+        const int cnt = min(RL_THREADS, k1 - kb), cnt4 = (cnt + 3) & ~3;
+        for (int u = 0; u < cnt4; u += 4) {
+            float4 q[4];
+            float d[4];
+            bool any = false;
+#pragma unroll
+            for (int j = 0; j < 4; ++j) {
+                q[j] = sq[u + j];
+                d[j] = rl_sqdist(q[j].x, q[j].y, q[j].z, px, py, pz);
+                any = any | (d[j] < ti) | (rv & (d[j] < q[j].w));
+            }
+            if (!__any(any)) continue;
+#pragma unroll
+            for (int j = 0; j < 4; ++j) {
+                const int k = kb + u + j;
+                if (d[j] < ti) {
+                    const unsigned slot = atomicAdd(&crow[i], 1u);
+                    if (slot < (unsigned)cap) lrow[(size_t)i * cap + slot] = (unsigned short)k;
+                }
+                const bool hc = rv && d[j] < q[j].w;
+                const unsigned long long mk = __ballot(hc);
+                if (mk) {
+                    const int leader = __ffsll((long long)mk) - 1;
+                    unsigned base = 0;
+                    if (lane == leader) {
+                        base = atomicAdd(&ccol[k], (unsigned)__popcll(mk));
+                        if (base + (unsigned)__popcll(mk) > (unsigned)cap) sq[u + j].w = -1.f;
+                    }
+                    base = (unsigned)__shfl((int)base, leader);
+                    if (hc) {
+                        const unsigned slot = base + (unsigned)__popcll(mk & ((1ull << lane) - 1ull));
+                        if (slot < (unsigned)cap) lcol[(size_t)k * cap + slot] = (unsigned short)i;
+                    }
+                }
+            }
+        }
+    }
+}
+
+__global__ __launch_bounds__(RL_THREADS) void recon_lists_query_kernel(ListQueryArgs a) {
+    __shared__ unsigned lds[RL_THREADS + 16];
+    recon_lists_query_block<RL_THREADS>(a, blockIdx.x, blockIdx.y, lds);
+}
+
+__global__ void recon_lists_state_kernel(ReconLists L, const int *need, unsigned long long *out, int *flags) {
+    const int c = blockIdx.x * blockDim.x + threadIdx.x;
+    if (c < 4) out[c] = L.stats[c];
+    if (c < L.b) flags[c] = sym_needed(need, c) ? 1 : 0;
+}
+
+size_t carve_recon_lists(ReconLists &L, void *base, int b, int n, int m, int cap, bool own_anchor) {
+    Carver cv(base);
+    const size_t B = (size_t)b;
+    L.b = b; L.n = n; L.m = m; L.cap = cap;
+    L.anchor = own_anchor ? cv.take<float>(B * n * 3) : nullptr;
+    L.tau_row = cv.take<float>(B * n); L.tau_col = cv.take<float>(B * m);
+    char *clr = cv.take<char>(sizeof(int) * (16 * B + B * n + B * m));
+    L.clear = clr; L.clear_bytes = sizeof(int) * (16 * B + B * n + B * m);
+    L.need[0] = reinterpret_cast<int *>(clr); L.need[1] = L.need[0] + 8 * B;
+    L.cnt_row = reinterpret_cast<unsigned *>(L.need[1] + 8 * B); L.cnt_col = L.cnt_row + B * n;
+    L.list_row = cv.take<unsigned short>(B * cap * n); L.list_col = cv.take<unsigned short>(B * cap * m);
+    L.dmax = cv.take<float>(B); L.skin = cv.take<float>(B);
+    L.stats = cv.take<unsigned long long>(4);
+    return cv.bytes();
+}
+
+int launch_recon_lists_build(const ReconLists &L, const ListBuild &in, hipStream_t st) {
+    GA_HIP(hipMemsetAsync(L.clear, 0, L.clear_bytes, st));
+    ListBuildArgs a;
+    a.L = L; a.in = in;
+    if (!a.L.anchor) a.L.anchor = const_cast<float *>(in.P);
+    const int rtiles = cdiv(L.n, RL_THREADS), stages = cdiv(L.m, RL_THREADS);
+    int cslices = 1;
+    while (cslices < stages && (long)rtiles * cslices * L.b < 4L * kCUs) cslices *= 2;
+    cslices = std::min(cslices, stages);
+    a.span = cdiv(stages, cslices) * RL_THREADS;
+    a.cslices = cdiv(L.m, a.span);
+    recon_lists_build_kernel<<<dim3(rtiles * a.cslices, L.b), RL_THREADS, 0, st>>>(a);
+    GA_LAUNCH_CHECK();
+    return GEOADV_OK;
+}
+
+ListRider recon_lists_rider(const ReconLists &L, const ListQuery &q, int threads) {
+    ListRider r;
+    r.a.L = L; r.a.q = q;
+    r.a.need_prev = L.need[q.call & 1]; r.a.need_next = L.need[(q.call + 1) & 1];
+    r.per_cloud = cdiv(L.n, threads) + cdiv(L.m, threads);
+    r.first_block = 0; r.blocks = r.per_cloud * L.b;
+    return r;
+}
+
+int launch_recon_lists_query(const ReconLists &L, const ListQuery &q, hipStream_t st) {
+    const ListQueryArgs a = recon_lists_rider(L, q, RL_THREADS).a;
+    recon_lists_query_kernel<<<dim3(cdiv(L.n, RL_THREADS) + cdiv(L.m, RL_THREADS), L.b), RL_THREADS, 0, st>>>(a);
+    GA_LAUNCH_CHECK();
+    return GEOADV_OK;
+}
+
+}
+
+using namespace geoadv;
+
+extern "C" size_t geoadv_nn_distance_lists_workspace_bytes(int b, int n, int m, int capacity) {
+    if (b <= 0 || n <= 0 || m <= 0 || capacity <= 0) return 256;
+    ReconLists L;
+    return carve_recon_lists(L, nullptr, b, n, m, capacity, false) + 256;
+}
+
+extern "C" int geoadv_nn_distance_lists(int b, int n, int m, const float *xyz1_anchor, const float *xyz2, const float *dist1_anchor,
+                                        const float *dist2_anchor, const float *skin, int capacity, const float *xyz1, float *dist1,
+                                        int *idx1, float *dist2, int *idx2, unsigned long long *state, int *flags, void *workspace,
+                                        size_t workspace_bytes, void *stream) {
+    GA_REQUIRE(b >= 0 && n >= 1 && m >= 1 && n <= RL_MAX_POINTS && m <= RL_MAX_POINTS,
+               "nn_distance_lists: bad dimensions (b=%d n=%d m=%d; clouds of at most %d points)", b, n, m, RL_MAX_POINTS);
+    GA_REQUIRE(capacity >= 1 && capacity <= RL_CAP_MAX, "nn_distance_lists: capacity=%d must be in [1, %d]", capacity, RL_CAP_MAX);
+    if (b == 0) return GEOADV_OK;
+    GA_REQUIRE(b <= 65535, "nn_distance_lists: at most 65535 clouds (got %d)", b);
+    GA_REQUIRE(xyz1_anchor && xyz2 && dist1_anchor && dist2_anchor && skin && xyz1 && dist1 && idx1 && dist2 && idx2 && state && flags && workspace,
+               "nn_distance_lists: null pointer");
+    GA_REQUIRE(workspace_bytes >= geoadv_nn_distance_lists_workspace_bytes(b, n, m, capacity),
+               "nn_distance_lists: workspace too small (%zu bytes, need %zu)", workspace_bytes,
+               geoadv_nn_distance_lists_workspace_bytes(b, n, m, capacity));
+    hipStream_t st = as_stream(stream);
+    ReconLists L;
+    carve_recon_lists(L, workspace, b, n, m, capacity, false);
+    GA_HIP(hipMemsetAsync(L.stats, 0, sizeof(unsigned long long) * 4, st));
+    ListBuild in{};
+    in.P = xyz1_anchor; in.Q = xyz2; in.dist1 = dist1_anchor; in.dist2 = dist2_anchor; in.skin = skin;
+    if (int rc = launch_recon_lists_build(L, in, st)) return rc;
+    L.anchor = const_cast<float *>(xyz1_anchor);
+    ListQuery q{};
+    q.P = xyz1; q.Q = xyz2; q.dist1 = dist1; q.idx1 = idx1; q.dist2 = dist2; q.idx2 = idx2; q.call = 0; q.answer_all = true;
+    if (int rc = launch_recon_lists_query(L, q, st)) return rc;
+    recon_lists_state_kernel<<<cdiv(std::max(b, 4), 256), 256, 0, st>>>(L, L.need[1], state, flags);
+    GA_LAUNCH_CHECK();
+    return GEOADV_OK;
+}
diff --git a/geometric_adv_amd/csrc/chamfer_sym.h b/geometric_adv_amd/csrc/chamfer_sym.h
--- a/geometric_adv_amd/csrc/chamfer_sym.h
+++ b/geometric_adv_amd/csrc/chamfer_sym.h
@@ -116,8 +116,10 @@
 struct GridArgs;
 struct JacRider;
 struct LossRider;
+struct ListRider;
 int launch_chamfer_sym(const SymPlan &p, const ChamferPair *pairs, float *workspace, const int *need1, const GridArgs *rider,
-                       const JacRider *jac, const LossRider *loss, unsigned long long *row64, hipStream_t stream);
+                       const JacRider *jac, const LossRider *loss, unsigned long long *row64, hipStream_t stream, const int *need0 = nullptr,
+                       const ListRider *lists = nullptr);
 int launch_chamfer_sym(const ChamferPair *pairs, int np, int b, int n, int m, float *workspace, hipStream_t stream);
 
 }
diff --git a/geometric_adv_amd/csrc/chamfer_sym.hip b/geometric_adv_amd/csrc/chamfer_sym.hip
--- a/geometric_adv_amd/csrc/chamfer_sym.hip
+++ b/geometric_adv_amd/csrc/chamfer_sym.hip
@@ -3,6 +3,7 @@
 #include "encoder_jac.h"
 #include "chamfer_sym.h"
 #include "chamfer_mx.h"
+#include "chamfer_lists.h"
 #include "loss_cgrad.h"
 #include <atomic>
 #include <limits.h>
@@ -29,6 +30,7 @@
     GridRider rider;
     JacRider jac;
     LossRider loss;
+    ListRider lists;
 };
 
 constexpr int CS_THREADS = 512;
@@ -79,6 +81,7 @@
     if (grid_rider_block<GR_MAX_N>(a.rider)) return;
     if (jac_rider_block(a.jac, stage)) return;
     if (loss_rider_block(a.loss, reinterpret_cast<unsigned *>(stage))) return;
+    if (list_rider_block<CS_THREADS>(a.lists, reinterpret_cast<unsigned *>(stage))) return;
     GA_STAMP(0, 0);
     const int lin = blockIdx.x - a.rider.blocks;
     const int xcd = lin & 7, slot = lin >> 3;
@@ -460,7 +463,7 @@
 }
 
 int launch_chamfer_sym(const SymPlan &p, const ChamferPair *pairs, float *workspace, const int *need1, const GridArgs *rider,
-                       const JacRider *jac, const LossRider *loss, unsigned long long *row64, hipStream_t stream) {
+                       const JacRider *jac, const LossRider *loss, unsigned long long *row64, hipStream_t stream, const int *need0, const ListRider *lists) {
     const SymRequest &r = p.req;
     if (p.grid == 0) return GEOADV_OK;
     GA_REQUIRE((need1 != nullptr) == r.need1 && (rider != nullptr) == (p.search.count > 0) && (jac != nullptr) == (p.jac.count > 0) &&
@@ -468,7 +471,7 @@
                "chamfer_sym: the launch's arguments are not the ones its plan was made for");
     const SymShape &s = p.shape;
     ChamferSymArgs a;
-    a.need[0] = nullptr; a.need[1] = need1;
+    a.need[0] = need0; a.need[1] = need1;
     a.pair_base = r.pair_base; a.q_clouds = r.q_clouds;
     for (int i = 0; i < r.np; ++i) a.pr[i] = pairs[i];
     a.n = r.n; a.m = r.m; a.clouds = r.b; a.pairs = r.np;
@@ -493,7 +496,13 @@
     if (p.loss.count) a.loss = *loss;
     else a.loss.done = nullptr;
     a.loss.first_block = p.loss.first; a.loss.blocks = p.loss.count; a.loss.clouds = r.b;
-    if (p.kernel == 0) chamfer_sym_kernel<<<p.grid, CS_THREADS, p.lds_bytes, stream>>>(a);
+    a.lists.blocks = 0;
+    if (lists) {
+        GA_REQUIRE(p.kernel == 0 && p.loss.count == 0, "chamfer_sym: this plan cannot host the list queries");
+        a.lists = *lists;
+        a.lists.first_block = (int)p.grid;
+    }
+    if (p.kernel == 0) chamfer_sym_kernel<<<p.grid + (unsigned)a.lists.blocks, CS_THREADS, p.lds_bytes, stream>>>(a);
     else chamfer_mx_kernel<8><<<p.grid, MX_THREADS, p.lds_bytes, stream>>>(a);
     GA_LAUNCH_CHECK();
     if (p.rows != GEOADV_PLAN_ROWS_MERGE_LAUNCH) return GEOADV_OK;
diff --git a/geometric_adv_amd/ops.py b/geometric_adv_amd/ops.py
--- a/geometric_adv_amd/ops.py
+++ b/geometric_adv_amd/ops.py
@@ -81,6 +81,38 @@
                                                _lib.ptr(dist2), _lib.ptr(idx2), _lib.ptr(ws), wf, _lib.stream_handle())
     _lib.check(st, "nn_distance_sym")
     return dist1, idx1, dist2, idx2
+
+
+def nn_distance_lists(xyz1_anchor, xyz2, dist1_anchor, dist2_anchor, skin, xyz1, capacity=16):
+    xyz1_anchor, xyz2 = _xyz_pair(xyz1_anchor, xyz2, "NnDistanceLists")
+    xyz1 = _f32(xyz1, "xyz1", 3)
+    if tuple(xyz1.shape) != tuple(xyz1_anchor.shape):
+        raise ValueError("nn_distance_lists expects xyz1 of the anchor's shape")
+    b, n, _ = xyz1.shape
+    m = xyz2.shape[1]
+    dev = xyz1.device
+    d1a, d2a = _f32(dist1_anchor, "dist1_anchor", 2), _f32(dist2_anchor, "dist2_anchor", 2)
+    if tuple(d1a.shape) != (b, n) or tuple(d2a.shape) != (b, m):
+        raise ValueError("nn_distance_lists expects the anchor minima as (b, n) and (b, m)")
+    sk = torch.as_tensor(skin, dtype=torch.float32, device=dev).reshape(-1)
+    sk = (sk.expand(b) if sk.numel() == 1 else sk).contiguous()
+    if sk.numel() != b:
+        raise ValueError("nn_distance_lists expects one skin, or one per cloud")
+    dist1 = torch.empty((b, n), dtype=torch.float32, device=dev)
+    idx1 = torch.empty((b, n), dtype=torch.int32, device=dev)
+    dist2 = torch.empty((b, m), dtype=torch.float32, device=dev)
+    idx2 = torch.empty((b, m), dtype=torch.int32, device=dev)
+    state = torch.zeros((4,), dtype=torch.int64, device=dev)
+    flags = torch.zeros((b,), dtype=torch.int32, device=dev)
+    wb = int(_lib.lib().geoadv_nn_distance_lists_workspace_bytes(b, n, m, int(capacity)))
+    ws = torch.empty((wb,), dtype=torch.uint8, device=dev)
+    with torch.cuda.device(dev):
+        st = _lib.lib().geoadv_nn_distance_lists(b, n, m, _lib.ptr(xyz1_anchor), _lib.ptr(xyz2), _lib.ptr(d1a), _lib.ptr(d2a),
+                                                 _lib.ptr(sk), int(capacity), _lib.ptr(xyz1), _lib.ptr(dist1), _lib.ptr(idx1),
+                                                 _lib.ptr(dist2), _lib.ptr(idx2), _lib.ptr(state), _lib.ptr(flags), _lib.ptr(ws), wb,
+                                                 _lib.stream_handle())
+    _lib.check(st, "nn_distance_lists")
+    return dist1, idx1, dist2, idx2, state[:3], flags
 
 
 def chamfer_per_pc(dist1, dist2):
diff --git a/include/geoadv.h b/include/geoadv.h
--- a/include/geoadv.h
+++ b/include/geoadv.h
@@ -26,6 +26,12 @@
 int geoadv_nn_distance_sym(int b, int n, const float *xyz1, int m, const float *xyz2,
                            float *dist1, int *idx1, float *dist2, int *idx2,
                            float *workspace, size_t workspace_floats, void *stream);
+
+size_t geoadv_nn_distance_lists_workspace_bytes(int b, int n, int m, int capacity);
+int geoadv_nn_distance_lists(int b, int n, int m, const float *xyz1_anchor, const float *xyz2, const float *dist1_anchor,
+                             const float *dist2_anchor, const float *skin, int capacity, const float *xyz1, float *dist1,
+                             int *idx1, float *dist2, int *idx2, unsigned long long *state, int *flags, void *workspace,
+                             size_t workspace_bytes, void *stream);
 
 int geoadv_chamfer_per_pc(int b, int n, int m, const float *dist1, const float *dist2, float *out, void *stream);
 
@@ -441,6 +447,7 @@
     int   encoder_backward;
     int   separate_adam;
     int   chamfer_kernel;
+    int   recon_lists;
     int    knn_rule;
     float  knn_thresh;
     float  knn_weight;
@@ -456,6 +463,9 @@
 #define GEOADV_CHAMFER_AUTO      0
 #define GEOADV_CHAMFER_TWO_SCAN  1
 #define GEOADV_CHAMFER_SYMMETRIC 2
+#define GEOADV_RECON_LISTS_ADAPTIVE 0
+#define GEOADV_RECON_LISTS_OFF      1
+#define GEOADV_RECON_LISTS_PINNED   2
 
 int  geoadv_attack_create(geoadv_attack **out, const geoadv_ae *ae, const geoadv_attack_config *cfg);
 void geoadv_attack_destroy(geoadv_attack *at);
@@ -515,6 +525,12 @@
 
 int geoadv_attack_search_state(geoadv_attack *at, int *searched, int *handed_back, void *stream);
 
+int geoadv_attack_set_recon_lists(geoadv_attack *at, int on);
+enum { GEOADV_LIST_STATE_ON = 0, GEOADV_LIST_STATE_ANCHORS, GEOADV_LIST_STATE_LIST_ITERATIONS, GEOADV_LIST_STATE_CERTIFIED,
+       GEOADV_LIST_STATE_REFUSED, GEOADV_LIST_STATE_UNLISTED, GEOADV_LIST_STATE_HANDED_BACK, GEOADV_LIST_STATE_FLAGGED,
+       GEOADV_LIST_STATE_PERIOD, GEOADV_LIST_STATE_COUNT };
+int geoadv_attack_list_state(geoadv_attack *at, long long state[GEOADV_LIST_STATE_COUNT], void *stream);
+
 typedef struct geoadv_trainer geoadv_trainer;
 typedef struct geoadv_train_config {
     int   batch;
```

Result: faster. 10240 attack-iterations/sec (median of 6 runs) (+7.7%).
